# giuliop/AlgoPlonk

Hardware: AMD Instinct MI355X
Metric: proofs/sec (higher is better)
Workload: dtype u32x8 (Montgomery Fr/Fp)

## Files before the change

algoplonk_amd/_lib.py:

```python
from __future__ import annotations

import ctypes as C
import os

_HERE = os.path.dirname(os.path.abspath(__file__))
LIB_PATH = os.environ.get("APK_LIB") or os.path.join(_HERE, "libapk.so")

APK_BN254 = 0
APK_BLS12_381 = 1
APK_OK = 0
APK_ERR_ARG, APK_ERR_HIP, APK_ERR_STATE, APK_ERR_WITNESS, APK_ERR_VERIFY = 1, 2, 3, 4, 5
ABI_VERSION = 5
G1_MAX = 96
G2_MAX = 192
MAX_COMMITMENTS = 2
NB_BLINDING = 9

SYMBOLS = [
    "apk_last_error", "apk_abi_version", "apk_device_count", "apk_g1_bytes", "apk_fp_bytes",
    "apk_ctx_create", "apk_ctx_destroy", "apk_msm_ctx_create", "apk_ctx_get_vk", "apk_msm_g1", "apk_msm_g1_device", "apk_msm_g1_batch_device", "apk_ctx_set_commit_hook", "apk_device_copy", "apk_ntt",
    "apk_prove", "apk_prove_device", "apk_verify", "apk_verify_ex", "apk_g2_decompress", "apk_g2_mul_generator", "apk_g1_mul_batch", "apk_g1_decompress", "apk_g1_to_lagrange", "apk_marshal_proof", "apk_marshal_public_inputs",
    "apk_fe_from_be", "apk_fe_to_be", "apk_hash_fr", "apk_host_fe_op", "apk_host_g1_op", "apk_g1_sum",
    "apk_device_fe_op", "apk_device_g1_op", "apk_host_feu_op", "apk_device_feu_op", "apk_feu_shape", "apk_device_poly_op",
    "apk_device_alloc", "apk_device_free", "apk_device_upload", "apk_device_download",
    "apk_host_alloc", "apk_host_free", "apk_host_register", "apk_host_unregister",
    "apk_stats_enable", "apk_stats_read", "apk_paths_read",
    "apk_ctx_set_wire_hook", "apk_coset_ntt_device",
    "apk_comm_create", "apk_comm_destroy", "apk_comm_rank", "apk_comm_world", "apk_comm_barrier", "apk_comm_max_f64", "apk_comm_bind",
    "apk_comm_transport", "apk_msm_g1_sharded", "apk_comm_split_begin", "apk_comm_split_end", "apk_comm_serve", "apk_comm_set_compute",
    "apk_comm_commit", "apk_comm_wires", "apk_comm_rccl_ranks", "apk_comm_rccl_selftest",
    "apk_comm_commit_local", "apk_comm_spmd_begin", "apk_comm_spmd_end", "apk_comm_allgather_device", "apk_comm_subcoset_active",
    "apk_ctx_set_subcoset", "apk_comm_transport_reason", "apk_comm_link_probe", "apk_comm_phase_ms", "apk_ctx_msm_window",
    "apk_verify_batch", "apk_g1_lincomb_segments", "apk_device_sched_read", "apk_runtime_read",
    "apk_kzg_open", "apk_kzg_open_device", "apk_kzg_batch_open", "apk_kzg_batch_open_device", "apk_kzg_verify", "apk_kzg_batch_verify",
    "apk_kzg_fold_challenge", "apk_kzg_shape",
    "apk_kzg_open_lagrange", "apk_kzg_open_lagrange_device", "apk_kzg_batch_open_lagrange", "apk_kzg_batch_open_lagrange_device",
    "apk_kzg_lagrange_shape",
    "apk_kzg_open_multi", "apk_kzg_open_multi_device", "apk_kzg_batch_verify_multi", "apk_kzg_multi_weights",
    "apk_kzg_open_multi_lagrange", "apk_kzg_open_multi_lagrange_device",
    "apk_kzg_all_prepare", "apk_kzg_open_all", "apk_kzg_open_all_device",
    "apk_kzg_cosets_prepare", "apk_kzg_open_cosets", "apk_kzg_open_cosets_device", "apk_kzg_verify_coset",
    "apk_kzg_batch_verify_cosets", "apk_kzg_cosets_weights", "apk_kzg_cosets_fold", "apk_kzg_cosets_phase_ms",
    "apk_proof_blob_len", "apk_unmarshal_proof", "apk_unmarshal_public_inputs", "apk_verify_blob", "apk_verify_batch_keys", "apk_verify_blobs",
]


class ApkError(RuntimeError):
    def __init__(self, code: int, msg: str):
        super().__init__("libapk error %d: %s" % (code, msg))
        self.code = code


class CircuitDesc(C.Structure):
    _fields_ = [
        ("curve", C.c_int), ("device", C.c_int), ("n", C.c_uint64), ("nb_public", C.c_uint32),
        ("nb_commitments", C.c_uint32), ("srs_g1", C.c_void_p), ("srs_g1_lagrange", C.c_void_p),
        ("ql", C.c_void_p), ("qr", C.c_void_p), ("qm", C.c_void_p), ("qo", C.c_void_p), ("qk", C.c_void_p),
        ("perm", C.c_void_p), ("qcp", C.c_void_p * MAX_COMMITMENTS),
        ("commitment_constraint_index", C.c_uint32 * MAX_COMMITMENTS), ("msm_window", C.c_int), ("slots", C.c_int),
# ... 45 lines not shown
    ]


class VerifyKeysTrace(C.Structure):
    _fields_ = [
        ("d", C.c_uint8 * 32), ("rho", (C.c_uint8 * 32) * 4), ("lin_commitment", (C.c_uint8 * G1_MAX) * 4),
        ("a", C.c_uint8 * G1_MAX), ("b", C.c_uint8 * G1_MAX), ("groups", C.c_uint32), ("folds", C.c_uint32),
    ]


class KzgVk(C.Structure):
    _fields_ = [("curve", C.c_int), ("g1", C.c_uint8 * G1_MAX), ("g2", (C.c_uint8 * G2_MAX) * 2)]


class Stats(C.Structure):
    _fields_ = [
        ("msm_accumulate_ms", C.c_double), ("msm_accumulate_launches", C.c_uint64), ("msm_pairs", C.c_uint64),
        ("msm_total_ms", C.c_double), ("msm_batches", C.c_uint64), ("ntt_ms", C.c_double), ("ntt_elements", C.c_uint64),
        ("prove_ms", C.c_double), ("proofs", C.c_uint64), ("round_ms", C.c_double * 4), ("host_lincomb_ms", C.c_double),
        ("msm_sort_ms", C.c_double), ("msm_tail_ms", C.c_double),
    ]


class PathCounts(C.Structure):
    _names = ["proofs", "msm_batches", "msm_sort_two_level", "msm_sort_two_level_by_load", "msm_sort_fused", "msm_lean_tail",
              "msm_rowcol_serial", "msm_combine_quad", "msm_small_units", "msm_one_launch", "msm_lagrange_wires", "ntt_sequences",
              "ntt_radix4", "ntt_radix4_by_load", "tail_fill_proofs", "host_lincomb_pooled", "msm_units_by_load", "host_inputs",
              "gang_proofs", "gang_msm_launches", "gang_ntt_launches", "gang_kernel_launches", "forms_by_device_load"]
    _later = ["msm_inplace"]
    _fields_ = [(n, C.c_uint64) for n in _names + _later]

    def as_dict(self) -> dict:
        return {n: int(getattr(self, n)) for n in self._names + self._later}


class DeviceSched(C.Structure):
    _names = ["contexts", "max_streams", "streams_in_use", "streams_peak", "proofs_in_flight", "proofs_peak", "waiting", "device_wide"]
    _fields_ = [(n, C.c_uint32) for n in _names]

    def as_dict(self) -> dict:
        return {n: int(getattr(self, n)) for n in self._names}


HWQ_UNSET, HWQ_UNREADABLE = -1, -2


class Runtime(C.Structure):
    _names = ["hw_queues_found", "hw_queues_left", "hw_queues_need", "hw_queues_written", "hw_queues_now", "first_hip_call",
              "hw_queues_at_first_hip", "reserved"]
    _fields_ = [(n, C.c_int32) for n in _names]

    def as_dict(self) -> dict:
        return {n: int(getattr(self, n)) for n in self._names if n != "reserved"}


POLY_VECS, POLY_FRS, POLY_INTS, POLY_OUTS = 32, 24, 8, 6
(POLY_GRAND_PRODUCT, POLY_SCAN, POLY_QUOTIENT, POLY_MERGE, POLY_EVAL, POLY_LINCOMB, POLY_DERIVE_POWERS, POLY_KZG_QUOTIENT, POLY_BLIND,
 POLY_BLIND3, POLY_TAIL, POLY_KZG_QUOTIENT2) = range(12)


class PolyArgs(C.Structure):
    _fields_ = [("vec", C.c_void_p * POLY_VECS), ("len", C.c_uint64 * POLY_VECS), ("fr", (C.c_uint8 * 32) * POLY_FRS),
                ("iv", C.c_int64 * POLY_INTS), ("out", C.c_void_p * POLY_OUTS), ("out_len", C.c_uint64 * POLY_OUTS)]


COMMIT_HOOK = C.CFUNCTYPE(C.c_int, C.c_void_p, C.c_int, C.c_uint32, C.POINTER(C.c_void_p), C.POINTER(C.c_uint32), C.c_void_p)
# ... 52 lines not shown
                                         C.POINTER(vp), C.POINTER(sz), C.c_uint32, C.POINTER(i32), C.POINTER(VerifyKeysTrace)]
    lib.apk_g1_lincomb_segments.argtypes = [i32, i32, vp, vp, C.POINTER(u64), C.c_uint32, vp]
    lib.apk_g2_decompress.argtypes = [i32, vp, vp]
    lib.apk_g2_mul_generator.argtypes = [i32, vp, vp]
    lib.apk_g1_mul_batch.argtypes = [i32, i32, vp, vp, u64, vp]
    lib.apk_g1_decompress.argtypes = [i32, i32, vp, u64, vp]
    lib.apk_g1_to_lagrange.argtypes = [i32, i32, vp, u64, vp]
    lib.apk_marshal_proof.argtypes = [C.POINTER(Proof), vp, sz, C.POINTER(sz)]
    lib.apk_marshal_public_inputs.argtypes = [i32, vp, C.c_uint32, vp, sz]
    lib.apk_fe_from_be.argtypes = [i32, i32, vp, vp]
    lib.apk_fe_to_be.argtypes = [i32, i32, vp, vp]
    lib.apk_hash_fr.argtypes = [i32, vp, vp]
    lib.apk_host_fe_op.argtypes = [i32, i32, i32, vp, vp, vp]
    lib.apk_host_g1_op.argtypes = [i32, i32, vp, vp, vp]
    lib.apk_device_fe_op.argtypes = [i32, i32, i32, i32, u64, vp, vp, vp]
    lib.apk_device_g1_op.argtypes = [i32, i32, i32, u64, vp, vp, vp]
    lib.apk_host_feu_op.argtypes = [i32, i32, i32, u64, vp, vp]
    lib.apk_device_feu_op.argtypes = [i32, i32, i32, i32, u64, vp, vp]
    lib.apk_feu_shape.argtypes = [i32, i32, C.POINTER(i32), C.POINTER(i32), C.POINTER(C.c_uint32)]
    if hasattr(lib, "apk_device_poly_op"):
        lib.apk_device_poly_op.argtypes = [i32, i32, i32, C.POINTER(PolyArgs)]
    lib.apk_g1_sum.argtypes = [i32, vp, u64, vp]
    lib.apk_device_alloc.argtypes = [vp, sz, C.POINTER(vp)]
    lib.apk_device_free.argtypes = [vp, vp]
    lib.apk_device_upload.argtypes = [vp, vp, vp, sz]
    lib.apk_device_download.argtypes = [vp, vp, vp, sz]
    lib.apk_host_alloc.argtypes = [i32, sz, C.POINTER(vp)]
    lib.apk_host_free.argtypes = [vp]
    lib.apk_host_register.argtypes = [vp, sz]
    lib.apk_host_unregister.argtypes = [vp]
    lib.apk_stats_enable.argtypes = [vp, i32]
    lib.apk_stats_read.argtypes = [vp, C.POINTER(Stats), i32]
    lib.apk_paths_read.argtypes = [vp, C.POINTER(PathCounts), i32]
    if hasattr(lib, "apk_device_sched_read"):
        lib.apk_device_sched_read.argtypes = [i32, C.POINTER(DeviceSched), i32]
    if hasattr(lib, "apk_runtime_read"):
        lib.apk_runtime_read.argtypes = [C.POINTER(Runtime)]
    lib.apk_ctx_msm_window.argtypes = [vp]
    lib.apk_ctx_set_wire_hook.argtypes = [vp, WIRE_HOOK, vp]
    lib.apk_coset_ntt_device.argtypes = [vp, vp, u64, vp]
    lib.apk_comm_create.argtypes = [i32, i32, C.c_char_p, i32, C.POINTER(vp)]
    lib.apk_comm_destroy.argtypes = [vp]; lib.apk_comm_destroy.restype = None
    lib.apk_comm_rank.argtypes = [vp]
    lib.apk_comm_world.argtypes = [vp]
    lib.apk_comm_barrier.argtypes = [vp]
    lib.apk_comm_max_f64.argtypes = [vp, C.POINTER(C.c_double)]
    lib.apk_comm_bind.argtypes = [vp, vp]
    lib.apk_comm_transport.argtypes = [vp]; lib.apk_comm_transport.restype = C.c_char_p
    lib.apk_comm_rccl_ranks.argtypes = [vp]
    lib.apk_comm_transport_reason.argtypes = [vp]; lib.apk_comm_transport_reason.restype = C.c_char_p
    lib.apk_comm_link_probe.argtypes = [vp, sz, sz, C.POINTER(C.c_double), C.POINTER(C.c_double)]
    lib.apk_comm_phase_ms.argtypes = [vp, C.POINTER(C.c_double), i32]
    lib.apk_comm_rccl_selftest.argtypes = [i32, C.POINTER(i32)]
    lib.apk_msm_g1_sharded.argtypes = [vp, vp, u64, vp]
    lib.apk_comm_split_begin.argtypes = [vp]
    lib.apk_comm_split_end.argtypes = [vp]
    lib.apk_comm_serve.argtypes = [vp, C.POINTER(u64)]
    lib.apk_comm_set_compute.argtypes = [vp, C.POINTER(Compute)]
    lib.apk_comm_commit.argtypes = [vp, i32, C.c_uint32, vp, vp, vp]
    lib.apk_comm_wires.argtypes = [vp, C.c_uint32, vp, vp, vp]
    lib.apk_comm_commit_local.argtypes = [vp, i32, C.c_uint32, vp, vp, vp]
    lib.apk_comm_spmd_begin.argtypes = [vp]
    lib.apk_comm_spmd_end.argtypes = [vp]
    lib.apk_comm_allgather_device.argtypes = [vp, vp, C.c_size_t]
    lib.apk_comm_subcoset_active.argtypes = [vp]
    lib.apk_ctx_set_subcoset.argtypes = [vp, i32, i32, vp, vp]
# ... 69 lines not shown
```

algoplonk_amd/csrc/apk_api.cpp:

```cpp
#include <stdarg.h>
#include <stdio.h>
#include <stdlib.h>
#include <string.h>
#include <atomic>
#include <mutex>
#include <string>
#include <type_traits>

#include <hip/hip_runtime_api.h>

#include "backend.h"
#include "device_sched.h"
#include "ec.h"
#include "kernels_kzg.h"
#include "kernels_kzg_lagrange.h"
#include "plonk_protocol.h"
#include "poly_run.h"
#include "proof_codec.h"
#include "runtime_env.h"
#include "selftest_ops.h"

namespace apk {

static thread_local std::string g_err;
// ... 492 lines not shown
    if (e != hipSuccess) { (void)hipGetLastError(); set_error("hipHostRegister(%zu): %s", bytes, hipGetErrorString(e)); return APK_ERR_HIP; }
    return APK_OK;
}
int apk_host_unregister(void* p) {
    if (!p) return APK_OK;
    hipError_t e = hipHostUnregister(p);
    if (e != hipSuccess) { (void)hipGetLastError(); set_error("hipHostUnregister: %s", hipGetErrorString(e)); return APK_ERR_HIP; }
    return APK_OK;
}

int apk_device_alloc(apk_ctx* ctx, size_t bytes, void** p) { NEED_CTX(); return ctx->be->dev_alloc(bytes, p); }
int apk_device_free(apk_ctx* ctx, void* p) { NEED_CTX(); return ctx->be->dev_free(p); }
int apk_device_upload(apk_ctx* ctx, void* d, const void* s, size_t b) { NEED_CTX(); return ctx->be->dev_upload(d, s, b); }
int apk_device_download(apk_ctx* ctx, void* d, const void* s, size_t b) { NEED_CTX(); return ctx->be->dev_download(d, s, b); }
int apk_stats_enable(apk_ctx* ctx, int en) { NEED_CTX(); return ctx->be->stats_enable(en); }
int apk_stats_read(apk_ctx* ctx, apk_stats* out, int reset) { NEED_CTX(); if (!out) { set_error("null out"); return APK_ERR_ARG; } return ctx->be->stats_read(out, reset); }
int apk_ctx_msm_window(apk_ctx* ctx) { if (!ctx || !ctx->be) return 0; return ctx->be->msm_window(); }
int apk_device_sched_read(int device, apk_device_sched* out, int reset) {
    if (!out) { set_error("null out"); return APK_ERR_ARG; }
    if (device < 0 || device >= 4096) { set_error("device %d out of range", device); return APK_ERR_ARG; }
    memset(out, 0, sizeof *out);
    out->max_streams = (uint32_t)sched_max_streams();
    out->device_wide = sched_device_wide() ? 1u : 0u;
    DeviceSched* sc = device_sched_for(device);
    if (!sc) return APK_OK;
    const DeviceSched::Counts c = sc->read(reset != 0);
    out->contexts = c.contexts; out->max_streams = c.max_streams;
    out->streams_in_use = c.streams_in_use; out->streams_peak = c.streams_peak;
    out->proofs_in_flight = c.proofs_in_flight; out->proofs_peak = c.proofs_peak;
    out->waiting = c.waiting;
    return APK_OK;
}
int apk_paths_read(apk_ctx* ctx, apk_path_counts* out, int reset) { NEED_CTX(); if (!out) { set_error("null out"); return APK_ERR_ARG; } return ctx->be->paths_read(out, reset); }
int apk_runtime_read(apk_runtime* out) {
    if (!out) { set_error("null out"); return APK_ERR_ARG; }
    memset(out, 0, sizeof *out);
    out->hw_queues_found = g_runtime.found; out->hw_queues_left = g_runtime.left;
    out->hw_queues_need = g_runtime.need; out->hw_queues_written = g_runtime.written;
    out->hw_queues_now = hwq_parse(getenv("GPU_MAX_HW_QUEUES"));
    out->first_hip_call = g_runtime.first_hip.load();
    out->hw_queues_at_first_hip = g_runtime.at_first_hip.load();
    return APK_OK;
}

int apk_g1_mul_batch(int curve, int device, const void* base, const void* scalars, uint64_t count, void* out) {
    if (!base || !scalars || !out) { set_error("null argument"); return APK_ERR_ARG; }
    if (count == 0) return APK_OK;
    if (count >= (1ull << 31)) { set_error("count too large"); return APK_ERR_ARG; }
    runtime_checkpoint();
    if (curve == APK_BN254) return g1_mul_batch_bn254(device, base, scalars, count, out);
    if (curve == APK_BLS12_381) return g1_mul_batch_bls12381(device, base, scalars, count, out);
    set_error("unsupported curve: %d", curve);
    return APK_ERR_ARG;
}

int apk_g1_decompress(int curve, int device, const uint8_t* compressed, uint64_t count, void* out) {
    if (!compressed || !out) { set_error("null argument"); return APK_ERR_ARG; }
    if (count == 0) return APK_OK;
    if (count >= (1ull << 31)) { set_error("count too large"); return APK_ERR_ARG; }
    runtime_checkpoint();
    if (curve == APK_BN254) return g1_decompress_bn254(device, compressed, count, out);
    if (curve == APK_BLS12_381) return g1_decompress_bls12381(device, compressed, count, out);
    set_error("unsupported curve: %d", curve);
    return APK_ERR_ARG;
}

// ... 124 lines not shown
```

algoplonk_amd/csrc/backend.h:

```cpp
#pragma once
#include <stdint.h>
#include <stddef.h>
#include <stdarg.h>
#include <stdio.h>
#include "../../include/apk.h"

namespace apk {

void set_error(const char* fmt, ...);

int env_int(const char* name, int dflt, int lo, int hi);

bool ctx_alive(const void* ctx);

class DeviceSched;
DeviceSched* device_sched_for(int device);
int device_stream_pool(int device, void** streams, int cap, int* count);

struct Backend {
    virtual ~Backend() {}
    virtual int init(const apk_circuit_desc* d) = 0;
    virtual int init_msm_only(int device, const void* bases, uint64_t count, int msm_window) = 0;
    virtual int get_vk(apk_vk* out) = 0;
    virtual int msm(int basis, const void* scalars, uint64_t len, bool on_device, void* out) = 0;
    virtual int msm_batch(int basis, uint32_t count, const void* const* d_scalars, const uint64_t* offsets, const uint64_t* lens, void* out) = 0;
    virtual int kzg_open(const void* poly, uint64_t len, bool on_device, const void* point, void* out_h, void* out_value) = 0;
    virtual int kzg_batch_open(uint32_t count, const void* const* polys, const uint64_t* lens, bool on_device, const void* digests,
                               const void* point, const uint8_t* extra, size_t extra_len, void* out_h, void* out_values, void* out_gamma) = 0;
    virtual int kzg_open_multi(uint32_t count, const void* const* polys, const uint64_t* lens, bool on_device, const void* points,
                               void* out_h, void* out_values) = 0;
    virtual int kzg_open_lagrange(const void* evals, uint64_t len, bool on_device, const void* point, void* out_h, void* out_value) = 0;
    virtual int kzg_batch_open_lagrange(uint32_t count, const void* const* evals, bool on_device, const void* digests, const void* point,
                                        const uint8_t* extra, size_t extra_len, void* out_h, void* out_values, void* out_gamma) = 0;
    virtual int kzg_open_multi_lagrange(uint32_t count, const void* const* evals, bool on_device, const void* points, void* out_h,
                                        void* out_values) = 0;
    virtual int kzg_all_prepare(const void* srs_g1, uint64_t count) = 0;
    virtual int kzg_open_all(const void* poly, uint64_t len, bool on_device, void* out_h, void* out_values) = 0;
    virtual int kzg_cosets_prepare(const void* srs_g1, uint64_t count, uint32_t coset_size) = 0;
    virtual int kzg_open_cosets(const void* poly, uint64_t len, bool on_device, void* out_h, void* out_values) = 0;
    virtual int set_commit_hook(apk_commit_hook fn, void* user) = 0;
    virtual int dev_copy(void* d, const void* s, size_t bytes) = 0;
    virtual int set_wire_hook(apk_wire_hook fn, void* user) = 0;
    virtual int set_subcoset(int k, int G, apk_gather_hook fn, void* user) = 0;
    virtual int device_ordinal() = 0;
    virtual int msm_window() = 0;
    virtual uint64_t domain_size() = 0;
    virtual int coset_ntt_dev(const void* d_in, uint64_t len, void* d_out) = 0;
    virtual int ntt(int which, int inverse, int coset, void* data) = 0;
    virtual int prove(const void* L, const void* R, const void* O, bool on_device, const void* pub, const void* blinding,
                      const void* const* pi2, apk_proof* out) = 0;
    virtual int dev_alloc(size_t bytes, void** p) = 0;
    virtual int dev_free(void* p) = 0;
    virtual int dev_upload(void* d, const void* s, size_t bytes) = 0;
    virtual int dev_download(void* d, const void* s, size_t bytes) = 0;
    virtual int stats_enable(int enable) = 0;
    virtual int stats_read(apk_stats* out, int reset) = 0;
    virtual int paths_read(apk_path_counts* out, int reset) = 0;
};

int g1_mul_batch_bn254(int device, const void* base, const void* scalars, uint64_t count, void* out);
int g1_mul_batch_bls12381(int device, const void* base, const void* scalars, uint64_t count, void* out);
int g1_decompress_bn254(int device, const uint8_t* in, uint64_t count, void* out);
int g1_decompress_bls12381(int device, const uint8_t* in, uint64_t count, void* out);
int g1_to_lagrange_bn254(int device, const void* points, uint64_t n, void* out);
int g1_to_lagrange_bls12381(int device, const void* points, uint64_t n, void* out);
int fe_op_device_bn254(int device, int field, int op, uint64_t count, const void* a, const void* b, void* out);
int fe_op_device_bls12381(int device, int field, int op, uint64_t count, const void* a, const void* b, void* out);
int feu_op_device_bn254(int device, int field, int op, uint64_t count, const void* in, void* out);
int feu_op_device_bls12381(int device, int field, int op, uint64_t count, const void* in, void* out);
int g1_op_device_bn254(int device, int op, uint64_t count, const void* p, const void* q, void* out);
int g1_op_device_bls12381(int device, int op, uint64_t count, const void* p, const void* q, void* out);
int poly_op_device_bn254(int device, int op, const apk_poly_args* args);
int poly_op_device_bls12381(int device, int op, const apk_poly_args* args);
int g1_lincomb_segments_bn254(int device, const void* points, const void* scalars, const uint64_t* seg, uint32_t nb_segments, void* out);
int g1_lincomb_segments_bls12381(int device, const void* points, const void* scalars, const uint64_t* seg, uint32_t nb_segments, void* out);
int g1_check_points_bn254(int device, const void* points, uint64_t count, uint8_t* flags);
int g1_check_points_bls12381(int device, const void* points, uint64_t count, uint8_t* flags);
int kzg_cosets_fold_bn254(int device, int log_l, uint32_t count, const void* values, const void* scale, const void* step, const void* tw, void* out);
int kzg_cosets_fold_bls12381(int device, int log_l, uint32_t count, const void* values, const void* scale, const void* step, const void* tw, void* out);
Backend* make_backend_bn254();
Backend* make_backend_bls12381();

int host_fe_from_be(int curve, int field, const uint8_t* be, void* out);
int host_fe_to_be(int curve, int field, const void* in, uint8_t* be);

}
```

algoplonk_amd/csrc/backend_impl.h:

```cpp
#pragma once
#include <hip/hip_runtime.h>
#include <algorithm>
#include <atomic>
#include <chrono>
#include <condition_variable>
#include <memory>
#include <new>
#include <mutex>
#include <string.h>
#include <time.h>
#include <vector>

#include "backend.h"
#include "dev_buf.h"
#include "slot_pinned.h"
#include "msm_run.h"
#include "kzg_run.h"
#include "kzg_all_run.h"
#include "kzg_cosets_run.h"
#include "ntt_run.h"
#include "kernels_poly.h"
#include "poly_run.h"
#include "gang_run.h"
#include "setup_run.h"
// ... 3 lines not shown
#include "plonk_protocol.h"

namespace apk {

template <class FRP, class FPP, int CURVE_ID>
class CurveBackend : public Backend {
  public:
    using Fr = Fe<FRP>;
    using Fp = Fe<FPP>;
    using Aff = Affine<FPP>;
    using Pt = XYZZ<FPP>;
    using PtU = XYZZ<FPP, FeU<FPP>>;
    using Proto = PlonkProtocol<FRP, FPP>;

    static Fr fr_u64(uint64_t v) {
        Fr a = Fr::zero();
        a.l[0] = (uint32_t)v;
        a.l[1] = (uint32_t)(v >> 32);
        return Fr::to_mont(a);
    }

    static_assert(PIN_AFF + MSM_MAX_BATCH * sizeof(Aff) <= PIN_XYZZ, "a proof's batch of affine commitments fits its region");
    static_assert(PIN_XYZZ + MSM_ARGS_MAX * sizeof(Pt) <= PIN_FR, "the XYZZ sums of a launch sequence fit their region");
    static_assert(PIN_FR + (EVAL_MAX > KZG_MAX_POLYS ? EVAL_MAX : KZG_MAX_POLYS) * sizeof(Fr) <= PIN_TAIL, "evaluations and an opening's values fit the scalar region");

    struct ProverKnobs {
        int lc_threads = env_int("APK_HOST_LINCOMB_THREADS", FPP::N <= 8 ? 1 : 3, 1, 8);
        bool host_glv = env_int("APK_HOST_GLV", 1, 0, 1) != 0;
        bool host_fixed = env_int("APK_HOST_FIXED", 1, 0, 1) != 0;
        int powers_derive = env_int("APK_POWERS_DERIVE", 1, 0, 1);
        int open_pair = env_int("APK_OPEN_PAIR", 1, 0, 1);
        int lin_early_h = env_int("APK_LIN_EARLY_H", 1, 0, 1);
        int tail_fill = env_int("APK_TAIL_FILL", 1, 0, 2);
    };
    static const ProverKnobs& prover_knobs() { static const ProverKnobs k{}; return k; }

    struct GraphKey {
        const void* table; MsmBatchArgs a;
        bool operator==(const GraphKey& o) const { return table == o.table && memcmp(&a, &o.a, sizeof a) == 0; }
    };
    struct Slot {
        hipStream_t stream = nullptr;
        hipStream_t own_stream = nullptr;
        Slot* lead = nullptr;
        int gang_idx = 0;
        bool in_gang = false;
        uint32_t res_off = 0;
        uint32_t res_write_off = 0;
        Gang gang;
        GangRecorder cmds;
        hipEvent_t ev0 = nullptr, ev1 = nullptr, ev2 = nullptr, ev3 = nullptr;
        size_t index = 0;
        DevBuf wl, wr, wo;
        DevBuf cl, cr, co, cz;
        DevBuf qk_lag, qk_can;
        DevBuf ratio, zlag, scan_tot;
        DevBuf el, er, eo, ez, eqk;
        DevBuf quot, hcan;
        DevBuf pw_z, pw_zi, pw_zw, pw_zwi;
        DevBuf tmp2, folded, tmp, q1, q2;
        DevBuf eval_partial, eval_result;
        DevBuf pi2_can[APK_MAX_COMMITMENTS], epi2[APK_MAX_COMMITMENTS];
        DevBuf scratch_in;
        KzgScratch<FRP> kzg;
        KzgAllScratch<FRP, FPP> kzg_all;
        KzgCosetsScratch<FRP, FPP> kzg_cosets;
        DevBuf ntt_wide;
        MsmWorkspace<FPP> msm;
        void* h_pinned = nullptr;
        uint32_t pending_pts = 0;
        uint8_t* d_pinned = nullptr;
        std::vector<std::pair<GraphKey, hipGraphExec_t>> graphs;
        bool hook_pending = false;
        int hook_basis = 0;
        MsmBatchArgs hook_args{};
        DevBuf sc_gather;
        DevBuf tail_flag;
        uint32_t epoch = 0;
        hipStream_t side = nullptr;
        hipEvent_t ev_acc = nullptr, ev_side = nullptr;
        hipEvent_t ev_sync = nullptr;
        int mark_acc = 0; bool side_pending = false;
    };

    int curve_ = CURVE_ID;
    int device_ = 0;
    uint32_t n_ = 0, log_n_ = 0, n4_ = 0;
    uint32_t nb_public_ = 0, nb_commit_ = 0;
    uint32_t cci_[APK_MAX_COMMITMENTS] = {0, 0};
    MsmCtxPlan msm_ctx_{};
    bool msm_only_ = false;
    std::unique_ptr<HostPool> lc_pool_;
    bool many_slots_ = false;
    int gang_cap_ = 1;
    uint32_t ws_batch_ = MSM_MAX_BATCH;
    Gang::Launcher gang_launcher_;
    uint32_t msm_bases_ = 0;
    Fr omega_, omega_inv_, omega4_, omega4_inv_, shift_, shift_inv_, n_inv_, n4_inv_;
    Fr zh_inv_[4];
    DevBuf tw_n_, twu_n_, twi_n_, tw_4n_, twi_4n_, coset_pre_, coset_post_inv_, scales_;
    DevBuf twu_n_x_, twi_n_x_, tw_4n_x_, twi_4n_x_;
    bool ntt_twu_ = false;
    DevBuf x4_, l0_4_;
    DevBuf s_lag_[3], ql_c_, qr_c_, qm_c_, qo_c_, qk_c_, s_c_[3], qcp_c_[APK_MAX_COMMITMENTS];
    DevBuf qk_lag_trace_;
    bool qk_direct_ = false;
    DevBuf eqk_trace_, inj_tab_[QK_INJECT_MAX];
    std::vector<uint32_t> inj_row_;
    std::vector<Fr> inj_trace_val_;
    DevBuf eql_, eqr_, eqm_, eqo_, es_[3], eqcp_[APK_MAX_COMMITMENTS];
    MsmTables tab_can_, tab_lag_;
    int wires_lag_mode_ = -1;
    DevBuf srs_keep_;
    Aff lag_dk_[3];
// ... 8 lines not shown
    KzgAllTables<FRP, FPP> all_tab_;
    std::mutex all_mu_;
    std::atomic<bool> all_ready_{false};
    bool tw_ready_ = false;
    KzgCosetsTables cos_tab_;
    std::atomic<uint32_t> cos_l_{0};
    std::vector<Slot*> slots_;
    std::vector<hipStream_t> stream_pool_;
    bool owns_streams_ = false;
    SlotGate gate_;
    struct InputSet {
        DevBuf w[3], pi2[APK_MAX_COMMITMENTS];
        hipStream_t copy = nullptr;
        hipEvent_t ready = nullptr;
        size_t index = 0;
    };
    std::vector<InputSet*> in_sets_;
    SlotGate in_gate_;
    hipStream_t copy_stream_ = nullptr;
    std::mutex mu_;
    apk_commit_hook hook_ = nullptr;
    void* hook_user_ = nullptr;
    apk_wire_hook wire_hook_ = nullptr;
    void* wire_hook_user_ = nullptr;
    struct SubCoset {
        int k = 0, G = 1, glog = 0;
        apk_gather_hook hook = nullptr;
        void* user = nullptr;
        DevBuf pre[2], post;
        Fr rho_inv[8];
        bool on() const { return G > 1 && hook; }
    } sc_;
    enum PathIdx { P_PROOFS, P_MSM_BATCHES, P_SORT2, P_SORT2_LOAD, P_SORT_FUSED, P_LEAN_TAIL, P_ROWCOL_SERIAL, P_COMBINE_QUAD, P_SMALL_UNITS,
                   P_ONE_LAUNCH, P_LAGRANGE_WIRES, P_NTT_SEQ, P_NTT_R4, P_NTT_R4_LOAD, P_TAIL_FILL, P_LINCOMB_POOL, P_UNIT_LOADED, P_HOST_INPUTS, P_GANG_PROOFS, P_GANG_MSM, P_GANG_NTT, P_GANG_KERNELS, P_DEVICE_LOAD, P_MSM_INPLACE, P_COUNT };
    std::atomic<uint64_t> paths_[P_COUNT] = {};
    void path(PathIdx i) { paths_[i].fetch_add(1, std::memory_order_relaxed); }
    bool device_load_over(int thr, bool* foreign = nullptr) {
        int own = 0;
        const int dev = gate_.load(&own);
        if (foreign) *foreign = dev > thr && own <= thr;
        return dev > thr;
    }
    int paths_read(apk_path_counts* out, int reset) override {
        static_assert(sizeof(apk_path_counts) >= P_COUNT * sizeof(uint64_t), "apk_path_counts holds every counter");
        memset(out, 0, sizeof *out);
        uint64_t* o = reinterpret_cast<uint64_t*>(out);
        for (int i = 0; i < P_COUNT; i++) o[i] = reset ? paths_[i].exchange(0, std::memory_order_relaxed) : paths_[i].load(std::memory_order_relaxed);
        return APK_OK;
    }
    bool stats_on_ = false;
    uint32_t simds_ = 1024;
    std::mutex stats_mu_;
    apk_stats stats_{};

    ~CurveBackend() override {
        (void)hipSetDevice(device_);
        gate_.detach();
        for (hipStream_t st : stream_pool_) if (st) (void)hipStreamSynchronize(st);
        if (copy_stream_) (void)hipStreamSynchronize(copy_stream_);
        for (InputSet* is : in_sets_) {
            if (is->ready) (void)hipEventDestroy(is->ready);
            delete is;
        }
        if (copy_stream_) (void)hipStreamDestroy(copy_stream_);
        for (Slot* s : slots_) {
            for (auto& e : s->graphs) (void)hipGraphExecDestroy(e.second);
            if (s->ev0) (void)hipEventDestroy(s->ev0);
            if (s->ev1) (void)hipEventDestroy(s->ev1);
            if (s->ev2) (void)hipEventDestroy(s->ev2);
            if (s->ev3) (void)hipEventDestroy(s->ev3);
            if (s->h_pinned) (void)hipHostFree(s->h_pinned);
            if (s->side) { (void)hipStreamSynchronize(s->side); (void)hipStreamDestroy(s->side); }
            if (s->ev_acc) (void)hipEventDestroy(s->ev_acc);
            if (s->ev_side) (void)hipEventDestroy(s->ev_side);
            if (s->ev_sync) (void)hipEventDestroy(s->ev_sync);
            delete s;
        }
        if (owns_streams_) for (hipStream_t st : stream_pool_) if (st) (void)hipStreamDestroy(st);
    }

    int run_ntt_batch(hipStream_t st, int which, bool inverse, int count, const Fr* const* ins, Fr* const* outs, const uint32_t* in_lens,
                      uint32_t out_len, const Fr* pre, const Fr* post, const Fr* scale, int sub_log = 0, bool semi = false) {
        Slot* m = gang_member();
        if (m && m->in_gang && st == m->stream && count <= NTT_MAX_BATCH) {
            NttReq<Fr> nr{};
            nr.which = which; nr.inverse = inverse; nr.count = count;
            for (int i = 0; i < count; i++) { nr.ins[i] = ins[i]; nr.outs[i] = outs[i]; nr.in_lens[i] = in_lens[i]; }
            nr.out_len = out_len; nr.pre = pre; nr.post = post; nr.scale = scale; nr.sub_log = sub_log; nr.semi = semi;
            GangReq r;
            r.kind = GANG_KIND_NTT; r.args = &nr; r.member = m;
            const int rc = m->lead->gang.meet(m->gang_idx, r, gang_launcher_);
            if (rc != APK_OK) set_error("%s", r.err.c_str());
            return rc;
        }
        return run_ntt_batch_now(st, which, inverse, count, ins, outs, in_lens, out_len, pre, post, scale, sub_log, semi);
    }
    const Fr* ntt_table(int which, bool inverse) const {
        if (ntt_twu_) return which ? (inverse ? ptr<Fr>(twi_4n_x_) : ptr<Fr>(tw_4n_x_)) : (inverse ? ptr<Fr>(twi_n_x_) : ptr<Fr>(twu_n_x_));
        return which ? (inverse ? ptr<Fr>(twi_4n_) : ptr<Fr>(tw_4n_)) : (inverse ? ptr<Fr>(twi_n_) : ptr<Fr>(twu_n_));
    }
    int run_ntt_batch_now(hipStream_t st, int which, bool inverse, int count, const Fr* const* ins, Fr* const* outs, const uint32_t* in_lens,
                          uint32_t out_len, const Fr* pre, const Fr* post, const Fr* scale, int sub_log = 0, bool semi = false) {
        const int log_n = (which ? (int)log_n_ + 2 : (int)log_n_) - sub_log;
        Slot* owner = nullptr;
        for (Slot* s : slots_) if (s->own_stream == st || (s->side && s->side == st)) owner = s;
        bool busy_now = false, busy_foreign = false;
        if (slots_.size() > 2 && ntt_plan_reads_load(log_n)) busy_now = device_load_over(1, &busy_foreign);
        const NttPlanIn in{log_n, count, out_len, sub_log, semi, (uint32_t)sizeof(FeU<FRP>), owner != nullptr, busy_now, busy_foreign};
        const NttPlan plan = ntt_plan(ntt_knobs(), in);
        if (plan.rc != APK_OK) { set_error("%s", plan.message); return plan.rc; }
        NttBatch nb{};
        for (int i = 0; i < count; i++) { nb.in[i] = ins[i]; nb.out[i] = outs[i]; nb.in_len[i] = in_lens[i]; }
        if (plan.needs_wide) for (int i = 0; i < count; i++) nb.wide[i] = ptr<FeU<FRP>>(owner->ntt_wide) + ((size_t)i << log_n);
        static constexpr PathIdx PATH_OF_BIT[] = {P_NTT_SEQ, P_NTT_R4, P_NTT_R4_LOAD, P_DEVICE_LOAD};
        for (uint32_t i = 0; i < sizeof PATH_OF_BIT / sizeof PATH_OF_BIT[0]; i++) if (plan.paths >> i & 1u) path(PATH_OF_BIT[i]);
        Slot* timed = stats_on_ ? owner : nullptr;
        if (timed) HIPCHK(hipEventRecord(timed->ev2, st));
        CHK(ntt_launch<FRP>(st, plan, nb, count, ntt_table(which, inverse), ntt_twu_, pre, post, scale));
        if (timed) {
            HIPCHK(hipEventRecord(timed->ev3, st));
            HIPCHK(hipEventSynchronize(timed->ev3));
            float ms = 0;
            HIPCHK(hipEventElapsedTime(&ms, timed->ev2, timed->ev3));
            std::lock_guard<std::mutex> g(stats_mu_);
            stats_.ntt_ms += ms;
            stats_.ntt_elements += ((uint64_t)1 << log_n) * count;
        }
        return APK_OK;
    }
    int run_ntt(hipStream_t st, int which, bool inverse, const Fr* in, Fr* out, uint32_t in_len, uint32_t out_len,
                const Fr* pre, const Fr* post, const Fr* scale, int sub_log = 0, bool semi = false) {
        return run_ntt_batch(st, which, inverse, 1, &in, &out, &in_len, out_len, pre, post, scale, sub_log, semi);
    }
    int coset_eval(hipStream_t st, int count, const Fr* const* ins, const uint32_t* lens, Fr* const* outs, int cls = 0) {
        if (!sc_.on()) return run_ntt_batch(st, 1, false, count, ins, outs, lens, n4_, ptr<Fr>(coset_pre_), nullptr, nullptr, 0, true);
        return run_ntt_batch(st, 1, false, count, ins, outs, lens, n4_ >> sc_.glog, ptr<Fr>(sc_.pre[cls]), nullptr, nullptr, sc_.glog);
    }
    int inv_ntt_n(hipStream_t st, const Fr* in, Fr* out) { return run_ntt(st, 0, true, in, out, n_, n_, nullptr, nullptr, ptr<Fr>(scales_)); }
    int coset_ntt_4n(hipStream_t st, const Fr* in, uint32_t len, Fr* out, bool semi = false) {
        return run_ntt(st, 1, false, in, out, len, n4_, ptr<Fr>(coset_pre_), nullptr, nullptr, 0, semi);
    }

    int build_lagrange_table(hipStream_t st, const Aff* d_srs, const void* h_lagrange) {
        DevBuf lag;
        CHK(lag.alloc((size_t)(n_ + 3) * sizeof(Aff)));
        if (h_lagrange) HIPCHK(hipMemcpyAsync(lag.p, h_lagrange, (size_t)n_ * sizeof(Aff), hipMemcpyHostToDevice, st));
        else CHK((g1_to_lagrange_dev<FRP, FPP>(d_srs, n_, ptr<Aff>(lag), st)));
        HIPCHK(hipMemcpyAsync(ptr<Aff>(lag) + n_, lag_dk_, sizeof lag_dk_, hipMemcpyHostToDevice, st));
        CHK((build_tables<FRP, FPP>(st, msm_ctx_, ptr<Aff>(lag), n_ + 3, tab_lag_, true)));
        HIPCHK(hipStreamSynchronize(st));
        lag_ready_.store(true, std::memory_order_release);
        return APK_OK;
    }
    bool lagrange_ready() const { return lag_ready_.load(std::memory_order_acquire); }
    bool lagrange_possible() const { return lagrange_ready() || (srs_keep_.p && !lag_failed_.load(std::memory_order_relaxed)); }
    bool ensure_lagrange_table(hipStream_t st) {
        if (lagrange_ready()) return true;
        std::lock_guard<std::mutex> lk(lag_mu_);
        if (lagrange_ready()) return true;
        if (!srs_keep_.p || lag_failed_.load(std::memory_order_relaxed)) return false;
        const int rc = build_lagrange_table(st, ptr<Aff>(srs_keep_), nullptr);
        if (rc != APK_OK) {
            (void)hipGetLastError();
            tab_lag_.table.release();
            tab_lag_.built = false;
// ... 24 lines not shown
        HIPCHK(hipStreamBeginCapture(s.stream, hipStreamCaptureModeThreadLocal));
        const int rc = run_msm_body(s, T, a);
        const hipError_t e = hipStreamEndCapture(s.stream, &g);
        if (rc != APK_OK) { if (g) (void)hipGraphDestroy(g); return rc; }
        HIPCHK(e);
        hipGraphExec_t exec = nullptr;
        HIPCHK(hipGraphInstantiate(&exec, g, nullptr, nullptr, 0));
        (void)hipGraphDestroy(g);
        constexpr size_t GRAPH_CACHE = 8;
        if (s.graphs.size() >= GRAPH_CACHE) {
            HIPCHK(hipStreamSynchronize(s.stream));
            (void)hipGraphExecDestroy(s.graphs.back().second);
            s.graphs.pop_back();
        }
        s.graphs.insert(s.graphs.begin(), std::make_pair(key, exec));
        HIPCHK(hipGraphLaunch(exec, s.stream));
        s.pending_pts = a.batch;
        return APK_OK;
    }

    int run_msm_body(Slot& s, const MsmTables& T, const MsmBatchArgs& a) {
        hipStream_t st = s.stream;
        MsmBatchIn in{};
        in.batch = a.batch; in.len = a.len; in.offset = a.offset;
        in.n_bases = T.n_bases; in.ctx_bases = msm_bases_;
        in.simds = simds_; in.slots = (uint32_t)slots_.size();
        if (slots_.size() > 2) in.others_busy = device_load_over(1, &in.others_foreign);
        in.scan_runs = APK_PHASE(32);
        in.ws_batch = ws_batch_;
        in.lt_max = MsmQuad<FPP>::LT;
        in.counts_words = s.msm.counts.bytes / 4; in.sort_tmp_bytes = s.msm.sort_tmp.bytes;
        in.has_sort_tmp = s.msm.sort_tmp.p != nullptr; in.has_ptot2 = s.msm.ptot2.p != nullptr;
        const MsmBatchPlan p = msm_plan_batch(msm_ctx_, msm_knobs(), in);
        static constexpr PathIdx PATH_OF_BIT[] = {P_UNIT_LOADED, P_SMALL_UNITS, P_SORT2, P_SORT2_LOAD, P_SORT_FUSED, P_LEAN_TAIL, P_COMBINE_QUAD, P_ROWCOL_SERIAL, P_DEVICE_LOAD, P_MSM_INPLACE};
        for (uint32_t i = 0; i < sizeof PATH_OF_BIT / sizeof PATH_OF_BIT[0]; i++) if (p.paths >> i & 1u) path(PATH_OF_BIT[i]);
        if (p.rc == APK_ERR_ARG) { set_error("%s", p.message); return p.rc; }
        if (p.rc == APK_OK) {
            path(P_MSM_BATCHES);
            if (s.res_write_off + a.batch > (uint32_t)MSM_ARGS_MAX) { set_error("msm: result area overflow"); return APK_ERR_STATE; }
        }
        Pt* const res_out = s.d_pinned ? pin_dev<Pt>(s.d_pinned, PIN_XYZZ) + s.res_write_off : ptr<Pt>(s.msm.result_xyzz);
        MsmEvents ev;
        if (stats_on_) { ev.before = s.ev0; ev.scanned = s.ev2; ev.accumulated = s.ev3; ev.reduced = s.ev1; }
        ev.acc = s.ev_acc; ev.mark_acc = s.mark_acc;
        CHK((msm_launch_batch<FRP, FPP>(st, msm_ctx_, s.msm, ptr<Aff>(T.table), T.n_bases, a, p, res_out, ev)));
        if (!s.d_pinned) HIPCHK(hipMemcpyAsync(pin_host<Pt>(s.h_pinned, PIN_XYZZ) + s.res_write_off, s.msm.result_xyzz.p, a.batch * sizeof(Pt), hipMemcpyDeviceToHost, st));
        s.pending_pts = a.batch;
        if (stats_on_) {
            HIPCHK(hipEventSynchronize(s.ev1));
            float tot = 0, acc = 0, srt = 0, tail = 0;
            HIPCHK(hipEventElapsedTime(&tot, s.ev0, s.ev1));
            HIPCHK(hipEventElapsedTime(&acc, s.ev2, s.ev3));
            HIPCHK(hipEventElapsedTime(&srt, s.ev0, s.ev2));
            HIPCHK(hipEventElapsedTime(&tail, s.ev3, s.ev1));
            std::lock_guard<std::mutex> g(stats_mu_);
            stats_.msm_sort_ms += srt;
            stats_.msm_tail_ms += tail;
            stats_.msm_total_ms += tot;
            stats_.msm_batches += 1;
            stats_.msm_accumulate_ms += acc;
            stats_.msm_accumulate_launches += 1;
            for (uint32_t b = 0; b < a.batch; b++) stats_.msm_pairs += a.len[b];
        }
        return APK_OK;
    }

    static Slot*& hook_slot() { static thread_local Slot* p = nullptr; return p; }

    int commit(Slot& s, const MsmTables& T, int basis, const MsmBatchArgs& a) {
        if (!hook_ && s.in_gang) {
            MsmReq mr{&T, a};
            GangReq r;
            r.kind = GANG_KIND_MSM; r.args = &mr; r.member = &s;
            const int rc = s.lead->gang.meet(s.gang_idx, r, gang_launcher_);
            if (rc != APK_OK) set_error("%s", r.err.c_str());
            return rc;
        }
        if (!hook_) return run_msm(s, T, a);
        for (uint32_t b = 0; b < a.batch; b++)
            if (a.len[b] > T.n_bases || a.offset[b] > T.n_bases - a.len[b]) { set_error("msm: %u scalars exceed the %u bases", a.len[b], T.n_bases); return APK_ERR_ARG; }
        s.hook_pending = true; s.hook_basis = basis; s.hook_args = a;
        s.hook_args.plain = T.plain ? 1u : 0u;
        return APK_OK;
    }

    int tail_fill(Slot& s) {
        const int on = prover_knobs().tail_fill;
        const int graphs = msm_knobs().graph;
        if (!on || graphs || hook_ || wire_hook_ || stats_on_ || !qk_direct_ || sc_.on()) return 0;
        if (gate_.load() != 1) return 0;
        if (!s.side) {
            int least = 0, greatest = 0;
            (void)hipDeviceGetStreamPriorityRange(&least, &greatest);
            if (hipStreamCreateWithPriority(&s.side, hipStreamNonBlocking, least) != hipSuccess) { s.side = nullptr; return 0; }
            if (hipEventCreateWithFlags(&s.ev_acc, hipEventDisableTiming) != hipSuccess ||
                hipEventCreateWithFlags(&s.ev_side, hipEventDisableTiming) != hipSuccess) return 0;
        }
        return s.ev_acc && s.ev_side ? on : 0;
    }
    int side_begin(Slot& s) { HIPCHK(hipStreamWaitEvent(s.side, s.ev_acc, 0)); return APK_OK; }
    int side_end(Slot& s) { HIPCHK(hipEventRecord(s.ev_side, s.side)); s.side_pending = true; return APK_OK; }

    int wait_stream(Slot& s) {
        static const int mode = env_int("APK_SYNC_BLOCKING", -1, -1, 2);
        static const int poll_us = env_int("APK_SYNC_POLL_US", 50, 1, 10000);
        const bool loaded = slots_.size() > 2 && device_load_over(2);
        if (s.ev_sync && (mode == 2 || (mode < 0 && loaded))) {
            HIPCHK(hipEventRecord(s.ev_sync, s.stream));
            for (;;) {
                const hipError_t e = hipEventQuery(s.ev_sync);
                if (e == hipSuccess) return APK_OK;
                if (e != hipErrorNotReady) { (void)hipGetLastError(); set_error("hipEventQuery: %s", hipGetErrorString(e)); return APK_ERR_HIP; }
                struct timespec ts = {0, (long)poll_us * 1000L};
                nanosleep(&ts, nullptr);
            }
        }
        if (mode == 1 && s.ev_sync) {
            HIPCHK(hipEventRecord(s.ev_sync, s.stream));
            HIPCHK(hipEventSynchronize(s.ev_sync));
            return APK_OK;
        }
        HIPCHK(hipStreamSynchronize(s.stream));
        return APK_OK;
    }

    int sync_results(Slot& s) {
        if (s.in_gang) {
            GangReq r;
            r.kind = GANG_KIND_FLUSH; r.member = &s;
            const int rc = s.lead->gang.meet(s.gang_idx, r, gang_launcher_);
            if (rc != APK_OK) { set_error("%s", r.err.c_str()); return rc; }
        }
        CHK(wait_stream(s));
        if (s.side_pending) { s.side_pending = false; HIPCHK(hipStreamWaitEvent(s.stream, s.ev_side, 0)); }
        if (s.hook_pending) {
            s.hook_pending = false;
            const MsmBatchArgs& a = s.hook_args;
            uint8_t pts[MSM_MAX_BATCH * sizeof(Aff)];
            hook_slot() = &s;
            const int rc = hook_(hook_user_, s.hook_basis, a.batch, a.scalars, a.len, pts);
            hook_slot() = nullptr;
            if (rc != APK_OK) { set_error("commit hook failed with %d", rc); return rc == APK_ERR_ARG ? APK_ERR_ARG : APK_ERR_STATE; }
            memcpy(pin_host<Aff>(s.h_pinned, PIN_AFF), pts, a.batch * sizeof(Aff));
            s.pending_pts = 0;
            return APK_OK;
        }
        const Slot& from = s.lead ? *s.lead : s;
        const Pt* g = pin_host<Pt>(from.h_pinned, PIN_XYZZ) + s.res_off;
        static_assert(MSM_MAX_BATCH <= HOST_AFFINE_BATCH, "a proof's batch of sums is one batch conversion");
        host_xyzz_batch_to_affine<FPP>(g, s.pending_pts, pin_host<Aff>(s.h_pinned, PIN_AFF));
        s.pending_pts = 0;
        return APK_OK;
    }

    int alloc_slot(Slot& s) {
        s.lead = &s;
        HIPCHK(hipEventCreate(&s.ev0));
        HIPCHK(hipEventCreate(&s.ev1));
        HIPCHK(hipEventCreate(&s.ev2));
        HIPCHK(hipEventCreate(&s.ev3));
        if (hipEventCreateWithFlags(&s.ev_sync, hipEventBlockingSync | hipEventDisableTiming) != hipSuccess) { (void)hipGetLastError(); s.ev_sync = nullptr; }
        HIPCHK(hipHostMalloc(&s.h_pinned, PIN_BYTES, hipHostMallocDefault));
        memset(s.h_pinned, 0, PIN_BYTES);
        static const int zero_copy = env_int("APK_ZERO_COPY", 1, 0, 1);
        if (zero_copy) {
            void* dp = nullptr;
            if (hipHostGetDevicePointer(&dp, s.h_pinned, 0) == hipSuccess) s.d_pinned = static_cast<uint8_t*>(dp);
            else (void)hipGetLastError();
        }
        const size_t fn = (size_t)n_ * sizeof(Fr), fn3 = (size_t)(n_ + 4) * sizeof(Fr), f4 = (size_t)n4_ * sizeof(Fr);
        if (msm_only_) {
            CHK(s.scratch_in.alloc((size_t)msm_bases_ * sizeof(Fr)));
            return s.msm.alloc(msm_ctx_, msm_knobs(), msm_bases_, 1, many_slots_);
        }
        CHK(s.wl.alloc(fn3)); CHK(s.wr.alloc(fn3)); CHK(s.wo.alloc(fn3));
        CHK(s.cl.alloc(fn3)); CHK(s.cr.alloc(fn3)); CHK(s.co.alloc(fn3)); CHK(s.cz.alloc(fn3));
        for (DevBuf* b : {&s.cl, &s.cr, &s.co, &s.cz}) HIPCHK(hipMemset(b->p, 0, fn3));
        CHK(s.qk_lag.alloc(fn)); CHK(s.qk_can.alloc(fn));
        CHK(s.ratio.alloc(fn)); CHK(s.zlag.alloc(fn));
        CHK(s.scan_tot.alloc((size_t)(2 * (cdiv(n_ + 4, SCAN_BLOCK) + 1) + 2) * sizeof(Fr)));
        CHK(s.el.alloc(f4)); CHK(s.er.alloc(f4)); CHK(s.eo.alloc(f4)); CHK(s.ez.alloc(f4)); CHK(s.eqk.alloc(f4));
        CHK(s.quot.alloc(f4)); CHK(s.hcan.alloc(f4));
        CHK(s.pw_z.alloc(fn3)); CHK(s.pw_zi.alloc(fn3)); CHK(s.pw_zw.alloc(fn3)); CHK(s.pw_zwi.alloc(fn3));
        CHK(s.tmp2.alloc(fn3)); CHK(s.folded.alloc(fn3)); CHK(s.tmp.alloc(fn3)); CHK(s.q1.alloc(fn3)); CHK(s.q2.alloc(fn3));
        CHK(s.eval_partial.alloc((size_t)EVAL_MAX * cdiv(n_ + 4, EVAL_BLOCK) * sizeof(Fr)));
        CHK(s.eval_result.alloc(EVAL_MAX * sizeof(Fr)));
        for (uint32_t k = 0; k < nb_commit_; k++) { CHK(s.pi2_can[k].alloc(fn)); CHK(s.epi2[k].alloc(f4)); }
        CHK(s.scratch_in.alloc(f4));
        CHK(s.tail_flag.alloc(16));
        HIPCHK(hipMemset(s.tail_flag.p, 0, 16));
        CHK(s.ntt_wide.alloc((size_t)NTT_MAX_BATCH * gang_cap_ * n4_ * sizeof(FeU<FRP>)));
        return s.msm.alloc(msm_ctx_, msm_knobs(), msm_bases_, ws_batch_, many_slots_);
    }

// ... 113 lines not shown
            pr[i] = reqs[i]->kind == GANG_KIND_MSM ? msm_of(reqs[i]).plan_req() : reqs[i]->kind == GANG_KIND_NTT ? ntt_of(reqs[i]).plan_req() : GangPlanReq{GANG_KIND_FLUSH, 0, nullptr, GangNttShape{}};
            recs[i] = &member_of(reqs[i]).cmds;
        }
        const GangPlan plan = gang_plan_meeting(pr, count, ws_batch_, (uint32_t)(NTT_MAX_BATCH * gang_cap_));
        int merged = 0;
        const int frc = gang_flush(recs, count, member_of(reqs[0]).stream, &merged);
        for (int i = 0; i < merged; i++) path(P_GANG_KERNELS);
        if (frc != APK_OK) {
            for (int i = 0; i < count; i++) { reqs[i]->rc = frc; reqs[i]->err = apk_last_error(); }
            return;
        }
        for (int i = 0; i < count; i++) if (reqs[i]->kind == GANG_KIND_FLUSH) reqs[i]->rc = APK_OK;
        for (int gi = 0; gi < plan.groups; gi++) {
            const GangGroup& g = plan.group[gi];
            Slot& lead = *member_of(reqs[g.req[0]]).lead;
            int rc;
            if (g.kind == GANG_KIND_MSM) {
                MsmBatchArgs c{};
                c.batch = g.total;
                for (int k = 0; k < g.n; k++) {
                    const MsmBatchArgs& a = msm_of(reqs[g.req[k]]).a;
                    for (uint32_t b = 0; b < a.batch; b++) { c.scalars[g.first[k] + b] = a.scalars[b]; c.len[g.first[k] + b] = a.len[b]; c.offset[g.first[k] + b] = a.offset[b]; }
                    member_of(reqs[g.req[k]]).res_off = g.res_off(k);
                }
                const uint32_t lead_pending = lead.pending_pts;
                lead.res_write_off = g.res_base;
                rc = run_msm(lead, *msm_of(reqs[g.req[0]]).T, c);
                lead.res_write_off = 0;
                lead.pending_pts = lead_pending;
                if (g.n > 1) path(P_GANG_MSM);
                for (int k = 0; k < g.n; k++) member_of(reqs[g.req[k]]).pending_pts = rc == APK_OK ? msm_of(reqs[g.req[k]]).a.batch : 0;
            } else {
                const Fr* ins[NTT_ARGS_MAX]; Fr* outs[NTT_ARGS_MAX]; uint32_t lens[NTT_ARGS_MAX];
                for (int k = 0; k < g.n; k++) {
                    const NttReq<Fr>& m = ntt_of(reqs[g.req[k]]);
                    for (int t = 0; t < m.count; t++) { ins[g.first[k] + t] = m.ins[t]; outs[g.first[k] + t] = m.outs[t]; lens[g.first[k] + t] = m.in_lens[t]; }
                }
                const NttReq<Fr>& f = ntt_of(reqs[g.req[0]]);
                rc = run_ntt_batch_now(lead.own_stream, f.which, f.inverse, (int)g.total, ins, outs, lens, f.out_len, f.pre, f.post, f.scale, f.sub_log, f.semi);
                if (g.n > 1) path(P_GANG_NTT);
            }
            for (int k = 0; k < g.n; k++) { reqs[g.req[k]]->rc = rc; if (rc != APK_OK) reqs[g.req[k]]->err = apk_last_error(); }
        }
    }

    Slot* acquire() {
        const SlotGate::Ticket t = gate_.acquire();
        Slot* s = slots_[t.slot];
        s->own_stream = s->stream = stream_pool_[(size_t)t.stream];
        return s;
    }
    void drain(Slot* s) {
        if (s->stream) (void)hipStreamSynchronize(s->stream);
        if (s->side_pending && s->side) { (void)hipStreamSynchronize(s->side); s->side_pending = false; }
        (void)hipGetLastError();
    }
    void release(Slot* s, bool ok) {
        if (!ok) drain(s);
        if (s->side_pending) { s->side_pending = false; if (s->own_stream) (void)hipStreamWaitEvent(s->own_stream, s->ev_side, 0); }
        s->own_stream = s->stream = nullptr;
        gate_.release(s->index);
    }
    struct SlotGuard {
        CurveBackend* b; Slot* s; bool ok = false;
        SlotGuard(CurveBackend* b_) : b(b_), s(b_->acquire()) {}
        ~SlotGuard() { b->release(s, ok); }
    };
    struct MaybeGuard {
        CurveBackend* b; Slot* s; bool owned; bool ok = false;
        static Slot* own(CurveBackend* b) { return std::count(b->slots_.begin(), b->slots_.end(), hook_slot()) ? hook_slot() : nullptr; }
        MaybeGuard(CurveBackend* b_) : b(b_), s(own(b_)), owned(s == nullptr) { if (owned) s = b->acquire(); }
        ~MaybeGuard() { if (owned) b->release(s, ok); }
// ... 992 lines not shown
        CHK(sync_results(s));
        run.bsb[k] = hp[0];
        run.cval[k] = Proto::hash_fr(run.bsb[k]);
        store_pt(run.out->bsb22[k], run.bsb[k]);
    }
    Fr* canon[3] = {ptr<Fr>(s.cl), ptr<Fr>(s.cr), ptr<Fr>(s.co)};
    const Fr* wires[3] = {run.dL, run.dR, run.dO};
    CHK(wire_route(run));
    const bool use_lag = run.use_lag;
    Fr* lagv[3] = {ptr<Fr>(s.wl), ptr<Fr>(s.wr), ptr<Fr>(s.wo)};
    if (use_lag)
        for (int j = 0; j < 3; j++) HIPCHK(hipMemcpyAsync(lagv[j], wires[j], fn, hipMemcpyDeviceToDevice, st));
    {
        const uint32_t lens[3] = {n, n, n};
        CHK(run_ntt_batch(st, 0, true, 3, wires, canon, lens, n, nullptr, nullptr, ptr<Fr>(scales_)));
    }
    {
        Blind3<FRP> b3{};
        for (int j = 0; j < 3; j++) {
            b3.p[j] = canon[j]; b3.b[j].v[0] = run.bl[2 * j]; b3.b[j].v[1] = run.bl[2 * j + 1];
            b3.lag[j] = use_lag ? lagv[j] : nullptr;
        }
        CHK((klaunch<Blind3K<FRP>, 256>(st, 3, 64, 0, b3, n, 2)));
    }
    const int fill = run.fill = tail_fill(s);
    if (fill) path(P_TAIL_FILL);
    {
        MsmBatchArgs a{};
        a.batch = 3;
        for (int j = 0; j < 3; j++) { a.scalars[j] = use_lag ? lagv[j] : canon[j]; a.len[j] = n + 2; a.offset[j] = 0; }
        a.plain = use_lag ? 1u : 0u;
        if (use_lag) path(P_LAGRANGE_WIRES);
        s.mark_acc = fill;
        const int rc = use_lag ? commit(s, tab_lag_, 1, a) : commit(s, tab_can_, 0, a);
        s.mark_acc = 0;
        CHK(rc);
    }
    if (!qk_direct_) {
        HIPCHK(hipMemcpyAsync(s.qk_lag.p, qk_lag_trace_.p, fn, hipMemcpyDeviceToDevice, st));
        if (nb_public_) HIPCHK(hipMemcpyAsync(s.qk_lag.p, run.pubv, (size_t)nb_public_ * sizeof(Fr), hipMemcpyHostToDevice, st));
        for (uint32_t k = 0; k < nb_commit_; k++)
            HIPCHK(hipMemcpyAsync(ptr<Fr>(s.qk_lag) + nb_public_ + cci_[k], &run.cval[k], sizeof(Fr), hipMemcpyHostToDevice, st));
        CHK(inv_ntt_n(st, ptr<Fr>(s.qk_lag), ptr<Fr>(s.qk_can)));
        CHK(coset_ntt_4n(st, ptr<Fr>(s.qk_can), n, ptr<Fr>(s.eqk)));
    }
    {
        Fr* ev[3] = {ptr<Fr>(s.el), ptr<Fr>(s.er), ptr<Fr>(s.eo)};
        const uint32_t lens[3] = {n + 2, n + 2, n + 2};
        if (wire_hook_ && !sc_.on()) {
            HIPCHK(hipStreamSynchronize(st));
            const void* cin[3] = {canon[0], canon[1], canon[2]};
            void* eout[3] = {ev[0], ev[1], ev[2]};
            hook_slot() = &s;
            const int rc = wire_hook_(wire_hook_user_, 3, cin, lens, eout);
            hook_slot() = nullptr;
            if (rc != APK_OK) { set_error("wire hook failed with %d", rc); return rc == APK_ERR_ARG ? APK_ERR_ARG : APK_ERR_STATE; }
        } else if (fill) {
            CHK(side_begin(s));
            CHK(run_ntt_batch(s.side, 1, false, 3, canon, ev, lens, n4_, ptr<Fr>(coset_pre_), nullptr, nullptr, 0, true));
            CHK(side_end(s));
        } else {
            CHK(coset_eval(st, 3, canon, lens, ev));
        }
    }
    CHK(sync_results(s));
    if (run.measuring) wire_route_finish(run);
    for (int j = 0; j < 3; j++) { run.lro[j] = hp[j]; store_pt(run.out->lro[j], run.lro[j]); }
    return APK_OK;
}

template <class FRP, class FPP, int CURVE_ID>
int CurveBackend<FRP, FPP, CURVE_ID>::round2_grand_product(ProofRun& run) {
    Slot& s = run.s;
    hipStream_t st = run.st;
    const uint32_t n = n_;
    const int fill = run.fill;
    {
        Fr* hfr = pin_host<Fr>(s.h_pinned, PIN_FR);
        const GpScan<FRP> g = poly_gp_scan<FRP>(ptr<Fr>(s.ratio), ptr<Fr>(s.tmp), ptr<Fr>(s.scan_tot), n);
        CHK(poly_gp_terms<FRP>(kl(), st, run.dL, run.dR, run.dO, (const Fr*)ptr<Fr>(s_lag_[0]), (const Fr*)ptr<Fr>(s_lag_[1]), (const Fr*)ptr<Fr>(s_lag_[2]),
                               (const Fr*)ptr<Fr>(tw_n_), n, run.beta * fr_u64(32), run.gamma, run.beta_u * fr_u64(32), run.beta_u2 * fr_u64(32), g));
        Fr* const tot_pin = pin_dev<Fr>(s.d_pinned, PIN_FR);
        Fr* const tot_out = tot_pin ? tot_pin : poly_gp_total_slot<FRP>(g, n);
        CHK(poly_gp_scans<FRP>(kl(), st, g, n, tot_out));
        if (!tot_pin) HIPCHK(hipMemcpyAsync(hfr, tot_out, sizeof(Fr), hipMemcpyDeviceToHost, st));
        CHK(sync_results(s));
        CHK(poly_gp_finish<FRP>(kl(), st, g, n, hfr[0], ptr<Fr>(s.zlag)));
    }
    CHK(inv_ntt_n(st, ptr<Fr>(s.zlag), ptr<Fr>(s.cz)));
    {
        Fr4<FRP> b{};
        b.v[0] = run.bl[6]; b.v[1] = run.bl[7]; b.v[2] = run.bl[8];
        CHK((klaunch<BlindK<FRP>, 256>(st, 1, 64, 0, ptr<Fr>(s.cz), n, b, 3)));
        MsmBatchArgs a{};
        a.batch = 1; a.scalars[0] = s.cz.p; a.len[0] = n + 3; a.offset[0] = 0;
        s.mark_acc = fill;
        const int rc = commit(s, tab_can_, 0, a);
        s.mark_acc = 0;
        CHK(rc);
    }
    if (fill) {
        CHK(side_begin(s));
        CHK(coset_ntt_4n(s.side, ptr<Fr>(s.cz), n + 3, ptr<Fr>(s.ez), true));
        CHK(side_end(s));
    } else {
        const Fr* cin = ptr<Fr>(s.cz); Fr* eout = ptr<Fr>(s.ez);
        const uint32_t zl = n + 3;
        CHK(coset_eval(st, 1, &cin, &zl, &eout));
        if (sc_.on() && sc_.glog == 3) {
            Fr* e2 = ptr<Fr>(s.eqk);
            CHK(coset_eval(st, 1, &cin, &zl, &e2, 1));
        }
    }
    CHK(sync_results(s));
    run.zcom = pin_host<Aff>(s.h_pinned, PIN_AFF)[0];
    store_pt(run.out->z, run.zcom);
    return APK_OK;
}

template <class FRP, class FPP, int CURVE_ID>
QuotientArgs<FRP> CurveBackend<FRP, FPP, CURVE_ID>::quotient_args(const ProofRun& run) {
    Slot& s = run.s;
    QuotientArgs<FRP> q{};
    q.l = ptr<Fr>(s.el); q.r = ptr<Fr>(s.er); q.o = ptr<Fr>(s.eo); q.z = ptr<Fr>(s.ez); q.qk = ptr<Fr>(s.eqk);
    if (qk_direct_) {
        q.qk = ptr<Fr>(eqk_trace_);
        q.nb_inject = (int)inj_row_.size();
        for (size_t j = 0; j < inj_row_.size(); j++) {
            const Fr written = j < nb_public_ ? run.pubv[j] : run.cval[j - nb_public_];
            q.inj_delta[j] = written - inj_trace_val_[j];
            q.inj_tab[j] = inj_row_[j] == 0 ? ptr<Fr>(l0_4_) : ptr<Fr>(inj_tab_[j]);
        }
    }
    q.ql = ptr<Fr>(eql_); q.qr = ptr<Fr>(eqr_); q.qm = ptr<Fr>(eqm_); q.qo = ptr<Fr>(eqo_);
    q.s1 = ptr<Fr>(es_[0]); q.s2 = ptr<Fr>(es_[1]); q.s3 = ptr<Fr>(es_[2]);
    q.x = ptr<Fr>(x4_); q.l0 = ptr<Fr>(l0_4_);
    q.nb_commit = (int)nb_commit_;
    for (uint32_t k = 0; k < nb_commit_; k++) { q.qcp[k] = ptr<Fr>(eqcp_[k]); q.pi2[k] = ptr<Fr>(s.epi2[k]); }
    const Fr c5 = fr_u64(1u << 5), c10 = fr_u64(1u << 10), c20 = fr_u64(1u << 20);
    q.alpha = run.alpha * c20; q.beta = run.beta * c5; q.gamma = run.gamma; q.beta_u = run.beta_u * c5; q.beta_u2 = run.beta_u2 * c5;
    q.alpha2 = run.alpha * run.alpha * c10;
    for (int k = 0; k < 4; k++) q.zh_inv[k] = zh_inv_[k] * c5;
    for (int j = 0; j < q.nb_inject; j++) q.inj_delta[j] = q.inj_delta[j] * c5;
    q.n4 = n4_;
    return q;
}

template <class FRP, class FPP, int CURVE_ID>
int CurveBackend<FRP, FPP, CURVE_ID>::round3_quotient(ProofRun& run) {
    Slot& s = run.s;
    hipStream_t st = run.st;
    const uint32_t n = n_;
    {
        QuotientArgs<FRP> q = quotient_args(run);
        if (!sc_.on()) {
            CHK((klaunch<QuotientK<FRP>, POLY_THREADS>(st, cdiv(n4_, POLY_THREADS), POLY_THREADS, 0, q, ptr<Fr>(s.quot))));
            CHK(run_ntt(st, 1, true, ptr<Fr>(s.quot), ptr<Fr>(s.hcan), n4_, n4_, nullptr, ptr<Fr>(coset_post_inv_), nullptr));
        } else {
            const uint32_t m = n4_ >> sc_.glog;
            q.n4 = m; q.sub_k = (uint32_t)sc_.k; q.sub_glog = (uint32_t)sc_.glog; q.zs = ptr<Fr>(s.eqk);
            quotient_kernel<FRP><<<cdiv(m, POLY_THREADS), POLY_THREADS, 0, st>>>(q, ptr<Fr>(s.quot)); KCHK();
            Fr* mine = ptr<Fr>(s.sc_gather) + (size_t)sc_.k * m;
            CHK(run_ntt(st, 1, true, ptr<Fr>(s.quot), mine, m, m, nullptr, ptr<Fr>(sc_.post), nullptr, sc_.glog));
            HIPCHK(hipStreamSynchronize(st));
            hook_slot() = &s;
            const int grc = sc_.hook(sc_.user, s.sc_gather.p, (size_t)m * sizeof(Fr));
            hook_slot() = nullptr;
            if (grc != APK_OK) { set_error("sub-coset gather hook failed with %d", grc); return grc == APK_ERR_ARG ? APK_ERR_ARG : APK_ERR_STATE; }
            SubMergeArgs<FRP> ma{};
            for (int e = 0; e < 8; e++) ma.rho_inv[e] = sc_.rho_inv[e];
            ma.m = m; ma.glog = (uint32_t)sc_.glog;
            subcoset_merge_kernel<FRP><<<cdiv(m, POLY_THREADS), POLY_THREADS, 0, st>>>(ma, ptr<Fr>(s.sc_gather), ptr<Fr>(coset_post_inv_), ptr<Fr>(s.hcan)); KCHK();
        }
        MsmBatchArgs a{};
        a.batch = 3;
        for (int j = 0; j < 3; j++) { a.scalars[j] = ptr<Fr>(s.hcan) + (size_t)j * (n + 2); a.len[j] = n + 2; a.offset[j] = 0; }
        CHK(commit(s, tab_can_, 0, a));
        s.epoch++;
        const uint32_t tail4 = (n4_ - 3 * (n + 2)) * (uint32_t)(sizeof(Fr) / 16);
        uint32_t* const flag_pin = pin_dev<uint32_t>(s.d_pinned, PIN_TAIL);
        CHK(poly_tail_nonzero(kl(), st, reinterpret_cast<const uint4*>(ptr<Fr>(s.hcan) + 3 * (size_t)(n + 2)), tail4, s.epoch,
                              flag_pin ? flag_pin : ptr<uint32_t>(s.tail_flag)));
        if (!flag_pin) HIPCHK(hipMemcpyAsync(pin_host<uint32_t>(s.h_pinned, PIN_TAIL), s.tail_flag.p, 4, hipMemcpyDeviceToHost, st));
    }
    CHK(sync_results(s));
    if (*pin_host<const volatile uint32_t>(s.h_pinned, PIN_TAIL) == s.epoch) {
        set_error("quotient is not a polynomial: the witness does not satisfy the circuit");
        return APK_ERR_WITNESS;
    }
    const Aff* hp = pin_host<Aff>(s.h_pinned, PIN_AFF);
    for (int j = 0; j < 3; j++) { run.hcom[j] = hp[j]; store_pt(run.out->h[j], run.hcom[j]); }
    return APK_OK;
}

template <class FRP, class FPP, int CURVE_ID>
int CurveBackend<FRP, FPP, CURVE_ID>::zeta_powers(ProofRun& run) {
    Slot& s = run.s;
    hipStream_t st = run.st;
    const uint32_t n = n_;
    const Fr& zeta = run.zeta;
    const Fr zw = zeta * omega_;
    const bool z0 = zeta.is_zero();
    const Fr zeta_inv = Fr::inv(zeta), zw_inv = zeta_inv * omega_inv_;
    Fr* outs[4] = {ptr<Fr>(s.pw_z), ptr<Fr>(s.pw_zw), ptr<Fr>(s.pw_zi), ptr<Fr>(s.pw_zwi)};
    const Fr ws[4] = {zeta, zw, zeta_inv, zw_inv};
    if (z0 || !prover_knobs().powers_derive) return powers_batch(st, z0 ? 2 : 4, outs, ws, n + 3);
    Fr* two[2] = {outs[0], outs[2]};
    const Fr w2[2] = {zeta, zeta_inv};
    CHK(powers_batch(st, 2, two, w2, n + 3));
    DerivePowers<FRP> dp{};
    dp.in[0] = outs[0]; dp.out[0] = outs[1]; dp.inverse[0] = 0;
    dp.in[1] = outs[2]; dp.out[1] = outs[3]; dp.inverse[1] = 1;
    return klaunch<DerivePowersK<FRP>, POLY_THREADS>(st, dim3(cdiv(n + 3, POLY_THREADS), 2), POLY_THREADS, 0, dp, (const Fr*)ptr<Fr>(twu_n_), n, n + 3);
}

// ... 129 lines not shown
```

algoplonk_amd/csrc/gang_run.h:

```cpp
#pragma once
#include <hip/hip_runtime.h>
#include <new>
#include <vector>

#include "dev_buf.h"
#include "gang_kernel.h"
#include "gang_plan.h"
#include "msm_run.h"
#include "ntt_plan.h"

namespace apk {

constexpr size_t CMD_BLOB = 1024;
struct Cmd {
    dim3 grid, block;
    uint32_t lds = 0;
    int (*multi)(hipStream_t, const Cmd* const*, int) = nullptr;
    alignas(16) unsigned char blob[CMD_BLOB];
    GangSig sig() const { return GangSig{true, reinterpret_cast<uintptr_t>(multi), grid.x, grid.y, block.x, lds}; }
};

template <class K, int BOUNDS, class... P>
int launch_multi(hipStream_t st, const Cmd* const* cmds, int count) {
    static_assert(sizeof(Pack<P...>) <= CMD_BLOB, "kernel arguments exceed a recorded launch's blob");
    static_assert(sizeof(GangPack<P...>) <= 4096, "a gang's arguments exceed the kernel argument segment");
    GangPack<P...> g{};
    for (int i = 0; i < count; i++) g.m[i] = *reinterpret_cast<const Pack<P...>*>(cmds[i]->blob);
    dim3 grid = cmds[0]->grid;
    grid.z = (uint32_t)count;
    polyG_kernel<K, BOUNDS, P...><<<grid, cmds[0]->block, cmds[0]->lds, st>>>(g);
    KCHK();
    return APK_OK;
}

class GangRecorder {
  public:
    template <class K, int BOUNDS, class... P>
    void record(dim3 grid, dim3 block, size_t lds, P... p) {
        cmds_.emplace_back();
        Cmd& c = cmds_.back();
        c.grid = grid; c.block = block; c.lds = (uint32_t)lds;
        c.multi = &launch_multi<K, BOUNDS, P...>;
// ... 6 lines not shown
  private:
    std::vector<Cmd> cmds_;
};

inline int gang_flush(GangRecorder* const* recs, int count, hipStream_t st, int* merged) {
    size_t longest = 0;
    for (int m = 0; m < count; m++) if (recs[m]->size() > longest) longest = recs[m]->size();
    int rc = APK_OK;
    for (size_t i = 0; i < longest && rc == APK_OK; i++) {
        GangSig sigs[GANG_MAX];
        for (int m = 0; m < count; m++) sigs[m] = i < recs[m]->size() ? (*recs[m])[i].sig() : GangSig{};
        const GangFlushStep s = gang_plan_flush_step(sigs, count);
        for (int g = 0; g < s.groups && rc == APK_OK; g++) {
            const Cmd* grp[GANG_MAX];
            for (int k = 0; k < s.n[g]; k++) grp[k] = &(*recs[s.member[g][k]])[i];
            rc = grp[0]->multi(st, grp, s.n[g]);
            if (s.n[g] > 1) ++*merged;
        }
    }
    for (int m = 0; m < count; m++) recs[m]->clear();
    return rc;
}

struct MsmReq {
    const MsmTables* T;
    MsmBatchArgs a;
    GangPlanReq plan_req() const { return GangPlanReq{GANG_KIND_MSM, a.batch, T, GangNttShape{}}; }
};
template <class Fr>
struct NttReq {
    int which; bool inverse; int count;
    const Fr* ins[NTT_MAX_BATCH]; Fr* outs[NTT_MAX_BATCH]; uint32_t in_lens[NTT_MAX_BATCH];
    uint32_t out_len; const Fr *pre, *post, *scale; int sub_log; bool semi;
    GangPlanReq plan_req() const { return GangPlanReq{GANG_KIND_NTT, (uint32_t)count, nullptr, GangNttShape{which, inverse, out_len, pre, post, scale, sub_log, semi}}; }
};

}
```

algoplonk_amd/csrc/kernels_msm.h:

```cpp
#pragma once
#include "ec.h"
#include "msm_plan.h"

namespace apk {

constexpr uint32_t MSM_HEAVY_UNITS = 512;
__device__ __forceinline__ uint32_t msm_heavy_threshold(int lanes_log, uint32_t per_lane) {
    const uint32_t t = (4u * per_lane) << lanes_log;
    return t < 32u ? 32u : (t > MSM_HEAVY_UNITS ? MSM_HEAVY_UNITS : t);
}

struct MsmBatchArgs {
    const void* scalars[MSM_ARGS_MAX];
    uint32_t len[MSM_ARGS_MAX];
    uint32_t offset[MSM_ARGS_MAX];
    uint32_t batch;
    uint32_t plain;
};


constexpr int MSM_DIGITS_THREADS = 1024;
template <class FR, bool SCATTER, bool PLAIN = false>
__global__ void __launch_bounds__(MSM_DIGITS_THREADS) msm_digits_kernel(MsmBatchArgs a, MsmWindows win, uint32_t nb, uint32_t n_max, uint32_t G,
                                                         uint32_t* __restrict__ counts,
// ... 652 lines not shown


struct MsmScanTotalsLds {
    uint32_t s_bintot[MSM_BINS];
    uint16_t s_bins[MSM_SCAN_MAX_BLOCKS * MSM_BINS];
};
__device__ __forceinline__ void msm_scan_totals_body(uint32_t* __restrict__ block_tot, uint32_t* __restrict__ block_bins, uint32_t nblocks, uint32_t total,
                                                     uint32_t* __restrict__ offsets, uint32_t* __restrict__ unit_off, uint32_t* __restrict__ full_off,
                                                     uint32_t* s_cnt, uint32_t* s_unit, uint32_t* s_full, MsmScanTotalsLds& L) {
    const uint32_t t = threadIdx.x;
    const uint32_t h = t < nblocks ? block_tot[t] : 0u, hu = t < nblocks ? block_tot[nblocks + t] : 0u,
                   hf = t < nblocks ? block_tot[2 * nblocks + t] : 0u;
    s_cnt[t] = h; s_unit[t] = hu; s_full[t] = hf;
    for (uint32_t i = t; i < nblocks * MSM_BINS; i += MSM_SCAN_BLOCK) L.s_bins[i] = (uint16_t)block_bins[i];
    __syncthreads();
    if (t < MSM_BINS) {
        uint32_t run = 0;
        for (uint32_t blk = 0; blk < nblocks; blk++) run += L.s_bins[blk * MSM_BINS + t];
        L.s_bintot[t] = run;
    }
    __syncthreads();
    for (uint32_t d = 1; d < MSM_SCAN_BLOCK; d <<= 1) {
        uint32_t vc = 0, vu = 0, vf = 0;
        if (t >= d) { vc = s_cnt[t - d]; vu = s_unit[t - d]; vf = s_full[t - d]; }
        __syncthreads();
        s_cnt[t] += vc; s_unit[t] += vu; s_full[t] += vf;
        __syncthreads();
    }
    if (t < nblocks) { block_tot[t] = s_cnt[t] - h; block_tot[nblocks + t] = s_unit[t] - hu; block_tot[2 * nblocks + t] = s_full[t] - hf; }
    if (t == MSM_SCAN_BLOCK - 1) {
        offsets[total] = s_cnt[t]; unit_off[total] = s_unit[t]; full_off[total] = s_full[t];
        const uint32_t nonempty = total - L.s_bintot[MSM_UNIT_MAX];
        block_bins[nblocks * MSM_BINS] = nonempty ? s_unit[t] / nonempty : 0u;
    }
    if (t < MSM_BINS) {
        uint32_t run = 0;
        const uint32_t top = t < (uint32_t)MSM_UNIT_MAX ? MSM_UNIT_MAX : MSM_BINS;
        for (uint32_t r = top - 1; r > t; r--) run += L.s_bintot[r];
        for (uint32_t blk = 0; blk < nblocks; blk++) {
            const uint32_t v = L.s_bins[blk * MSM_BINS + t];
            block_bins[blk * MSM_BINS + t] = run;
            run += v;
        }
    }
}
template <int FUSED, int ITEMS = 1>
__global__ void __launch_bounds__(MSM_SCAN_BLOCK) msm_scan_local_kernel(const uint32_t* __restrict__ hist, uint32_t total, uint32_t unit,
                                                                         uint32_t* __restrict__ offsets, uint32_t* __restrict__ unit_off,
                                                                         uint32_t* __restrict__ full_off, uint32_t* __restrict__ rem_rank,
                                                                         uint32_t* __restrict__ merge_rank,
                                                                         uint32_t* __restrict__ block_tot ,
                                                                         uint32_t* __restrict__ block_bins , uint32_t nblocks,
                                                                         uint32_t* __restrict__ done) {
    constexpr uint32_t items = ITEMS;
    wave_priority<APK_PRIO_SORT>();
    __shared__ uint32_t s_cnt[MSM_SCAN_BLOCK];
    __shared__ uint32_t s_unit[MSM_SCAN_BLOCK];
    __shared__ uint32_t s_full[MSM_SCAN_BLOCK];
    __shared__ uint32_t s_bins[MSM_BINS];
    const uint32_t t = threadIdx.x, i0 = (blockIdx.x * MSM_SCAN_BLOCK + t) * items;
    if (t < MSM_BINS) s_bins[t] = 0;
    __syncthreads();
    uint32_t hv[ITEMS], sh = 0, su = 0, sf = 0;
#pragma unroll
    for (int it = 0; it < ITEMS; it++) {
        const uint32_t i = i0 + (uint32_t)it;
// ... 215 lines not shown
        }
    }
    if (slot < total_buckets && lane == 0 && !settled && unit_off[k + 1] - unit_off[k] <= heavy) bucket_sum[k] = acc;
}

template <class FP>
__device__ __forceinline__ void msm_combine_heavy_body(const XYZZ<FP, FeU<FP>>* __restrict__ partial, const uint32_t* __restrict__ unit_off,
                                                       uint32_t total_buckets, XYZZ<FP, FeU<FP>>* __restrict__ bucket_sum, uint32_t blk, uint32_t nblk,
                                                       uint32_t heavy) {
    using PT = XYZZ<FP, FeU<FP>>;
    __shared__ PT sm[256];
    const uint32_t t = threadIdx.x;
    const uint32_t per = (total_buckets + nblk - 1) / nblk;
    const uint32_t k0 = blk * per, k1 = min(k0 + per, total_buckets);
    bool any = false;
    for (uint32_t k = k0 + t; k < k1; k += 256) any |= unit_off[k + 1] - unit_off[k] > heavy;
    if (!__syncthreads_or(any)) return;
    for (uint32_t k = k0; k < k1; k++) {
        const uint32_t beg = unit_off[k], end = unit_off[k + 1];
        if (end - beg <= heavy) continue;
        PT acc = PT::inf();
        for (uint32_t u = beg + t; u < end; u += 256) acc.add_lazy(partial[u]);
        sm[t] = acc;
        __syncthreads();
        for (uint32_t d = 128; d >= 1; d >>= 1) {
            if (t < d) { PT o = sm[t + d]; acc.add_lazy(o); sm[t] = acc; }
            __syncthreads();
        }
        if (t == 0) bucket_sum[k] = acc;
        __syncthreads();
    }
}


template <class FP>
__global__ void __launch_bounds__(256) msm_rowcol_kernel(const XYZZ<FP, FeU<FP>>* __restrict__ bucket_sum, uint32_t nb, uint32_t rows,
                                                         uint32_t cols, XYZZ<FP, FeU<FP>>* __restrict__ rc) {
    wave_priority<APK_PRIO_TAIL>();
    using PT = XYZZ<FP, FeU<FP>>;
    __shared__ PT sm[256];
    const uint32_t m = blockIdx.y, x = blockIdx.x, t = threadIdx.x;
    const PT* src = bucket_sum + (size_t)m * nb;
    PT acc = PT::inf();
    if (x < rows) {
        for (uint32_t lo = t; lo < cols; lo += 256) acc.add_lazy(src[x * cols + lo]);
    } else {
        const uint32_t col = x - rows;
        for (uint32_t hi = t; hi < rows; hi += 256) acc.add_lazy(src[hi * cols + col]);
    }
    sm[t] = acc;
    __syncthreads();
    for (uint32_t d = 128; d >= 1; d >>= 1) {
        if (t < d) { PT o = sm[t + d]; acc.add_lazy(o); sm[t] = acc; }
        __syncthreads();
    }
    if (t == 0) rc[(size_t)m * (rows + cols) + x] = acc;
}

template <class FP>
__global__ void __launch_bounds__(256) msm_bitsum_kernel(const XYZZ<FP, FeU<FP>>* __restrict__ rc, uint32_t rows, uint32_t cols,
                                                         XYZZ<FP, FeU<FP>>* __restrict__ bit_partial) {
    wave_priority<APK_PRIO_TAIL>();
    using PT = XYZZ<FP, FeU<FP>>;
    __shared__ PT sm[256];
    const uint32_t bit = blockIdx.x, which = blockIdx.y, m = blockIdx.z, t = threadIdx.x;
    const PT* src = rc + (size_t)m * (rows + cols) + (which ? rows : 0);
// ... 347 lines not shown
```

algoplonk_amd/csrc/kernels_ntt.h:

```cpp
#pragma once
#include "ff.h"
#include "ffu.h"
#include "ntt_plan.h"

namespace apk {

__device__ __forceinline__ uint32_t bitrev32(uint32_t x, int bits) { return __brev(x) >> (32 - bits); }

struct NttBatch {
    const void* in[NTT_ARGS_MAX];
    void* out[NTT_ARGS_MAX];
    uint32_t in_len[NTT_ARGS_MAX];
    void* wide[NTT_ARGS_MAX];
};

template <class FR, bool TWU = false>
__global__ void __launch_bounds__(NTT_THREADS) ntt_pass_kernel(NttBatch nb, const Fe<FR>* __restrict__ tw,
                                                               const Fe<FR>* __restrict__ pre,
                                                               const Fe<FR>* __restrict__ post,
                                                               const Fe<FR>* __restrict__ scale,
                                                               NttPassArgs a) {
    wave_priority<APK_PRIO_FR>();
    using Fr = Fe<FR>;
    using Fu = FeU<FR>;
    static_assert(Fu::HEADROOM >= 64, "values reach (4 + 2 log2 N) p < 64 p over the stages of a transform (N <= 2^29)");
    extern __shared__ __attribute__((aligned(16))) unsigned char smem_raw[];
    Fu* sm = reinterpret_cast<Fu*>(smem_raw);
    const Fu* __restrict__ twu = reinterpret_cast<const Fu*>(tw);
    auto twiddle = [&](uint32_t idx) -> Fu {
        if constexpr (TWU) return twu[idx];
        else { Fr w = tw[idx]; return Fu::unpack(w.l); }
    };
    Fr* __restrict__ out = reinterpret_cast<Fr*>(nb.out[blockIdx.y]);
    const Fr* __restrict__ in = reinterpret_cast<const Fr*>(nb.in[blockIdx.y]);
    Fu* __restrict__ wide = reinterpret_cast<Fu*>(nb.wide[blockIdx.y]);
    const uint32_t in_len = nb.in_len[blockIdx.y];
    const int s = a.t1 - a.t0;
    const int tile_log = a.tile_log;
    const int clog = tile_log - s;
    const uint32_t C = 1u << clog;
    const uint32_t tile_elems = 1u << tile_log;
    const uint32_t g0 = blockIdx.x << clog;
    const uint32_t lomask = (1u << a.t0) - 1u;

    const uint32_t NT = blockDim.x;
    for (uint32_t e = threadIdx.x; e < tile_elems; e += NT) {
        uint32_t c = e & (C - 1), mid = e >> clog;
        uint32_t g = g0 + c;
        uint32_t idx = ((g >> a.t0) << a.t1) | (mid << a.t0) | (g & lomask);
        Fu v;
        if (a.first) {
            uint32_t src = bitrev32(idx, a.log_n);
            if (src < in_len) {
                Fr raw = in[src];
// ... 53 lines not shown
            if (t != 0) {
                y2 = Fu::mul_nr(twiddle(k2 << a.tw_shift), y2);
                sm[e00] = Fu::add_n(y0, y2);
                sm[e10] = Fu::template sub_k<2>(y0, y2);
            } else {
                sm[e00] = Fu::add_n(y0, y2);
                sm[e10] = Fu::template sub_k<4>(y0, y2);
            }
            sm[e01] = Fu::add_n(y1, y3);
            sm[e11] = Fu::template sub_n<2>(y1, y3);
        }
        __syncthreads();
    }
    const uint32_t nbf = tile_elems >> 1;
    for (; q < s; q++) {
        const int t = a.t0 + q;
        for (uint32_t bf = threadIdx.x; bf < nbf; bf += NT) {
            uint32_t c = bf & (C - 1), pr = bf >> clog;
            uint32_t low = pr & ((1u << q) - 1u);
            uint32_t mid0 = ((pr >> q) << (q + 1)) | low;
            uint32_t mid1 = mid0 | (1u << q);
            uint32_t g = g0 + c;
            uint32_t imod = (low << a.t0) | (g & lomask);
            uint32_t tidx = (imod << (a.log_n - 1 - t)) << a.tw_shift;
            uint32_t e0 = (mid0 << clog) | c, e1 = (mid1 << clog) | c;
            Fu u = sm[e0];
            Fu v = sm[e1];
            if (t != 0 && !(padded && v.is_zero())) v = Fu::mul_nr(twiddle(tidx), v);
            sm[e0] = Fu::add_n(u, v);
            sm[e1] = Fu::template sub_k<2>(u, v);
        }
        __syncthreads();
    }
    for (uint32_t e = threadIdx.x; e < tile_elems; e += NT) {
        uint32_t c = e & (C - 1), mid = e >> clog;
        uint32_t g = g0 + c;
        uint32_t idx = ((g >> a.t0) << a.t1) | (mid << a.t0) | (g & lomask);
        Fu v = sm[e];
        if (!a.last) { wide[idx] = v; continue; }
        if (idx >= a.out_len) continue;
        if (post) { Fr pw = post[idx]; v = Fu::mul_nr(Fu::unpack(pw.l), v); }
        if (scale) { Fr sc = scale[0]; v = Fu::mul_nr(Fu::unpack(sc.l), v); }
        if (!(post || scale)) v = Fu::template reduce_2p<32>(v);
        if (post || scale || !a.semi) v = Fu::template canon<1>(v);
        Fr o;
        v.pack(o.l);
        out[idx] = o;
    }
}

template <class FR>
__global__ void __launch_bounds__(256) unpack_table_kernel(const Fe<FR>* __restrict__ in, FeU<FR>* __restrict__ out, uint32_t count) {
    const uint32_t i = blockIdx.x * blockDim.x + threadIdx.x;
    if (i >= count) return;
    Fe<FR> v = in[i];
    out[i] = FeU<FR>::unpack(v.l);
}

constexpr int POWERS_MAX_BATCH = 4;
template <class FR>
struct PowersBatch {
    Fe<FR>* out[POWERS_MAX_BATCH];
    Fe<FR> w[POWERS_MAX_BATCH];
    Fe<FR> scale[POWERS_MAX_BATCH];
};
template <class FR>
struct PowersK {
    static __device__ __forceinline__ void run(PowersBatch<FR> pb, uint32_t count) {
        using Fr = Fe<FR>;
        using U = FeU<FR>;
        constexpr uint32_t PER = 8;
        Fr* __restrict__ out = pb.out[blockIdx.y];
        uint32_t t = blockIdx.x * blockDim.x + threadIdx.x;
        uint32_t start = t * PER;
        if (start >= count) return;
        const U wu = U::from_fe(pb.w[blockIdx.y]);
        U r = U::one();
        bool started = false;
        for (int b = 31; b >= 0; b--) {
            if (started) r = U::sqr(r);
            if ((start >> b) & 1u) { r = started ? U::mul(r, wu) : wu; started = true; }
// ... 16 lines not shown
```

algoplonk_amd/csrc/msm_plan.h:

```cpp
#pragma once
#include <stdint.h>
#include <stdio.h>
#include "../../include/apk.h"

namespace apk {

static inline uint32_t cdiv(uint64_t a, uint64_t b) { return (uint32_t)((a + b - 1) / b); }

constexpr int MSM_MAX_BATCH = 4;
constexpr int MSM_ARGS_MAX = 16;
constexpr int MSM_UNIT = 16;
constexpr int MSM_UNIT_MIN = 16, MSM_UNIT_MAX = 64;
constexpr int MSM_UNIT_SMALL = 4;
constexpr uint64_t MSM_SMALL_ENTRIES = 1ull << 20;
constexpr int MSM_COMBINE_LANES = 16;
#ifndef APK_MSM_PACKED_NB
#define APK_MSM_PACKED_NB 65536
#endif
constexpr uint32_t MSM_PACKED_NB = APK_MSM_PACKED_NB;
constexpr uint32_t MSM_G_MAX = 256;
constexpr uint32_t MSM_PART_MAX = 8192;
constexpr uint32_t MSM_PART_GMAX = 16384;
constexpr uint32_t MSM_LDS_WORDS = 40960;
constexpr uint32_t MSM_PART_TILE = 36864;
// ... 17 lines not shown
    uint16_t off[MSM_MAX_WINDOWS + 1];
    uint8_t width[MSM_MAX_WINDOWS];
};
struct MsmPartCfg {
    uint32_t idx_bits, pb_log;
    uint32_t P;
    uint32_t run_lanes;
};

struct MsmKnobs {
    int window = 0;
    uint32_t part_target = MSM_PART_TILE - 2048;
    int part_pblog = 0;
    int graph = 0;
    uint32_t unit = 0;
    uint32_t unit_loaded = 48;
    uint32_t unit_loaded_bases = 65536;
    uint32_t unit_small = MSM_UNIT_SMALL;
    uint32_t small_waves = 2;
    uint32_t slice = 2048;
    int digits_threads = 1024;
    int lean_tail = -1;
    int sort2 = -1;
    int part_small_scan = 1;
    int sort_fused = 1;
    int scan_fused = 0;
    int combine_dyn = 1;
    int sorted_merge = 1;
    int combine_quad = -1;
    int quad_tail = -1;
    int rowcol_serial = -1;
    int rowcol_lanes = 16;
    int inplace = -1;
};

struct MsmCtxPlan {
    int rc = APK_OK;
    char message[224] = {0};
    int c = 0, W = 0;
    uint32_t NB = 0;
    MsmWindows win{};
    MsmPartCfg part{};
};

inline size_t msm_digits_lds_bytes(uint32_t NB) { return NB >= MSM_PACKED_NB ? (size_t)NB * 2 : (size_t)NB * 4; }
inline bool msm_one_level_ok(uint32_t NB) { return NB <= 65536u; }
inline uint32_t msm_ctx_stage_max(const MsmCtxPlan& x) { return msm_part_stage_max(x.part.P ? x.part.P : 4u); }

inline MsmCtxPlan msm_plan_window(int bits, uint32_t bases, int c, const MsmKnobs& k) {
    MsmCtxPlan x;
    x.c = c;
    x.rc = APK_ERR_ARG;
    if (c < 7 || c > 20) { snprintf(x.message, sizeof x.message, "msm_window %d out of [7,20]", c); return x; }
    if (c == 17 && (uint64_t)bases > (uint64_t)MSM_G_MAX * 3072u) { snprintf(x.message, sizeof x.message, "msm_window 17 supports at most %u bases", MSM_G_MAX * 3072u); return x; }
    x.W = (bits + 1 + c - 1) / c;
    x.NB = 1u << (c - 1);
    {
        const int base = (bits + 1) / x.W, extra = (bits + 1) % x.W;
        x.win.W = x.W;
        int o = 0;
        for (int j = 0; j < x.W; j++) {
            x.win.off[j] = (uint16_t)o;
            x.win.width[j] = (uint8_t)(base + (j < extra ? 1 : 0));
            o += x.win.width[j];
        }
        x.win.off[x.W] = (uint16_t)o;
    }
// ... 60 lines not shown
    uint32_t items = 1;
    while (items < (uint32_t)MSM_SCAN_ITEMS_MAX && (uint64_t)MSM_SCAN_BLOCK * MSM_SCAN_MAX_BLOCKS * items < total_buckets) items <<= 1;
    return items;
}

struct MsmWorkspacePlan {
    uint64_t counts;
    uint64_t sort_tmp;
    uint64_t partial;
    uint64_t scan_blk;
};
inline MsmWorkspacePlan msm_plan_workspace(const MsmCtxPlan& x, const MsmKnobs& k, uint32_t bases, uint32_t batch, bool many_slots) {
    MsmWorkspacePlan w{};
    const uint64_t entries = (uint64_t)batch * bases * x.W;
    const uint32_t tb = batch * x.NB;
    const uint64_t g2max = (uint64_t)cdiv(bases, msm_slice_two_level(x, k)) + 1u;
    const uint64_t g2 = g2max > MSM_PART_GMAX ? MSM_PART_GMAX : g2max;
    const uint64_t two_level = (uint64_t)batch * g2 * ((uint64_t)x.part.P + 1) * 2 + (uint64_t)batch * x.part.P * (2 + MSM_PART_CHUNKS);
    const uint64_t one_level = msm_one_level_ok(x.NB) ? (uint64_t)tb * MSM_G_MAX : 0;
    w.counts = one_level > two_level ? one_level : two_level;
    if (msm_sort2_wanted(x, k, bases, many_slots) && (x.part.P >= 4 || !msm_one_level_ok(x.NB)))
        w.sort_tmp = entries + (uint64_t)batch * MSM_PART_GMAX * (uint64_t)x.W + 4096u;
    const uint64_t big = msm_max_units(entries, MSM_UNIT_MIN, tb);
    const uint64_t small = msm_max_units(entries < 4 * MSM_SMALL_ENTRIES ? entries : 4 * MSM_SMALL_ENTRIES, MSM_UNIT_SMALL, tb);
    w.partial = big > small ? big : small;
    w.scan_blk = (uint64_t)(3 + MSM_BINS) * (cdiv(tb, MSM_SCAN_BLOCK) + 1);
    return w;
}

enum MsmSortForm { MSM_SORT_ONE_LEVEL, MSM_SORT_FOUR_LAUNCH, MSM_SORT_FUSED };
enum MsmPathBit : uint32_t {
    MSM_PATH_UNIT_LOADED = 1u << 0, MSM_PATH_SMALL_UNITS = 1u << 1, MSM_PATH_SORT2 = 1u << 2, MSM_PATH_SORT2_LOAD = 1u << 3, MSM_PATH_SORT_FUSED = 1u << 4,
    MSM_PATH_LEAN_TAIL = 1u << 5, MSM_PATH_COMBINE_QUAD = 1u << 6, MSM_PATH_ROWCOL_SERIAL = 1u << 7, MSM_PATH_DEVICE_LOAD = 1u << 8,
    MSM_PATH_INPLACE = 1u << 9
};
struct MsmBatchIn {
    uint32_t batch;
    const uint32_t* len;
    const uint32_t* offset;
    uint32_t n_bases;
    uint32_t ctx_bases;
    uint32_t simds, slots;
    bool others_busy, others_foreign;
    bool scan_runs;
    uint32_t ws_batch;
    uint32_t lt_max;
    uint64_t counts_words, sort_tmp_bytes;
    bool has_sort_tmp, has_ptot2;
};
struct MsmBatchPlan {
    int rc = APK_OK;
    char message[160] = {0};
    uint32_t paths = 0;
    uint32_t maxlen = 0, total_buckets = 0;
    uint64_t entries = 0;
    uint32_t unit = 0, max_units = 0;
    uint32_t G = 0;
    MsmSortForm sort = MSM_SORT_ONE_LEVEL;
    bool small_scan = false;
    uint32_t stage_cap = 0, tile_cap = 0, run_lanes = 0;
    uint32_t scan_items = 1, scan_nblk = 0;
    bool lean = false;
    uint32_t per_lane = 5;
    int lanes_log = 0;
    bool dyn_lanes = false, cquad = false;
    bool inplace = false;
    int quad = 0;
    bool serial = false;
    int rowcol_lanes = 16;
    uint32_t rows = 0, cols = 0, cols_log = 0, nbits = 0, lt = 0;
};

inline MsmBatchPlan msm_plan_batch(const MsmCtxPlan& x, const MsmKnobs& k, const MsmBatchIn& in) {
    MsmBatchPlan p;
    if (in.batch == 0 || in.batch > in.ws_batch || in.batch > (uint32_t)MSM_ARGS_MAX) {
        p.rc = APK_ERR_ARG;
        snprintf(p.message, sizeof p.message, "msm: a batch of %u exceeds the workspace's %u", in.batch, in.ws_batch);
        return p;
    }
    for (uint32_t b = 0; b < in.batch; b++) {
        if (in.len[b] > in.n_bases || in.offset[b] > in.n_bases - in.len[b]) {
            p.rc = APK_ERR_ARG;
            snprintf(p.message, sizeof p.message, "msm: %u scalars exceed the %u bases", in.len[b], in.n_bases);
            return p;
        }
        if (in.len[b] > p.maxlen) p.maxlen = in.len[b];
        p.entries += (uint64_t)in.len[b] * x.W;
    }
    const uint64_t entries = p.entries;
    const uint32_t maxlen = p.maxlen, total_buckets = p.total_buckets = in.batch * x.NB;
    uint32_t unit = k.unit;
    if (!unit) {
        const uint64_t lanes_wanted = (uint64_t)in.simds * 64 * 8;
        const uint64_t by_size = entries / lanes_wanted;
        if (by_size >= 24) {
            unit = by_size > (uint64_t)MSM_UNIT_MAX ? (uint32_t)MSM_UNIT_MAX : (uint32_t)by_size;
        } else {
            uint64_t best = ~0ull;
            for (uint32_t u = MSM_UNIT; u <= MSM_UNIT + 2; u++) {
// ... 35 lines not shown
        return p;
    }
    if (sort2) { p.paths |= MSM_PATH_SORT2; if (k.sort2 < 0 && in.n_bases < 65536u) p.paths |= MSM_PATH_SORT2_LOAD; }
    if (p.lean) p.paths |= MSM_PATH_LEAN_TAIL;
    if (sort2) {
        const uint32_t per_slice = cdiv(maxlen, p.G);
        p.stage_cap = per_slice * (uint32_t)x.W;
        if (p.stage_cap > stage_max) p.stage_cap = stage_max;
        p.tile_cap = (uint32_t)(entries / ((uint64_t)in.batch * P)) + (uint32_t)(entries / ((uint64_t)in.batch * P)) / 7u + 256u;
        if (p.tile_cap > MSM_PART_TILE) p.tile_cap = MSM_PART_TILE;
        const bool fused = k.sort_fused && !k.graph  && p.stage_cap / P >= 64u &&
                           (uint64_t)per_slice * x.W <= stage_max && in.has_ptot2 && (uint64_t)in.ws_batch * P <= (uint64_t)MSM_MAX_BATCH * MSM_PART_MAX &&
                           (uint64_t)in.batch * p.G * (P + 1) <= in.counts_words &&
                           (uint64_t)in.batch * p.G * p.stage_cap * 4 <= in.sort_tmp_bytes;
        p.sort = fused ? MSM_SORT_FUSED : MSM_SORT_FOUR_LAUNCH;
        if (fused) p.paths |= MSM_PATH_SORT_FUSED;
        const uint32_t mean_run = p.stage_cap / P + 1;
        p.run_lanes = 8;
        while (p.run_lanes < 64 && p.run_lanes < mean_run) p.run_lanes <<= 1;
    }
    p.scan_items = msm_scan_items(total_buckets);
    p.scan_nblk = cdiv(total_buckets, (uint64_t)MSM_SCAN_BLOCK * p.scan_items);
    p.per_lane = p.lean && total_buckets >= 32768u ? 32u : 5u;
    {
        const uint64_t upb = (entries / unit) / total_buckets + 1;
        while ((1u << p.lanes_log) < MSM_COMBINE_LANES && (upb >> p.lanes_log) > p.per_lane) p.lanes_log++;
    }
    p.dyn_lanes = k.combine_dyn && !p.lean && in.scan_runs;
    if (p.dyn_lanes) { p.lanes_log += 2; if ((1u << p.lanes_log) > MSM_COMBINE_LANES) p.lanes_log = 4; }
    p.cquad = k.combine_quad >= 0 ? k.combine_quad != 0 : (!p.lean && !k.graph && x.NB <= 4096u);
    if (p.cquad) p.paths |= MSM_PATH_COMBINE_QUAD;
    p.inplace = in.scan_runs && (k.inplace >= 0 ? k.inplace != 0 : (p.lanes_log == 0 && !p.cquad));
    if (p.inplace) p.paths |= MSM_PATH_INPLACE;
    const int m_bits = x.c - 1;
    p.cols_log = (uint32_t)(m_bits - m_bits / 2);
    p.rows = 1u << (m_bits / 2); p.cols = 1u << p.cols_log;
    p.nbits = p.cols_log + 1;
    p.quad = k.quad_tail >= 0 ? k.quad_tail : (in.slots <= 2 ? 7 : 14);
    p.lt = (p.rows > p.cols ? p.rows : p.cols) > in.lt_max ? in.lt_max : (p.rows > p.cols ? p.rows : p.cols);
    if (k.quad_tail < 0 && !k.graph && p.rows % 4 == 0 && p.cols % 4 == 0) p.serial = k.rowcol_serial >= 0 ? k.rowcol_serial != 0 : p.lean;
    if (p.serial) p.paths |= MSM_PATH_ROWCOL_SERIAL;
    p.rowcol_lanes = k.rowcol_lanes == 8 && p.rows % 8 == 0 && p.cols % 8 == 0 ? 8 : 16;
    return p;
}

}
```

algoplonk_amd/csrc/msm_run.h:

```cpp
#pragma once
#include <hip/hip_runtime.h>

#include "backend.h"
#include "dev_buf.h"
#include "kernels_msm.h"
#include "msm_plan.h"

namespace apk {

inline MsmKnobs msm_knobs_from_env() {
    MsmKnobs k;
    k.window = env_int("APK_MSM_WINDOW", 0, 0, 20);
    k.part_target = (uint32_t)env_int("APK_MSM_PART_TARGET", MSM_PART_TILE - 2048, 1024, MSM_PART_TILE - 2048);
    k.part_pblog = env_int("APK_MSM_PART_PBLOG", 0, 0, 8);
    k.graph = env_int("APK_MSM_GRAPH", 0, 0, 1);
    k.unit = (uint32_t)env_int("APK_MSM_UNIT", 0, 0, MSM_UNIT_MAX);
    k.unit_loaded = (uint32_t)env_int("APK_MSM_UNIT_LOADED", 48, 0, MSM_UNIT_MAX);
    k.unit_loaded_bases = (uint32_t)env_int("APK_MSM_UNIT_LOADED_BASES", 65536, 0, 1 << 30);
    k.unit_small = (uint32_t)env_int("APK_MSM_UNIT_SMALL", MSM_UNIT_SMALL, MSM_UNIT_SMALL, MSM_UNIT_MIN);
    k.small_waves = (uint32_t)env_int("APK_MSM_SMALL_WAVES", 2, 1, 4);
    k.slice = (uint32_t)env_int("APK_MSM_SLICE", 2048, 64, 1 << 20);
    k.digits_threads = env_int("APK_MSM_DIGITS_THREADS", MSM_DIGITS_THREADS, 64, MSM_DIGITS_THREADS) & ~63;
    k.lean_tail = env_int("APK_MSM_LEAN_TAIL", -1, -1, 1);
    k.sort2 = env_int("APK_MSM_SORT2", -1, -1, 1);
    k.part_small_scan = env_int("APK_MSM_PART_SMALL_SCAN", 1, 0, 1);
    k.sort_fused = env_int("APK_MSM_SORT_FUSED", 1, 0, 1);
    k.scan_fused = env_int("APK_MSM_SCAN_FUSED", 0, 0, 1);
    k.combine_dyn = env_int("APK_MSM_COMBINE_DYN", 1, 0, 1);
    k.sorted_merge = env_int("APK_MSM_SORTED_MERGE", 1, 0, 1);
    k.combine_quad = env_int("APK_MSM_COMBINE_QUAD", -1, -1, 1);
    k.quad_tail = env_int("APK_MSM_QUAD_TAIL", -1, -1, 15);
    k.rowcol_serial = env_int("APK_MSM_ROWCOL_SERIAL", -1, -1, 1);
    k.rowcol_lanes = env_int("APK_MSM_ROWCOL_LANES", 16, 8, 16);
    k.inplace = env_int("APK_MSM_INPLACE", -1, -1, 1);
    return k;
}
inline const MsmKnobs& msm_knobs() { static const MsmKnobs k = msm_knobs_from_env(); return k; }

struct MsmTables {
    DevBuf table;
    uint32_t n_bases = 0;
    bool built = false;
    bool plain = false;
};

template <class FRP, class FPP>
int build_tables(hipStream_t st, const MsmCtxPlan& x, const Affine<FPP>* d_bases, uint32_t count, MsmTables& T, bool plain = false) {
    using Fr = Fe<FRP>;
    using Aff = Affine<FPP>;
    CHK(T.table.alloc((size_t)count * x.W * sizeof(Aff)));
    T.n_bases = count;
    T.plain = plain;
    MsmPreScale pre{};
#ifndef APK_MSM_NO_RINV
    if (!plain) {
        Fr one_int{};
        one_int.l[0] = 1u;
        const Fr rinv = Fr::from_mont(one_int);
        static_assert(Fr::N <= 16, "MsmPreScale holds 16 words");
        for (int i = 0; i < Fr::N; i++) pre.l[i] = rinv.l[i];
        pre.nwords = Fr::N;
    }
#endif
    msm_table_kernel<FPP><<<cdiv(count, 256), 256, 0, st>>>(d_bases, count, x.win, pre, ptr<Aff>(T.table));
    KCHK();
    T.built = true;
    return APK_OK;
// ... 35 lines not shown
        const uint32_t tb = batch * x.NB;
        const MsmWorkspacePlan w = msm_plan_workspace(x, k, bases, batch, many_slots);
        CHK(hist.alloc((size_t)(tb + 1) * 4)); CHK(offsets.alloc((size_t)(tb + 1) * 4));
        CHK(unit_off.alloc((size_t)(tb + 1) * 4));
        CHK(scan_blk.alloc((size_t)w.scan_blk * 4));
        CHK(merge_rank.alloc((size_t)(tb + 1) * 4)); CHK(merge_list.alloc((size_t)(tb + 1) * 4));
        CHK(full_off.alloc((size_t)(tb + 1) * 4)); CHK(rem_rank.alloc((size_t)(tb + 1) * 4)); CHK(rem_list.alloc((size_t)(tb + 1) * 4));
        CHK(counts.alloc((size_t)w.counts * 4));
        CHK(sorted.alloc(entries * 4));
        if (w.sort_tmp) {
            CHK(sort_tmp.alloc(w.sort_tmp * 4));
            CHK(ptot2.alloc((size_t)2 * MSM_MAX_BATCH * MSM_PART_MAX * 4));
            HIPCHK(hipMemset(ptot2.p, 0, (size_t)2 * MSM_MAX_BATCH * MSM_PART_MAX * 4));
        }
        CHK(partial.alloc(w.partial * sizeof(PtU)));
        CHK(bucket_sum.alloc((size_t)tb * sizeof(PtU)));
        {
            const int m_bits = x.c - 1;
            const uint32_t rows = 1u << (m_bits / 2), cols = 1u << (m_bits - m_bits / 2);
            CHK(rowcol.alloc((size_t)batch * (rows + cols) * sizeof(PtU)));
        }
        CHK(bit_partial.alloc((size_t)batch * 2 * 32 * sizeof(PtU)));
        CHK(result_xyzz.alloc(MSM_ARGS_MAX * sizeof(Pt)));
        CHK(done_count.alloc((MSM_ARGS_MAX + 1) * sizeof(uint32_t)));
        HIPCHK(hipMemset(done_count.p, 0, (MSM_ARGS_MAX + 1) * sizeof(uint32_t)));
        return APK_OK;
    }
};

struct MsmEvents {
    hipEvent_t before = nullptr, scanned = nullptr, accumulated = nullptr, reduced = nullptr;
    hipEvent_t acc = nullptr;
    int mark_acc = 0;
};

#ifdef APK_DEBUG_KNOCKOUT
#define APK_PHASE(bit) ((env_int("APK_DEBUG_SKIP", 0, 0, 127) & (bit)) == 0)
#else
#define APK_PHASE(bit) true
#endif

template <class FRP, class FPP>
int msm_launch_sort(hipStream_t st, const MsmCtxPlan& x, MsmWorkspace<FPP>& ws, uint32_t n_bases, const MsmBatchArgs& a, const MsmBatchPlan& p) {
    const int dth = msm_knobs().digits_threads;
    const dim3 gd(p.G, a.batch);
    if (p.sort == MSM_SORT_ONE_LEVEL) {
        if (!APK_PHASE(1)) return APK_OK;
        const size_t lds = msm_digits_lds_bytes(x.NB);
        if (a.plain) msm_digits_kernel<FRP, false, true><<<gd, dth, lds, st>>>(a, x.win, x.NB, n_bases, p.G, ptr<uint32_t>(ws.counts), nullptr, nullptr);
        else msm_digits_kernel<FRP, false, false><<<gd, dth, lds, st>>>(a, x.win, x.NB, n_bases, p.G, ptr<uint32_t>(ws.counts), nullptr, nullptr);
        KCHK();
        msm_colscan_kernel<0><<<cdiv(p.total_buckets, 256), 256, 0, st>>>(ptr<uint32_t>(ws.counts), x.NB, p.G, p.total_buckets, ptr<uint32_t>(ws.hist));
        KCHK();
        return APK_OK;
    }
    if (!APK_PHASE(1)) return APK_OK;
    const MsmPartCfg& pc = x.part;
    const uint32_t P = pc.P, G = p.G, stage_cap = p.stage_cap, tile_cap = p.tile_cap;
    uint32_t* pcounts = ptr<uint32_t>(ws.counts);
    uint32_t* runstart = pcounts + (size_t)a.batch * G * P;
    uint32_t* ptot = runstart + (size_t)a.batch * G * P;
    uint32_t* csum = ptot + (size_t)a.batch * P;
    const size_t cursors_lds = (size_t)(2 * P + 1) * 4;
    if (p.sort == MSM_SORT_FUSED) {
        uint32_t* pt_cur = ptr<uint32_t>(ws.ptot2) + (size_t)(ws.ptot_parity & 1u) * MSM_MAX_BATCH * MSM_PART_MAX;
        uint32_t* pt_next = ptr<uint32_t>(ws.ptot2) + (size_t)((ws.ptot_parity & 1u) ^ 1u) * MSM_MAX_BATCH * MSM_PART_MAX;
// ... 58 lines not shown
        msm_scan_apply_kernel<PtU><<<cdiv(total_buckets, MSM_SCAN_BLOCK), MSM_SCAN_BLOCK, 0, st>>>(blk_tot, blk_bins, ptr<uint32_t>(ws.hist), ptr<uint32_t>(ws.rem_rank),
                                                                  ptr<uint32_t>(ws.merge_rank), nblk,
                                                                  total_buckets, unit, ptr<uint32_t>(ws.offsets), ptr<uint32_t>(ws.unit_off),
                                                                  ptr<uint32_t>(ws.full_off), ptr<uint32_t>(ws.rem_list), ptr<uint32_t>(ws.merge_list), items,
                                                                  p.inplace ? ptr<PtU>(ws.bucket_sum) : nullptr);
        KCHK();
    }
    if (p.sort == MSM_SORT_ONE_LEVEL && APK_PHASE(64)) {
        const dim3 gd(p.G, a.batch);
        const int dth = msm_knobs().digits_threads;
        const size_t lds = msm_digits_lds_bytes(x.NB);
        if (a.plain) msm_digits_kernel<FRP, true, true><<<gd, dth, lds, st>>>(a, x.win, x.NB, n_bases, p.G, ptr<uint32_t>(ws.counts), ptr<uint32_t>(ws.offsets), ptr<uint32_t>(ws.sorted));
        else msm_digits_kernel<FRP, true, false><<<gd, dth, lds, st>>>(a, x.win, x.NB, n_bases, p.G, ptr<uint32_t>(ws.counts), ptr<uint32_t>(ws.offsets), ptr<uint32_t>(ws.sorted));
        KCHK();
    }
    return APK_OK;
}

template <class FPP>
int msm_launch_accumulate(hipStream_t st, MsmWorkspace<FPP>& ws, const Affine<FPP>* table, const MsmBatchPlan& p, const MsmEvents& ev) {
    using PtU = typename MsmWorkspace<FPP>::PtU;
    const uint32_t total_buckets = p.total_buckets;
    if (APK_PHASE(2))
    msm_accumulate_kernel<FPP><<<cdiv(p.max_units, MsmAcc<FPP>::THREADS), MsmAcc<FPP>::THREADS, 0, st>>>(table, ptr<uint32_t>(ws.sorted), ptr<uint32_t>(ws.offsets),
                                                                    ptr<uint32_t>(ws.unit_off), ptr<uint32_t>(ws.full_off), ptr<uint32_t>(ws.rem_list),
                                                                    total_buckets, p.max_units, p.unit, ptr<PtU>(ws.partial),
                                                                    p.inplace ? ptr<PtU>(ws.bucket_sum) : nullptr);
    KCHK();
    if (ev.accumulated) HIPCHK(hipEventRecord(ev.accumulated, st));
    if (ev.mark_acc == 1 && ev.acc) HIPCHK(hipEventRecord(ev.acc, st));
    if (!APK_PHASE(4)) return APK_OK;
    const uint32_t* avg_partials = p.dyn_lanes ? ptr<uint32_t>(ws.scan_blk) + (size_t)(3 + MSM_BINS) * p.scan_nblk : nullptr;
    const uint32_t* merge_list = msm_knobs().sorted_merge ? ptr<uint32_t>(ws.merge_list) : nullptr;
    if (p.cquad) {
        const uint32_t qblocks = cdiv(((uint64_t)total_buckets << p.lanes_log) * 4, 256);
        msm_combine_quad_kernel<FPP><<<qblocks + MSM_HEAVY_BLOCKS, 256, 0, st>>>(
            ptr<PtU>(ws.partial), ptr<uint32_t>(ws.unit_off), merge_list, total_buckets, p.lanes_log,
            qblocks, ptr<PtU>(ws.bucket_sum), avg_partials, p.per_lane, p.inplace ? 1u : 0u);
    } else {
        const uint32_t normal_blocks = cdiv((uint64_t)total_buckets << p.lanes_log, 256);
        msm_combine_kernel<FPP><<<normal_blocks + MSM_HEAVY_BLOCKS, 256, 0, st>>>(
            ptr<PtU>(ws.partial), ptr<uint32_t>(ws.unit_off), merge_list, total_buckets, p.lanes_log,
            normal_blocks, ptr<PtU>(ws.bucket_sum), avg_partials, p.per_lane, p.inplace ? 1u : 0u);
    }
    KCHK();
    return APK_OK;
}

template <class FPP>
int msm_launch_reduce(hipStream_t st, const MsmCtxPlan& x, MsmWorkspace<FPP>& ws, const MsmBatchArgs& a, const MsmBatchPlan& p, XYZZ<FPP>* res_out) {
    using PtU = typename MsmWorkspace<FPP>::PtU;
    const uint32_t rows = p.rows, cols = p.cols, lt = p.lt, nbits = p.nbits;
    const int quad = p.quad, cols_log = (int)p.cols_log;
    if (!APK_PHASE(8)) {
    } else if (p.serial) {
        if (p.rowcol_lanes == 8)
            msm_rowcol_serial_kernel<FPP, 8><<<dim3((rows + cols + 31) / 32, a.batch), 256, 0, st>>>(ptr<PtU>(ws.bucket_sum), x.NB, rows, cols, ptr<PtU>(ws.rowcol));
        else
            msm_rowcol_serial_kernel<FPP, 16><<<dim3((rows + cols + 15) / 16, a.batch), 256, 0, st>>>(ptr<PtU>(ws.bucket_sum), x.NB, rows, cols, ptr<PtU>(ws.rowcol));
    }
    else if (quad & 1)
        msm_rowcol_quad_kernel<FPP><<<dim3(rows + cols, a.batch), 4 * lt, lt * sizeof(PtU), st>>>(ptr<PtU>(ws.bucket_sum), x.NB, rows, cols, ptr<PtU>(ws.rowcol));
    else if (quad & 8)
        msm_rowcol_hybrid_kernel<FPP><<<dim3(rows + cols, a.batch), 256, 0, st>>>(ptr<PtU>(ws.bucket_sum), x.NB, rows, cols, ptr<PtU>(ws.rowcol));
    else
        msm_rowcol_kernel<FPP><<<dim3(rows + cols, a.batch), 256, 0, st>>>(ptr<PtU>(ws.bucket_sum), x.NB, rows, cols, ptr<PtU>(ws.rowcol));
    KCHK();
// ... 1 lines not shown
    } else if ((quad & 6) == 6) {
        const uint32_t threads = 4 * lt > 256 ? 4 * lt : 256;
        const size_t lds = (size_t)(lt > 64 ? lt : 64) * sizeof(PtU);
        msm_bitsum_final_quad_kernel<FPP><<<dim3(nbits, 2, a.batch), threads, lds, st>>>(
            ptr<PtU>(ws.rowcol), rows, cols, lt, ptr<PtU>(ws.bit_partial), ptr<uint32_t>(ws.done_count), cols_log, res_out);
        KCHK();
    } else {
        if (quad & 2)
            msm_bitsum_quad_kernel<FPP><<<dim3(nbits, 2, a.batch), 4 * lt, lt * sizeof(PtU), st>>>(ptr<PtU>(ws.rowcol), rows, cols, ptr<PtU>(ws.bit_partial));
        else
            msm_bitsum_kernel<FPP><<<dim3(nbits, 2, a.batch), 256, 0, st>>>(ptr<PtU>(ws.rowcol), rows, cols, ptr<PtU>(ws.bit_partial));
        KCHK();
        if (quad & 4)
            msm_final_quad_kernel<FPP><<<a.batch, 256, 0, st>>>(ptr<PtU>(ws.bit_partial), nbits, cols_log, nullptr, res_out);
        else
            msm_final_kernel<FPP><<<a.batch, 64, 0, st>>>(ptr<PtU>(ws.bit_partial), nbits, cols_log, nullptr, res_out);
        KCHK();
    }
    return APK_OK;
}

template <class FRP, class FPP>
int msm_launch_batch(hipStream_t st, const MsmCtxPlan& x, MsmWorkspace<FPP>& ws, const Affine<FPP>* table, uint32_t n_bases, const MsmBatchArgs& a,
                     const MsmBatchPlan& p, XYZZ<FPP>* res_out, const MsmEvents& ev) {
    if (ev.before) HIPCHK(hipEventRecord(ev.before, st));
    if (ev.mark_acc == 2 && ev.acc) HIPCHK(hipEventRecord(ev.acc, st));
    if (p.rc != APK_OK) { set_error("%s", p.message); return p.rc; }
    CHK((msm_launch_sort<FRP>(st, x, ws, n_bases, a, p)));
    CHK((msm_launch_scan<FRP>(st, x, ws, n_bases, a, p)));
    if (ev.scanned) HIPCHK(hipEventRecord(ev.scanned, st));
    CHK(msm_launch_accumulate(st, ws, table, p, ev));
    CHK(msm_launch_reduce(st, x, ws, a, p, res_out));
    if (ev.reduced) HIPCHK(hipEventRecord(ev.reduced, st));
    return APK_OK;
}

}
```

algoplonk_amd/csrc/ntt_run.h:

```cpp
#pragma once
#include <hip/hip_runtime.h>

#include "backend.h"
#include "dev_buf.h"
#include "kernels_ntt.h"
#include "ntt_plan.h"

namespace apk {

inline const NttKnobs& ntt_knobs() {
    static const NttKnobs k = [] {
        NttKnobs e;
        e.tile_log = env_int("APK_NTT_TILE_LOG", 0, 0, NTT_TILE_LOG);
        e.stages = env_int("APK_NTT_STAGES", 0, 0, NTT_TILE_LOG);
        e.radix4 = env_int("APK_NTT_RADIX4", -1, -1, 1);
        e.threads = env_int("APK_NTT_THREADS", 0, 0, NTT_THREADS) & ~63;
        return e;
    }();
    return k;
}

template <class FRP>
int ntt_allow_tile_lds() {
    const int lds = (int)(((size_t)1 << NTT_TILE_LOG) * sizeof(FeU<FRP>));
    HIPCHK(hipFuncSetAttribute(reinterpret_cast<const void*>(&ntt_pass_kernel<FRP, false>), hipFuncAttributeMaxDynamicSharedMemorySize, lds));
    HIPCHK(hipFuncSetAttribute(reinterpret_cast<const void*>(&ntt_pass_kernel<FRP, true>), hipFuncAttributeMaxDynamicSharedMemorySize, lds));
    return APK_OK;
}

template <class FRP>
int ntt_launch(hipStream_t st, const NttPlan& plan, const NttBatch& nb, int count, const Fe<FRP>* tw, bool twu, const Fe<FRP>* pre,
               const Fe<FRP>* post, const Fe<FRP>* scale) {
    const dim3 grid(plan.grid_x, count);
    for (int p = 0; p < plan.passes; p++) {
        if (twu) ntt_pass_kernel<FRP, true><<<grid, plan.threads, plan.lds_bytes, st>>>(nb, tw, pre, post, scale, plan.pass[p]);
        else ntt_pass_kernel<FRP, false><<<grid, plan.threads, plan.lds_bytes, st>>>(nb, tw, pre, post, scale, plan.pass[p]);
        KCHK();
    }
    return APK_OK;
}

}
```

algoplonk_amd/csrc/poly_run.h:

```cpp
#pragma once
#include <hip/hip_runtime.h>
#include <string.h>

#include "dev_buf.h"
#include "gang_kernel.h"
#include "kernels_poly.h"
#include "msm_plan.h"

namespace apk {

struct PlainLaunch {
    template <class K, int BOUNDS, class... P>
    int go(hipStream_t st, dim3 grid, dim3 block, size_t lds, P... p) const {
        poly1_kernel<K, BOUNDS, P...><<<grid, block, lds, st>>>(p...);
        KCHK();
        return APK_OK;
    }
};

static inline uint32_t poly_scan_blocks(uint32_t count) { return cdiv(count, SCAN_BLOCK); }
template <class FRP, class KL>
int poly_scan(const KL& kl, hipStream_t st, Fe<FRP>* data, uint32_t count, bool rev, bool mul_op, Fe<FRP>* tot, Fe<FRP>* out, int shift) {
    using Fr = Fe<FRP>;
    const uint32_t nb = poly_scan_blocks(count);
// ... 64 lines not shown
int poly_gp_terms(const KL& kl, hipStream_t st, const Fe<FRP>* L, const Fe<FRP>* R, const Fe<FRP>* O, const Fe<FRP>* S1, const Fe<FRP>* S2,
                  const Fe<FRP>* S3, const Fe<FRP>* tw, uint32_t n, Fe<FRP> beta32, Fe<FRP> gamma, Fe<FRP> beta_u32, Fe<FRP> beta_u2_32,
                  const GpScan<FRP>& g) {
    return kl.template go<GpTermsK<FRP>, POLY_THREADS>(st, cdiv(n, POLY_THREADS), POLY_THREADS, 0, L, R, O, S1, S2, S3, tw, n, beta32, gamma,
                                                       beta_u32, beta_u2_32, g.data[0], g.data[1]);
}
template <class FRP, class KL>
int poly_gp_scans(const KL& kl, hipStream_t st, const GpScan<FRP>& g, uint32_t n, Fe<FRP>* total_out) {
    const uint32_t nb = poly_scan_blocks(n);
    CHK((kl.template go<GpScanBlockK<FRP>, POLY_THREADS>(st, dim3(nb, 2), POLY_THREADS, 0, g, n)));
    CHK((kl.template go<GpScanTotalsK<FRP>, POLY_THREADS>(st, 2, POLY_THREADS, 0, g, nb, total_out)));
    return APK_OK;
}
template <class FRP, class KL>
int poly_gp_finish(const KL& kl, hipStream_t st, const GpScan<FRP>& g, uint32_t n, const Fe<FRP>& den_total, Fe<FRP>* z) {
    const Fe<FRP> den_total_inv = Fe<FRP>::inv(den_total);
    return kl.template go<GpFinishK<FRP>, POLY_THREADS>(st, cdiv(n, POLY_THREADS), POLY_THREADS, 0, g, n, den_total_inv, z);
}

static inline uint32_t poly_tail_grid(uint32_t count4) { return cdiv(count4, 256 * 8) < 512 ? cdiv(count4, 256 * 8) : 512; }
template <class KL>
int poly_tail_nonzero(const KL& kl, hipStream_t st, const uint4* words, uint32_t count4, uint32_t epoch, uint32_t* flag) {
    return kl.template go<TailNonzeroK<0>, 256>(st, poly_tail_grid(count4), 256, 0, words, count4, epoch, flag);
}

static inline const char* poly_op_check(int op, const apk_poly_args* a) {
    if (!a) return "null argument block";
    constexpr uint64_t CAP = 1ull << 26;
    auto in = [&](int i, uint64_t len) { return a->vec[i] && a->len[i] == len; };
    auto out = [&](int i, uint64_t len) { return a->out[i] && a->out_len[i] == len; };
    auto pow2 = [](int64_t v) { return v >= 2 && v <= (int64_t)CAP && (v & (v - 1)) == 0; };
    auto flag = [&](int i) { return a->iv[i] == 0 || a->iv[i] == 1; };
    const int64_t* iv = a->iv;
    static constexpr int places[] = {7, 1, 25, 2, 2 * EVAL_MAX + 1, LC_MAX, 3, 3, 1, 6, 1, 6};
    if (op < 0 || op >= (int)(sizeof places / sizeof places[0])) return "unknown polynomial-stage op";
    for (int i = places[op]; i < APK_POLY_VECS; i++) if (a->vec[i]) return "a vector outside the op's layout must be null";
    switch (op) {
        case APK_POLY_GRAND_PRODUCT: {
            if (!pow2(iv[0])) return "grand product: n must be a power of two, 2 .. 2^26";
            const uint64_t n = (uint64_t)iv[0];
            for (int i = 0; i < 6; i++) if (!in(i, n)) return "grand product: L, R, O, S1, S2, S3 take n elements each";
            if (!in(6, n / 2)) return "grand product: the twiddle table takes n / 2 elements";
            if (!out(0, n) || !out(1, n) || !out(2, n)) return "grand product: num, den and Z take n elements each";
            return nullptr;
        }
        case APK_POLY_SCAN: {
            if (a->len[0] == 0 || a->len[0] > CAP) return "scan: 1 .. 2^26 elements";
            if (!in(0, a->len[0]) || !out(0, a->len[0])) return "scan: data and out take the same number of elements";
            if (!flag(0) || !flag(1) || !flag(2)) return "scan: op, rev and shift are 0 or 1";
            if (iv[1] && iv[2]) return "scan: shift is for forward scans only";
            return nullptr;
        }
        case APK_POLY_QUOTIENT: {
            if (iv[4] < 0 || iv[4] > 3) return "quotient: sub_glog > 3";
            if (iv[0] < 4 || (uint64_t)iv[0] > CAP >> iv[4]) return "quotient: 4 .. 2^26 points";
            if (iv[1] < 0 || iv[1] > 2) return "quotient: nb_commit > 2";
            if (iv[2] < 0 || iv[2] > QK_INJECT_MAX) return "quotient: nb_inject > QK_INJECT_MAX";
            if (iv[3] < 0 || iv[3] >= (1 << iv[4])) return "quotient: sub_k outside the 2^sub_glog classes";
            const uint64_t m = (uint64_t)iv[0], full = m << iv[4];
            for (int i = 0; i < 4; i++) if (!in(i, m)) return "quotient: l, r, o, z take n4 elements each";
            if (iv[4] == 3 ? !in(4, m) : a->vec[4] != nullptr) return "quotient: zs takes n4 elements with eight classes and is null otherwise";
            for (int k = 0; k < 2; k++)
                if (k < iv[1] ? !in(5 + k, m) || !in(17 + k, full) : (a->vec[5 + k] || a->vec[17 + k])) return "quotient: pi2 (n4) and qcp (the whole coset) per commitment, null beyond";
            for (int i = 7; i <= 16; i++) if (!in(i, full)) return "quotient: the per-circuit tables take the whole coset (n4 << sub_glog)";
            for (int j = 0; j < QK_INJECT_MAX; j++)
                if (j < iv[2] ? !in(19 + j, full) : a->vec[19 + j] != nullptr) return "quotient: one whole-coset table per injection, null beyond";
            if (!out(0, m)) return "quotient: out takes n4 elements";
// ... 39 lines not shown
            if (!flag(1)) return "kzg quotient: z_is_zero is 0 or 1";
            if (!in(0, len) || (iv[1] ? (a->vec[1] || a->vec[2]) : (!in(1, len) || !in(2, len))) || !out(0, len - 1))
                return "kzg quotient: f takes len elements, q len - 1, pw and pwi len each or null for z = 0";
            return nullptr;
        }
        case APK_POLY_KZG_QUOTIENT2: {
            for (int p = 0; p < 2; p++) {
                if (iv[p] < 2 || (uint64_t)iv[p] > CAP) return "kzg quotient pair: 2 .. 2^26 coefficients each";
                const uint64_t len = (uint64_t)iv[p];
                if (!in(3 * p, len) || !in(3 * p + 1, len) || !in(3 * p + 2, len) || !out(p, len - 1))
                    return "kzg quotient pair: f, pw and pwi take len elements each, q len - 1, per polynomial";
            }
            return nullptr;
        }
        case APK_POLY_BLIND: {
            if (iv[0] < 3 || (uint64_t)iv[0] > CAP || iv[1] < 1 || iv[1] > 3) return "blind: n 3 .. 2^26, d 1 .. 3";
            const uint64_t cap = (uint64_t)(iv[0] + iv[1]);
            if (!in(0, cap) || !out(0, cap)) return "blind: p and out take n + d elements";
            return nullptr;
        }
        case APK_POLY_BLIND3: {
            if (iv[0] < 3 || (uint64_t)iv[0] > CAP || iv[1] < 1 || iv[1] > 3) return "blind3: n 3 .. 2^26, d 1 .. 3";
            const uint64_t cap = (uint64_t)(iv[0] + iv[1]);
            for (int i = 0; i < 6; i++)
                if (a->vec[i] ? (!in(i, cap) || !out(i, cap)) : a->out[i] != nullptr) return "blind3: p and lag take n + d elements each, with an out each, or are null";
            return nullptr;
        }
        case APK_POLY_TAIL: {
            if (a->len[0] == 0 || a->len[0] > CAP) return "tail: 1 .. 2^26 records of 16 bytes";
            if (!in(0, a->len[0]) || !out(0, 1)) return "tail: the records and one flag word";
            if (iv[0] < 0 || iv[0] > 0xffffffffll || iv[1] < 0 || iv[1] > 0xffffffffll) return "tail: epoch and flag are 32-bit words";
            return nullptr;
        }
        default: return "unknown polynomial-stage op";
    }
}

}
```

algoplonk_amd/csrc/seam_run.h:

```cpp
#pragma once
#include <hip/hip_runtime.h>
#include <string.h>

#include "backend.h"
#include "dev_buf.h"
#include "kernels_poly.h"
#include "poly_run.h"
#include "selftest_ops.h"
#include "setup_run.h"

namespace apk {

template <class P>
__global__ void __launch_bounds__(256) fe_op_kernel(int op, uint32_t count, const Fe<P>* __restrict__ a, const Fe<P>* __restrict__ b,
                                                    Fe<P>* __restrict__ out) {
    const uint32_t i = blockIdx.x * blockDim.x + threadIdx.x;
    if (i < count) (void)fe_op_t<P>(op, a + i, b + i, out + i);
}
template <class P>
__global__ void __launch_bounds__(256) feu_op_kernel(int op, uint32_t count, const uint32_t* __restrict__ in, uint32_t* __restrict__ out) {
    constexpr int L = FeU<P>::L;
    const uint32_t i = blockIdx.x * blockDim.x + threadIdx.x;
    if (i < count) (void)feu_op_t<P>(op, in + (size_t)i * 4 * L, out + (size_t)i * L);
}
template <class FRP, class FPP>
__global__ void __launch_bounds__(256) g1_op_kernel(int op, uint32_t count, const Affine<FPP>* __restrict__ p, const uint8_t* __restrict__ q,
                                                    uint32_t q_bytes, Affine<FPP>* __restrict__ out) {
    const uint32_t t = blockIdx.x * blockDim.x + threadIdx.x;
    if (op >= 20) {
        const uint32_t i = t >> 2;
        if (i < count) (void)g1_quad_op_t<FRP, FPP>(op, (int)(t & 3u), p + i, q ? q + (size_t)i * q_bytes : nullptr, out + t);
    } else if (t < count) {
        (void)g1_op_t<FRP, FPP>(op, p + t, q ? q + (size_t)t * q_bytes : nullptr, out + t);
    }
}

template <class P>
int fe_op_device_t(int op, uint64_t count, const void* a, const void* b, void* out) {
    using F = Fe<P>;
// ... 156 lines not shown
                const uint32_t l0 = u(0), l1 = u(1);
                CHK(mk(res[0], l0)); CHK(mk(res[1], l1)); CHK(mk(scratch[0], (size_t)l0 + l1)); CHK(mk(scratch[1], poly_scan_blocks(l0) + poly_scan_blocks(l1)));
                for (int p = 0; p < 2; p++) {
                    b.f[p] = v(3 * p); b.pw[p] = v(3 * p + 1); b.pwi[p] = v(3 * p + 2); b.len[p] = u(p); b.q[p] = ptr<Fr>(res[p]);
                    b.tmp[p] = ptr<Fr>(scratch[0]) + (p ? l0 : 0); b.tot[p] = ptr<Fr>(scratch[1]) + (p ? poly_scan_blocks(l0) : 0);
                }
                CHK(poly_kzg_quotient_batch<FRP>(kl, st, b, 2));
                CHK(down(0, res[0].p));
                return down(1, res[1].p);
            }
            case APK_POLY_BLIND: {
                Fr4<FRP> b{};
                for (int i = 0; i < 3; i++) b.v[i] = c(i);
                CHK((kl.template go<BlindK<FRP>, 256>(st, 1, 64, 0, v(0), u(0), b, (int)u(1))));
                return down(0, v(0));
            }
            case APK_POLY_BLIND3: {
                Blind3<FRP> b3{};
                for (int j = 0; j < 3; j++) {
                    b3.p[j] = v(j); b3.lag[j] = v(3 + j);
                    for (int i = 0; i < 4; i++) b3.b[j].v[i] = c(4 * j + i);
                }
                CHK((kl.template go<Blind3K<FRP>, 256>(st, 3, 64, 0, b3, u(0), (int)u(1))));
                for (int i = 0; i < 6; i++) if (a.out[i]) CHK(down(i, v(i)));
                return APK_OK;
            }
            case APK_POLY_TAIL: {
                const uint32_t flag0 = u(1);
                CHK(scratch[0].alloc(16));
                HIPCHK(hipMemcpy(scratch[0].p, &flag0, 4, hipMemcpyHostToDevice));
                CHK(poly_tail_nonzero(kl, st, reinterpret_cast<const uint4*>(in[0].p), (uint32_t)a.len[0], u(0), ptr<uint32_t>(scratch[0])));
                return down(0, scratch[0].p, 4);
            }
        }
        set_error("unknown polynomial-stage op %d", op);
        return APK_ERR_ARG;
    }
};
template <class FRP, class FPP>
int poly_op_device_impl(int device, int op, const apk_poly_args* args) {
    CHK(pick_device(device));
    PolySeam<FRP> seam(*args);
    return seam.run(op);
}

}
```

algoplonk_amd/plonk.py:

```python
from __future__ import annotations

import ctypes as C
import os
from dataclasses import dataclass, field
from typing import List, Optional, Sequence

from . import ecc, frontend
from . import _lib
from ._lib import lib, check
from .setup import SRS


@dataclass
class VerifyingKey:
    curve: ecc.ID
    Size: int
    SizeInv: int
    Generator: int
    CosetShift: int
    NbPublicVariables: int
    Ql: ecc.Point
    Qr: ecc.Point
    Qm: ecc.Point
    Qo: ecc.Point
# ... 52 lines not shown
        try:
            self.close()
        except Exception:
            pass

    def msm(self, scalars: Sequence[int], basis: int = 0) -> ecc.Point:
        cv = self.curve
        buf = cv.fr_vector(scalars)
        out = C.create_string_buffer(2 * cv.fp_bytes)
        check(lib.apk_msm_g1(self.ctx, basis, buf, len(scalars), out))
        return cv.g1_from_bytes(out.raw)

    def ntt(self, values: Sequence[int], which: int = 0, inverse: bool = False, coset: bool = False) -> List[int]:
        cv = self.curve
        buf = C.create_string_buffer(cv.fr_vector(values), len(values) * 32)
        check(lib.apk_ntt(self.ctx, which, int(inverse), int(coset), buf))
        return cv.fr_vector_decode(buf.raw)

    def stats(self, reset: bool = False) -> "_lib.Stats":
        st = _lib.Stats()
        check(lib.apk_stats_read(self.ctx, C.byref(st), int(reset)))
        return st

    def enable_stats(self, on: bool = True) -> None:
        check(lib.apk_stats_enable(self.ctx, int(on)))

    @property
    def msm_window(self) -> int:
        return lib.apk_ctx_msm_window(self.ctx)

    def paths(self, reset: bool = False) -> dict:
        pc = _lib.PathCounts()
        check(lib.apk_paths_read(self.ctx, C.byref(pc), int(reset)))
        return pc.as_dict()


@dataclass
class Proof:
    curve: ecc.ID
    raw: "_lib.Proof"

    def _pt(self, slot) -> ecc.Point:
        return self.curve.g1_from_bytes(bytes(slot))

    def _fr(self, slot) -> int:
        return self.curve.fr_from_mont_bytes(bytes(slot))

    @property
    def LRO(self): return [self._pt(self.raw.lro[i]) for i in range(3)]
    @property
    def Z(self): return self._pt(self.raw.z)
    @property
    def H(self): return [self._pt(self.raw.h[i]) for i in range(3)]
    @property
    def Bsb22Commitments(self): return [self._pt(self.raw.bsb22[i]) for i in range(self.raw.nb_commitments)]
    @property
    def BatchedProofH(self): return self._pt(self.raw.batched_h)
    @property
    def ClaimedValues(self): return [self._fr(self.raw.claimed_values[i]) for i in range(6 + self.raw.nb_commitments)]
    @property
    def ZShiftedOpeningH(self): return self._pt(self.raw.zshift_h)
    @property
    def ZShiftedOpeningClaimedValue(self): return self._fr(self.raw.zshift_value)
    @property
    def challenges(self): return {k: self._fr(getattr(self.raw, k)) for k in ("gamma", "beta", "alpha", "zeta", "gamma_kzg")}


# ... 233 lines not shown
```

include/apk.h:

```cpp
#ifndef APK_H
#define APK_H

#include <stddef.h>
#include <stdint.h>

#ifdef __cplusplus
extern "C" {
#endif

#define APK_ABI_VERSION 5

#define APK_BN254 0
#define APK_BLS12_381 1

#define APK_OK 0
#define APK_ERR_ARG 1
#define APK_ERR_HIP 2
#define APK_ERR_STATE 3
#define APK_ERR_WITNESS 4
#define APK_ERR_VERIFY 5

#define APK_FR_BYTES 32
#define APK_G1_MAX_BYTES 96
#define APK_G2_MAX_BYTES 192
// ... 229 lines not shown
int apk_g2_decompress(int curve, const uint8_t* compressed, void* out);
int apk_g2_mul_generator(int curve, const void* scalar_fr, void* out);

int apk_g1_mul_batch(int curve, int device, const void* base, const void* scalars, uint64_t count, void* out);

int apk_g1_decompress(int curve, int device, const uint8_t* compressed, uint64_t count, void* out);
int apk_g1_to_lagrange(int curve, int device, const void* points, uint64_t n, void* out);

int apk_marshal_proof(const apk_proof* proof, uint8_t* out, size_t cap, size_t* len);
int apk_marshal_public_inputs(int curve, const void* public_inputs, uint32_t nb_public, uint8_t* out, size_t cap);
int apk_fe_from_be(int curve, int field, const uint8_t* be, void* out);
int apk_fe_to_be(int curve, int field, const void* in, uint8_t* be);
int apk_hash_fr(int curve, const void* g1_affine, void* out_fr);

int apk_host_fe_op(int curve, int field, int op, const void* a, const void* b, void* out);
int apk_host_g1_op(int curve, int op, const void* p, const void* q, void* out);
int apk_device_fe_op(int curve, int field, int op, int device, uint64_t count, const void* a, const void* b, void* out);
int apk_device_g1_op(int curve, int op, int device, uint64_t count, const void* p, const void* q, void* out);
int apk_host_feu_op(int curve, int field, int op, uint64_t count, const void* in, void* out);
int apk_device_feu_op(int curve, int field, int op, int device, uint64_t count, const void* in, void* out);
int apk_feu_shape(int curve, int field, int* ul, int* ub, uint32_t* headroom);
#define APK_POLY_GRAND_PRODUCT 0
#define APK_POLY_SCAN 1
#define APK_POLY_QUOTIENT 2
#define APK_POLY_MERGE 3
#define APK_POLY_EVAL 4
#define APK_POLY_LINCOMB 5
#define APK_POLY_DERIVE_POWERS 6
#define APK_POLY_KZG_QUOTIENT 7
#define APK_POLY_BLIND 8
#define APK_POLY_BLIND3 9
#define APK_POLY_TAIL 10
#define APK_POLY_KZG_QUOTIENT2 11
#define APK_POLY_VECS 32
#define APK_POLY_FRS 24
#define APK_POLY_INTS 8
#define APK_POLY_OUTS 6
typedef struct {
    const void* vec[APK_POLY_VECS];
    uint64_t len[APK_POLY_VECS];
    uint8_t fr[APK_POLY_FRS][32];
    int64_t iv[APK_POLY_INTS];
    void* out[APK_POLY_OUTS];
    uint64_t out_len[APK_POLY_OUTS];
} apk_poly_args;
int apk_device_poly_op(int curve, int op, int device, const apk_poly_args* args);
int apk_g1_sum(int curve, const void* points, uint64_t count, void* out);

int apk_host_alloc(int device, size_t bytes, void** ptr);
int apk_host_free(void* ptr);
int apk_host_register(void* ptr, size_t bytes);
int apk_host_unregister(void* ptr);

int apk_device_alloc(apk_ctx* ctx, size_t bytes, void** d_ptr);
int apk_device_free(apk_ctx* ctx, void* d_ptr);
int apk_device_upload(apk_ctx* ctx, void* d_dst, const void* src, size_t bytes);
int apk_device_download(apk_ctx* ctx, void* dst, const void* d_src, size_t bytes);
int apk_device_copy(apk_ctx* ctx, void* d_dst, const void* d_src, size_t bytes);

typedef struct {
    double msm_accumulate_ms;
    uint64_t msm_accumulate_launches;
    uint64_t msm_pairs;
    double msm_total_ms;
    uint64_t msm_batches;
    double ntt_ms;
// ... 5 lines not shown
    double msm_sort_ms;
    double msm_tail_ms;
} apk_stats;
int apk_stats_enable(apk_ctx* ctx, int enable);
int apk_stats_read(apk_ctx* ctx, apk_stats* out, int reset);

typedef struct {
    uint64_t proofs;
    uint64_t msm_batches;
    uint64_t msm_sort_two_level;
    uint64_t msm_sort_two_level_by_load;
    uint64_t msm_sort_fused;
    uint64_t msm_lean_tail;
    uint64_t msm_rowcol_serial;
    uint64_t msm_combine_quad;
    uint64_t msm_small_units;
    uint64_t msm_one_launch;
    uint64_t msm_lagrange_wires;
    uint64_t ntt_sequences;
    uint64_t ntt_radix4;
    uint64_t ntt_radix4_by_load;
    uint64_t tail_fill_proofs;
    uint64_t host_lincomb_pooled;
    uint64_t msm_units_by_load;
    uint64_t host_inputs;
    uint64_t gang_proofs;
    uint64_t gang_msm_launches;
    uint64_t gang_ntt_launches;
    uint64_t gang_kernel_launches;
    uint64_t forms_by_device_load;
    uint64_t msm_inplace;
} apk_path_counts;
int apk_paths_read(apk_ctx* ctx, apk_path_counts* out, int reset);

typedef struct {
    uint32_t contexts;
    uint32_t max_streams;
    uint32_t streams_in_use, streams_peak;
    uint32_t proofs_in_flight, proofs_peak;
    uint32_t waiting;
    uint32_t device_wide;
} apk_device_sched;
int apk_device_sched_read(int device, apk_device_sched* out, int reset);

#define APK_HWQ_UNSET (-1)
#define APK_HWQ_UNREADABLE (-2)
typedef struct {
    int32_t hw_queues_found;
    int32_t hw_queues_left;
    int32_t hw_queues_need;
    int32_t hw_queues_written;
    int32_t hw_queues_now;
    int32_t first_hip_call;
    int32_t hw_queues_at_first_hip;
    int32_t reserved;
} apk_runtime;
int apk_runtime_read(apk_runtime* out);

#ifdef __cplusplus
}
#endif
#endif
```

Before: 556.0.

## Fuse tail check into NTT last pass, add thin MSM merge and early sums

Adds three separate mechanisms. The first folds the blinding-tail nonzero check into the last NTT pass through a new tail kernel, removing a separate pass over the data. The second adds a thin combine kernel for the MSM bucket merge. The third records an event right after the MSM batch finishes so the host can read the sums without waiting for the whole stream. It also adds path counters and a test op, and the extra conditions add complexity and a risk of ordering bugs.

New measurement: 559.9, median of 4. Within noise of the previous version (+0.7%).

```diff
diff --git a/algoplonk_amd/_lib.py b/algoplonk_amd/_lib.py
--- a/algoplonk_amd/_lib.py
+++ b/algoplonk_amd/_lib.py
@@ -24,7 +24,7 @@
     "apk_device_fe_op", "apk_device_g1_op", "apk_host_feu_op", "apk_device_feu_op", "apk_feu_shape", "apk_device_poly_op",
     "apk_device_alloc", "apk_device_free", "apk_device_upload", "apk_device_download",
     "apk_host_alloc", "apk_host_free", "apk_host_register", "apk_host_unregister",
-    "apk_stats_enable", "apk_stats_read", "apk_paths_read",
+    "apk_stats_enable", "apk_stats_read", "apk_paths_read", "apk_paths_more_read",
     "apk_ctx_set_wire_hook", "apk_coset_ntt_device",
     "apk_comm_create", "apk_comm_destroy", "apk_comm_rank", "apk_comm_world", "apk_comm_barrier", "apk_comm_max_f64", "apk_comm_bind",
     "apk_comm_transport", "apk_msm_g1_sharded", "apk_comm_split_begin", "apk_comm_split_end", "apk_comm_serve", "apk_comm_set_compute",
@@ -136,6 +136,14 @@
 
     def as_dict(self) -> dict:
         return {n: int(getattr(self, n)) for n in self._names + self._later}
+
+
+class PathCountsMore(C.Structure):
+    _names = ["msm_thin_merge", "tail_in_ntt", "early_sums"]
+    _fields_ = [(n, C.c_uint64) for n in _names] + [("reserved", C.c_uint64 * 5)]
+
+    def as_dict(self) -> dict:
+        return {n: int(getattr(self, n)) for n in self._names}
 
 
 class DeviceSched(C.Structure):
@@ -254,6 +262,8 @@
     lib.apk_stats_enable.argtypes = [vp, i32]
     lib.apk_stats_read.argtypes = [vp, C.POINTER(Stats), i32]
     lib.apk_paths_read.argtypes = [vp, C.POINTER(PathCounts), i32]
+    if hasattr(lib, "apk_paths_more_read"):
+        lib.apk_paths_more_read.argtypes = [vp, C.POINTER(PathCountsMore), i32]
     if hasattr(lib, "apk_device_sched_read"):
         lib.apk_device_sched_read.argtypes = [i32, C.POINTER(DeviceSched), i32]
     if hasattr(lib, "apk_runtime_read"):
diff --git a/algoplonk_amd/csrc/apk_api.cpp b/algoplonk_amd/csrc/apk_api.cpp
--- a/algoplonk_amd/csrc/apk_api.cpp
+++ b/algoplonk_amd/csrc/apk_api.cpp
@@ -548,6 +548,7 @@
     return APK_OK;
 }
 int apk_paths_read(apk_ctx* ctx, apk_path_counts* out, int reset) { NEED_CTX(); if (!out) { set_error("null out"); return APK_ERR_ARG; } return ctx->be->paths_read(out, reset); }
+int apk_paths_more_read(apk_ctx* ctx, apk_path_counts_more* out, int reset) { NEED_CTX(); if (!out) { set_error("null out"); return APK_ERR_ARG; } return ctx->be->paths_more_read(out, reset); }
 int apk_runtime_read(apk_runtime* out) {
     if (!out) { set_error("null out"); return APK_ERR_ARG; }
     memset(out, 0, sizeof *out);
diff --git a/algoplonk_amd/csrc/backend.h b/algoplonk_amd/csrc/backend.h
--- a/algoplonk_amd/csrc/backend.h
+++ b/algoplonk_amd/csrc/backend.h
@@ -56,6 +56,7 @@
     virtual int stats_enable(int enable) = 0;
     virtual int stats_read(apk_stats* out, int reset) = 0;
     virtual int paths_read(apk_path_counts* out, int reset) = 0;
+    virtual int paths_more_read(apk_path_counts_more* out, int reset) = 0;
 };
 
 int g1_mul_batch_bn254(int device, const void* base, const void* scalars, uint64_t count, void* out);
diff --git a/algoplonk_amd/csrc/backend_impl.h b/algoplonk_amd/csrc/backend_impl.h
--- a/algoplonk_amd/csrc/backend_impl.h
+++ b/algoplonk_amd/csrc/backend_impl.h
@@ -59,6 +59,8 @@
         int open_pair = env_int("APK_OPEN_PAIR", 1, 0, 1);
         int lin_early_h = env_int("APK_LIN_EARLY_H", 1, 0, 1);
         int tail_fill = env_int("APK_TAIL_FILL", 1, 0, 2);
+        int tail_in_ntt = env_int("APK_TAIL_IN_NTT", 1, 0, 1);
+        int early_sums = env_int("APK_EARLY_SUMS", -1, -1, 1);
     };
     static const ProverKnobs& prover_knobs() { static const ProverKnobs k{}; return k; }
 
@@ -107,6 +109,9 @@
         hipStream_t side = nullptr;
         hipEvent_t ev_acc = nullptr, ev_side = nullptr;
         hipEvent_t ev_sync = nullptr;
+        hipEvent_t ev_batch = nullptr;
+        bool early_next = false;
+        bool batch_marked = false;
         int mark_acc = 0; bool side_pending = false;
     };
 
@@ -181,8 +186,9 @@
         bool on() const { return G > 1 && hook; }
     } sc_;
     enum PathIdx { P_PROOFS, P_MSM_BATCHES, P_SORT2, P_SORT2_LOAD, P_SORT_FUSED, P_LEAN_TAIL, P_ROWCOL_SERIAL, P_COMBINE_QUAD, P_SMALL_UNITS,
-                   P_ONE_LAUNCH, P_LAGRANGE_WIRES, P_NTT_SEQ, P_NTT_R4, P_NTT_R4_LOAD, P_TAIL_FILL, P_LINCOMB_POOL, P_UNIT_LOADED, P_HOST_INPUTS, P_GANG_PROOFS, P_GANG_MSM, P_GANG_NTT, P_GANG_KERNELS, P_DEVICE_LOAD, P_MSM_INPLACE, P_COUNT };
-    std::atomic<uint64_t> paths_[P_COUNT] = {};
+                   P_ONE_LAUNCH, P_LAGRANGE_WIRES, P_NTT_SEQ, P_NTT_R4, P_NTT_R4_LOAD, P_TAIL_FILL, P_LINCOMB_POOL, P_UNIT_LOADED, P_HOST_INPUTS, P_GANG_PROOFS, P_GANG_MSM, P_GANG_NTT, P_GANG_KERNELS, P_DEVICE_LOAD, P_MSM_INPLACE, P_COUNT,
+                   P_MSM_THIN_MERGE = P_COUNT, P_TAIL_IN_NTT, P_EARLY_SUMS, P_COUNT_ALL };
+    std::atomic<uint64_t> paths_[P_COUNT_ALL] = {};
     void path(PathIdx i) { paths_[i].fetch_add(1, std::memory_order_relaxed); }
     bool device_load_over(int thr, bool* foreign = nullptr) {
         int own = 0;
@@ -195,6 +201,13 @@
         memset(out, 0, sizeof *out);
         uint64_t* o = reinterpret_cast<uint64_t*>(out);
         for (int i = 0; i < P_COUNT; i++) o[i] = reset ? paths_[i].exchange(0, std::memory_order_relaxed) : paths_[i].load(std::memory_order_relaxed);
+        return APK_OK;
+    }
+    int paths_more_read(apk_path_counts_more* out, int reset) override {
+        static_assert(sizeof(apk_path_counts_more) >= (P_COUNT_ALL - P_COUNT) * sizeof(uint64_t), "apk_path_counts_more holds every later counter");
+        memset(out, 0, sizeof *out);
+        uint64_t* o = reinterpret_cast<uint64_t*>(out);
+        for (int i = P_COUNT; i < P_COUNT_ALL; i++) o[i - P_COUNT] = reset ? paths_[i].exchange(0, std::memory_order_relaxed) : paths_[i].load(std::memory_order_relaxed);
         return APK_OK;
     }
     bool stats_on_ = false;
@@ -223,18 +236,20 @@
             if (s->ev_acc) (void)hipEventDestroy(s->ev_acc);
             if (s->ev_side) (void)hipEventDestroy(s->ev_side);
             if (s->ev_sync) (void)hipEventDestroy(s->ev_sync);
+            if (s->ev_batch) (void)hipEventDestroy(s->ev_batch);
             delete s;
         }
         if (owns_streams_) for (hipStream_t st : stream_pool_) if (st) (void)hipStreamDestroy(st);
     }
 
     int run_ntt_batch(hipStream_t st, int which, bool inverse, int count, const Fr* const* ins, Fr* const* outs, const uint32_t* in_lens,
-                      uint32_t out_len, const Fr* pre, const Fr* post, const Fr* scale, int sub_log = 0, bool semi = false) {
+                      uint32_t out_len, const Fr* pre, const Fr* post, const Fr* scale, int sub_log = 0, bool semi = false,
+                      const NttTail* tails = nullptr ) {
         Slot* m = gang_member();
         if (m && m->in_gang && st == m->stream && count <= NTT_MAX_BATCH) {
             NttReq<Fr> nr{};
             nr.which = which; nr.inverse = inverse; nr.count = count;
-            for (int i = 0; i < count; i++) { nr.ins[i] = ins[i]; nr.outs[i] = outs[i]; nr.in_lens[i] = in_lens[i]; }
+            for (int i = 0; i < count; i++) { nr.ins[i] = ins[i]; nr.outs[i] = outs[i]; nr.in_lens[i] = in_lens[i]; if (tails) nr.tails[i] = tails[i]; }
             nr.out_len = out_len; nr.pre = pre; nr.post = post; nr.scale = scale; nr.sub_log = sub_log; nr.semi = semi;
             GangReq r;
             r.kind = GANG_KIND_NTT; r.args = &nr; r.member = m;
@@ -242,14 +257,15 @@
             if (rc != APK_OK) set_error("%s", r.err.c_str());
             return rc;
         }
-        return run_ntt_batch_now(st, which, inverse, count, ins, outs, in_lens, out_len, pre, post, scale, sub_log, semi);
+        return run_ntt_batch_now(st, which, inverse, count, ins, outs, in_lens, out_len, pre, post, scale, sub_log, semi, tails);
     }
     const Fr* ntt_table(int which, bool inverse) const {
         if (ntt_twu_) return which ? (inverse ? ptr<Fr>(twi_4n_x_) : ptr<Fr>(tw_4n_x_)) : (inverse ? ptr<Fr>(twi_n_x_) : ptr<Fr>(twu_n_x_));
         return which ? (inverse ? ptr<Fr>(twi_4n_) : ptr<Fr>(tw_4n_)) : (inverse ? ptr<Fr>(twi_n_) : ptr<Fr>(twu_n_));
     }
     int run_ntt_batch_now(hipStream_t st, int which, bool inverse, int count, const Fr* const* ins, Fr* const* outs, const uint32_t* in_lens,
-                          uint32_t out_len, const Fr* pre, const Fr* post, const Fr* scale, int sub_log = 0, bool semi = false) {
+                          uint32_t out_len, const Fr* pre, const Fr* post, const Fr* scale, int sub_log = 0, bool semi = false,
+                          const NttTail* tails = nullptr) {
         const int log_n = (which ? (int)log_n_ + 2 : (int)log_n_) - sub_log;
         Slot* owner = nullptr;
         for (Slot* s : slots_) if (s->own_stream == st || (s->side && s->side == st)) owner = s;
@@ -260,12 +276,15 @@
         if (plan.rc != APK_OK) { set_error("%s", plan.message); return plan.rc; }
         NttBatch nb{};
         for (int i = 0; i < count; i++) { nb.in[i] = ins[i]; nb.out[i] = outs[i]; nb.in_len[i] = in_lens[i]; }
+        NttTails nt{};
+        bool any_tail = false;
+        if (tails) for (int i = 0; i < count; i++) { nt.t[i] = tails[i]; any_tail |= tails[i].flag != nullptr; }
         if (plan.needs_wide) for (int i = 0; i < count; i++) nb.wide[i] = ptr<FeU<FRP>>(owner->ntt_wide) + ((size_t)i << log_n);
         static constexpr PathIdx PATH_OF_BIT[] = {P_NTT_SEQ, P_NTT_R4, P_NTT_R4_LOAD, P_DEVICE_LOAD};
         for (uint32_t i = 0; i < sizeof PATH_OF_BIT / sizeof PATH_OF_BIT[0]; i++) if (plan.paths >> i & 1u) path(PATH_OF_BIT[i]);
         Slot* timed = stats_on_ ? owner : nullptr;
         if (timed) HIPCHK(hipEventRecord(timed->ev2, st));
-        CHK(ntt_launch<FRP>(st, plan, nb, count, ntt_table(which, inverse), ntt_twu_, pre, post, scale));
+        CHK(ntt_launch<FRP>(st, plan, nb, count, ntt_table(which, inverse), ntt_twu_, pre, post, scale, any_tail ? &nt : nullptr));
         if (timed) {
             HIPCHK(hipEventRecord(timed->ev3, st));
             HIPCHK(hipEventSynchronize(timed->ev3));
@@ -278,8 +297,8 @@
         return APK_OK;
     }
     int run_ntt(hipStream_t st, int which, bool inverse, const Fr* in, Fr* out, uint32_t in_len, uint32_t out_len,
-                const Fr* pre, const Fr* post, const Fr* scale, int sub_log = 0, bool semi = false) {
-        return run_ntt_batch(st, which, inverse, 1, &in, &out, &in_len, out_len, pre, post, scale, sub_log, semi);
+                const Fr* pre, const Fr* post, const Fr* scale, int sub_log = 0, bool semi = false, const NttTail* tail = nullptr) {
+        return run_ntt_batch(st, which, inverse, 1, &in, &out, &in_len, out_len, pre, post, scale, sub_log, semi, tail);
     }
     int coset_eval(hipStream_t st, int count, const Fr* const* ins, const uint32_t* lens, Fr* const* outs, int cls = 0) {
         if (!sc_.on()) return run_ntt_batch(st, 1, false, count, ins, outs, lens, n4_, ptr<Fr>(coset_pre_), nullptr, nullptr, 0, true);
@@ -370,7 +389,7 @@
         in.counts_words = s.msm.counts.bytes / 4; in.sort_tmp_bytes = s.msm.sort_tmp.bytes;
         in.has_sort_tmp = s.msm.sort_tmp.p != nullptr; in.has_ptot2 = s.msm.ptot2.p != nullptr;
         const MsmBatchPlan p = msm_plan_batch(msm_ctx_, msm_knobs(), in);
-        static constexpr PathIdx PATH_OF_BIT[] = {P_UNIT_LOADED, P_SMALL_UNITS, P_SORT2, P_SORT2_LOAD, P_SORT_FUSED, P_LEAN_TAIL, P_COMBINE_QUAD, P_ROWCOL_SERIAL, P_DEVICE_LOAD, P_MSM_INPLACE};
+        static constexpr PathIdx PATH_OF_BIT[] = {P_UNIT_LOADED, P_SMALL_UNITS, P_SORT2, P_SORT2_LOAD, P_SORT_FUSED, P_LEAN_TAIL, P_COMBINE_QUAD, P_ROWCOL_SERIAL, P_DEVICE_LOAD, P_MSM_INPLACE, P_MSM_THIN_MERGE};
         for (uint32_t i = 0; i < sizeof PATH_OF_BIT / sizeof PATH_OF_BIT[0]; i++) if (p.paths >> i & 1u) path(PATH_OF_BIT[i]);
         if (p.rc == APK_ERR_ARG) { set_error("%s", p.message); return p.rc; }
         if (p.rc == APK_OK) {
@@ -381,6 +400,7 @@
         MsmEvents ev;
         if (stats_on_) { ev.before = s.ev0; ev.scanned = s.ev2; ev.accumulated = s.ev3; ev.reduced = s.ev1; }
         ev.acc = s.ev_acc; ev.mark_acc = s.mark_acc;
+        if (s.early_next && s.ev_batch && s.d_pinned && p.rc == APK_OK) { ev.done = s.ev_batch; s.batch_marked = true; }
         CHK((msm_launch_batch<FRP, FPP>(st, msm_ctx_, s.msm, ptr<Aff>(T.table), T.n_bases, a, p, res_out, ev)));
         if (!s.d_pinned) HIPCHK(hipMemcpyAsync(pin_host<Pt>(s.h_pinned, PIN_XYZZ) + s.res_write_off, s.msm.result_xyzz.p, a.batch * sizeof(Pt), hipMemcpyDeviceToHost, st));
         s.pending_pts = a.batch;
@@ -439,14 +459,14 @@
     int side_begin(Slot& s) { HIPCHK(hipStreamWaitEvent(s.side, s.ev_acc, 0)); return APK_OK; }
     int side_end(Slot& s) { HIPCHK(hipEventRecord(s.ev_side, s.side)); s.side_pending = true; return APK_OK; }
 
-    int wait_stream(Slot& s) {
+    int wait_stream(Slot& s, hipEvent_t behind = nullptr) {
         static const int mode = env_int("APK_SYNC_BLOCKING", -1, -1, 2);
         static const int poll_us = env_int("APK_SYNC_POLL_US", 50, 1, 10000);
         const bool loaded = slots_.size() > 2 && device_load_over(2);
         if (s.ev_sync && (mode == 2 || (mode < 0 && loaded))) {
-            HIPCHK(hipEventRecord(s.ev_sync, s.stream));
+            if (!behind) HIPCHK(hipEventRecord(s.ev_sync, s.stream));
             for (;;) {
-                const hipError_t e = hipEventQuery(s.ev_sync);
+                const hipError_t e = hipEventQuery(behind ? behind : s.ev_sync);
                 if (e == hipSuccess) return APK_OK;
                 if (e != hipErrorNotReady) { (void)hipGetLastError(); set_error("hipEventQuery: %s", hipGetErrorString(e)); return APK_ERR_HIP; }
                 struct timespec ts = {0, (long)poll_us * 1000L};
@@ -454,22 +474,32 @@
             }
         }
         if (mode == 1 && s.ev_sync) {
-            HIPCHK(hipEventRecord(s.ev_sync, s.stream));
-            HIPCHK(hipEventSynchronize(s.ev_sync));
+            if (!behind) HIPCHK(hipEventRecord(s.ev_sync, s.stream));
+            HIPCHK(hipEventSynchronize(behind ? behind : s.ev_sync));
             return APK_OK;
         }
-        HIPCHK(hipStreamSynchronize(s.stream));
-        return APK_OK;
-    }
-
-    int sync_results(Slot& s) {
+        if (behind) HIPCHK(hipEventSynchronize(behind));
+        else HIPCHK(hipStreamSynchronize(s.stream));
+        return APK_OK;
+    }
+    bool early_sums_ok(const Slot& s, bool measuring, int fill) {
+        const int k = prover_knobs().early_sums;
+        if (!k || !s.ev_batch || !s.d_pinned || s.in_gang || hook_ || wire_hook_ || stats_on_ || sc_.on() || fill || measuring || msm_knobs().graph) return false;
+        return k > 0 || (slots_.size() > 2 && device_load_over(2));
+    }
+
+    int sync_results(Slot& s, bool early = false) {
         if (s.in_gang) {
             GangReq r;
             r.kind = GANG_KIND_FLUSH; r.member = &s;
             const int rc = s.lead->gang.meet(s.gang_idx, r, gang_launcher_);
             if (rc != APK_OK) { set_error("%s", r.err.c_str()); return rc; }
         }
-        CHK(wait_stream(s));
+        const bool marked = s.batch_marked;
+        s.batch_marked = false;
+        const bool behind_batch = early && marked && !s.in_gang && !s.hook_pending;
+        CHK(wait_stream(s, behind_batch ? s.ev_batch : nullptr));
+        if (behind_batch) path(P_EARLY_SUMS);
         if (s.side_pending) { s.side_pending = false; HIPCHK(hipStreamWaitEvent(s.stream, s.ev_side, 0)); }
         if (s.hook_pending) {
             s.hook_pending = false;
@@ -498,6 +528,7 @@
         HIPCHK(hipEventCreate(&s.ev2));
         HIPCHK(hipEventCreate(&s.ev3));
         if (hipEventCreateWithFlags(&s.ev_sync, hipEventBlockingSync | hipEventDisableTiming) != hipSuccess) { (void)hipGetLastError(); s.ev_sync = nullptr; }
+        if (hipEventCreateWithFlags(&s.ev_batch, hipEventDisableTiming) != hipSuccess) { (void)hipGetLastError(); s.ev_batch = nullptr; }
         HIPCHK(hipHostMalloc(&s.h_pinned, PIN_BYTES, hipHostMallocDefault));
         memset(s.h_pinned, 0, PIN_BYTES);
         static const int zero_copy = env_int("APK_ZERO_COPY", 1, 0, 1);
@@ -677,12 +708,16 @@
                 for (int k = 0; k < g.n; k++) member_of(reqs[g.req[k]]).pending_pts = rc == APK_OK ? msm_of(reqs[g.req[k]]).a.batch : 0;
             } else {
                 const Fr* ins[NTT_ARGS_MAX]; Fr* outs[NTT_ARGS_MAX]; uint32_t lens[NTT_ARGS_MAX];
+                NttTail tails[NTT_ARGS_MAX];
                 for (int k = 0; k < g.n; k++) {
                     const NttReq<Fr>& m = ntt_of(reqs[g.req[k]]);
-                    for (int t = 0; t < m.count; t++) { ins[g.first[k] + t] = m.ins[t]; outs[g.first[k] + t] = m.outs[t]; lens[g.first[k] + t] = m.in_lens[t]; }
+                    for (int t = 0; t < m.count; t++) {
+                        ins[g.first[k] + t] = m.ins[t]; outs[g.first[k] + t] = m.outs[t]; lens[g.first[k] + t] = m.in_lens[t];
+                        tails[g.first[k] + t] = m.tails[t];
+                    }
                 }
                 const NttReq<Fr>& f = ntt_of(reqs[g.req[0]]);
-                rc = run_ntt_batch_now(lead.own_stream, f.which, f.inverse, (int)g.total, ins, outs, lens, f.out_len, f.pre, f.post, f.scale, f.sub_log, f.semi);
+                rc = run_ntt_batch_now(lead.own_stream, f.which, f.inverse, (int)g.total, ins, outs, lens, f.out_len, f.pre, f.post, f.scale, f.sub_log, f.semi, tails);
                 if (g.n > 1) path(P_GANG_NTT);
             }
             for (int k = 0; k < g.n; k++) { reqs[g.req[k]]->rc = rc; if (rc != APK_OK) reqs[g.req[k]]->err = apk_last_error(); }
@@ -1741,8 +1776,9 @@
         a.plain = use_lag ? 1u : 0u;
         if (use_lag) path(P_LAGRANGE_WIRES);
         s.mark_acc = fill;
+        s.early_next = early_sums_ok(s, run.measuring, fill);
         const int rc = use_lag ? commit(s, tab_lag_, 1, a) : commit(s, tab_can_, 0, a);
-        s.mark_acc = 0;
+        s.mark_acc = 0; s.early_next = false;
         CHK(rc);
     }
     if (!qk_direct_) {
@@ -1772,7 +1808,7 @@
             CHK(coset_eval(st, 3, canon, lens, ev));
         }
     }
-    CHK(sync_results(s));
+    CHK(sync_results(s, true));
     if (run.measuring) wire_route_finish(run);
     for (int j = 0; j < 3; j++) { run.lro[j] = hp[j]; store_pt(run.out->lro[j], run.lro[j]); }
     return APK_OK;
@@ -1804,8 +1840,9 @@
         MsmBatchArgs a{};
         a.batch = 1; a.scalars[0] = s.cz.p; a.len[0] = n + 3; a.offset[0] = 0;
         s.mark_acc = fill;
+        s.early_next = early_sums_ok(s, false, fill);
         const int rc = commit(s, tab_can_, 0, a);
-        s.mark_acc = 0;
+        s.mark_acc = 0; s.early_next = false;
         CHK(rc);
     }
     if (fill) {
@@ -1821,7 +1858,7 @@
             CHK(coset_eval(st, 1, &cin, &zl, &e2, 1));
         }
     }
-    CHK(sync_results(s));
+    CHK(sync_results(s, true));
     run.zcom = pin_host<Aff>(s.h_pinned, PIN_AFF)[0];
     store_pt(run.out->z, run.zcom);
     return APK_OK;
@@ -1862,9 +1899,15 @@
     const uint32_t n = n_;
     {
         QuotientArgs<FRP> q = quotient_args(run);
+        s.epoch++;
+        uint32_t* const flag_pin = pin_dev<uint32_t>(s.d_pinned, PIN_TAIL);
+        uint32_t* const flag = flag_pin ? flag_pin : ptr<uint32_t>(s.tail_flag);
+        const bool tail_in_ntt = prover_knobs().tail_in_ntt && !sc_.on() && !hook_ && !wire_hook_;
         if (!sc_.on()) {
             CHK((klaunch<QuotientK<FRP>, POLY_THREADS>(st, cdiv(n4_, POLY_THREADS), POLY_THREADS, 0, q, ptr<Fr>(s.quot))));
-            CHK(run_ntt(st, 1, true, ptr<Fr>(s.quot), ptr<Fr>(s.hcan), n4_, n4_, nullptr, ptr<Fr>(coset_post_inv_), nullptr));
+            const NttTail tail{flag, 3 * (n + 2), s.epoch};
+            if (tail_in_ntt) path(P_TAIL_IN_NTT);
+            CHK(run_ntt(st, 1, true, ptr<Fr>(s.quot), ptr<Fr>(s.hcan), n4_, n4_, nullptr, ptr<Fr>(coset_post_inv_), nullptr, 0, false, tail_in_ntt ? &tail : nullptr));
         } else {
             const uint32_t m = n4_ >> sc_.glog;
             q.n4 = m; q.sub_k = (uint32_t)sc_.k; q.sub_glog = (uint32_t)sc_.glog; q.zs = ptr<Fr>(s.eqk);
@@ -1885,11 +1928,10 @@
         a.batch = 3;
         for (int j = 0; j < 3; j++) { a.scalars[j] = ptr<Fr>(s.hcan) + (size_t)j * (n + 2); a.len[j] = n + 2; a.offset[j] = 0; }
         CHK(commit(s, tab_can_, 0, a));
-        s.epoch++;
-        const uint32_t tail4 = (n4_ - 3 * (n + 2)) * (uint32_t)(sizeof(Fr) / 16);
-        uint32_t* const flag_pin = pin_dev<uint32_t>(s.d_pinned, PIN_TAIL);
-        CHK(poly_tail_nonzero(kl(), st, reinterpret_cast<const uint4*>(ptr<Fr>(s.hcan) + 3 * (size_t)(n + 2)), tail4, s.epoch,
-                              flag_pin ? flag_pin : ptr<uint32_t>(s.tail_flag)));
+        if (!tail_in_ntt) {
+            const uint32_t tail4 = (n4_ - 3 * (n + 2)) * (uint32_t)(sizeof(Fr) / 16);
+            CHK(poly_tail_nonzero(kl(), st, reinterpret_cast<const uint4*>(ptr<Fr>(s.hcan) + 3 * (size_t)(n + 2)), tail4, s.epoch, flag));
+        }
         if (!flag_pin) HIPCHK(hipMemcpyAsync(pin_host<uint32_t>(s.h_pinned, PIN_TAIL), s.tail_flag.p, 4, hipMemcpyDeviceToHost, st));
     }
     CHK(sync_results(s));
diff --git a/algoplonk_amd/csrc/gang_run.h b/algoplonk_amd/csrc/gang_run.h
--- a/algoplonk_amd/csrc/gang_run.h
+++ b/algoplonk_amd/csrc/gang_run.h
@@ -8,6 +8,7 @@
 #include "gang_plan.h"
 #include "msm_run.h"
 #include "ntt_plan.h"
+#include "kernels_ntt.h"
 
 namespace apk {
 
@@ -80,6 +81,7 @@
     int which; bool inverse; int count;
     const Fr* ins[NTT_MAX_BATCH]; Fr* outs[NTT_MAX_BATCH]; uint32_t in_lens[NTT_MAX_BATCH];
     uint32_t out_len; const Fr *pre, *post, *scale; int sub_log; bool semi;
+    NttTail tails[NTT_MAX_BATCH];
     GangPlanReq plan_req() const { return GangPlanReq{GANG_KIND_NTT, (uint32_t)count, nullptr, GangNttShape{which, inverse, out_len, pre, post, scale, sub_log, semi}}; }
 };
 
diff --git a/algoplonk_amd/csrc/kernels_msm.h b/algoplonk_amd/csrc/kernels_msm.h
--- a/algoplonk_amd/csrc/kernels_msm.h
+++ b/algoplonk_amd/csrc/kernels_msm.h
@@ -708,6 +708,9 @@
         offsets[total] = s_cnt[t]; unit_off[total] = s_unit[t]; full_off[total] = s_full[t];
         const uint32_t nonempty = total - L.s_bintot[MSM_UNIT_MAX];
         block_bins[nblocks * MSM_BINS] = nonempty ? s_unit[t] / nonempty : 0u;
+        uint32_t multi = 0;
+        for (uint32_t r = MSM_UNIT_MAX + 2; r < (uint32_t)MSM_BINS; r++) multi += L.s_bintot[r];
+        block_bins[nblocks * MSM_BINS + 1] = multi;
     }
     if (t < MSM_BINS) {
         uint32_t run = 0;
@@ -989,6 +992,57 @@
     }
 }
 
+template <class FP>
+__global__ void __launch_bounds__(256) msm_combine_thin_kernel(const XYZZ<FP, FeU<FP>>* __restrict__ partial, const uint32_t* __restrict__ unit_off,
+                                                               const uint32_t* __restrict__ merge_list, const uint32_t* __restrict__ merge_count,
+                                                               XYZZ<FP, FeU<FP>>* __restrict__ bucket_sum, uint32_t per_lane) {
+    wave_priority<APK_PRIO_TAIL>();
+    using PT = XYZZ<FP, FeU<FP>>;
+    const uint32_t count = *merge_count;
+    if (count == 0) return;
+    __shared__ PT sm[4];
+    __shared__ unsigned long long s_heavy[4];
+    const uint32_t heavy = msm_heavy_threshold(0, per_lane);
+    const uint32_t t = threadIdx.x, G = gridDim.x, lane = t & 63u, wave = t >> 6;
+    for (uint32_t base = 0; base < count; base += 256u * G) {
+        const uint32_t i = base + t * G + blockIdx.x;
+        uint32_t k = 0, beg = 0, end = 0;
+        if (i < count) { k = merge_list[i]; beg = unit_off[k]; end = unit_off[k + 1]; }
+        const bool is_heavy = end - beg > heavy;
+        if (i < count && !is_heavy) {
+            PT acc = PT::inf();
+            for (uint32_t u = beg; u < end; u++) acc.add_lazy(partial[u]);
+            bucket_sum[k] = acc;
+        }
+        const unsigned long long mine = __ballot(is_heavy);
+        if (!__syncthreads_or(is_heavy)) continue;
+        if (lane == 0) s_heavy[wave] = mine;
+        __syncthreads();
+        for (uint32_t w = 0; w < 4; w++) {
+            unsigned long long m = s_heavy[w];
+            while (m) {
+                const uint32_t l = (uint32_t)__ffsll(m) - 1u;
+                m &= m - 1;
+                const uint32_t kh = merge_list[base + (w * 64u + l) * G + blockIdx.x];
+                const uint32_t hbeg = unit_off[kh], hend = unit_off[kh + 1];
+                PT acc = PT::inf();
+                for (uint32_t u = hbeg + t; u < hend; u += 256) acc.add_lazy(partial[u]);
+                for (int d = 32; d >= 1; d >>= 1) {
+                    PT o = shfl_down_point<PT>(acc, d, 64);
+                    if (lane < (uint32_t)d) acc.add_lazy(o);
+                }
+                if (lane == 0) sm[wave] = acc;
+                __syncthreads();
+                if (t == 0) {
+                    for (uint32_t v = 1; v < 4; v++) { PT o = sm[v]; acc.add_lazy(o); }
+                    bucket_sum[kh] = acc;
+                }
+                __syncthreads();
+            }
+        }
+    }
+}
+
 
 template <class FP>
 __global__ void __launch_bounds__(256) msm_rowcol_kernel(const XYZZ<FP, FeU<FP>>* __restrict__ bucket_sum, uint32_t nb, uint32_t rows,
diff --git a/algoplonk_amd/csrc/kernels_ntt.h b/algoplonk_amd/csrc/kernels_ntt.h
--- a/algoplonk_amd/csrc/kernels_ntt.h
+++ b/algoplonk_amd/csrc/kernels_ntt.h
@@ -7,19 +7,24 @@
 
 __device__ __forceinline__ uint32_t bitrev32(uint32_t x, int bits) { return __brev(x) >> (32 - bits); }
 
+struct NttTail {
+    uint32_t* flag;
+    uint32_t first, epoch;
+};
 struct NttBatch {
     const void* in[NTT_ARGS_MAX];
     void* out[NTT_ARGS_MAX];
     uint32_t in_len[NTT_ARGS_MAX];
     void* wide[NTT_ARGS_MAX];
 };
-
-template <class FR, bool TWU = false>
-__global__ void __launch_bounds__(NTT_THREADS) ntt_pass_kernel(NttBatch nb, const Fe<FR>* __restrict__ tw,
-                                                               const Fe<FR>* __restrict__ pre,
-                                                               const Fe<FR>* __restrict__ post,
-                                                               const Fe<FR>* __restrict__ scale,
-                                                               NttPassArgs a) {
+struct NttTails {
+    NttTail t[NTT_ARGS_MAX];
+};
+
+template <class FR, bool TWU, bool TAIL>
+__device__ __forceinline__ void ntt_pass_body(const NttBatch& nb, const Fe<FR>* __restrict__ tw, const Fe<FR>* __restrict__ pre,
+                                              const Fe<FR>* __restrict__ post, const Fe<FR>* __restrict__ scale, const NttPassArgs& a,
+                                              const NttTail& tail) {
     wave_priority<APK_PRIO_FR>();
     using Fr = Fe<FR>;
     using Fu = FeU<FR>;
@@ -139,6 +144,8 @@
         }
         __syncthreads();
     }
+    const bool check_tail = TAIL && a.last && tail.flag && (post || scale || !a.semi);
+    uint32_t tail_bits = 0;
     for (uint32_t e = threadIdx.x; e < tile_elems; e += NT) {
         uint32_t c = e & (C - 1), mid = e >> clog;
         uint32_t g = g0 + c;
@@ -153,7 +160,30 @@
         Fr o;
         v.pack(o.l);
         out[idx] = o;
-    }
+        if constexpr (TAIL) {
+            if (check_tail && idx >= tail.first) {
+#pragma unroll
+                for (int w = 0; w < Fr::N; w++) tail_bits |= o.l[w];
+            }
+        }
+    }
+    if constexpr (TAIL) {
+        if (check_tail && __ballot(tail_bits != 0) != 0 && (threadIdx.x & 63) == 0) *reinterpret_cast<volatile uint32_t*>(tail.flag) = tail.epoch;
+    }
+}
+template <class FR, bool TWU = false>
+__global__ void __launch_bounds__(NTT_THREADS) ntt_pass_kernel(NttBatch nb, const Fe<FR>* __restrict__ tw,
+                                                               const Fe<FR>* __restrict__ pre,
+                                                               const Fe<FR>* __restrict__ post,
+                                                               const Fe<FR>* __restrict__ scale,
+                                                               NttPassArgs a) {
+    ntt_pass_body<FR, TWU, false>(nb, tw, pre, post, scale, a, NttTail{});
+}
+template <class FR, bool TWU = false>
+__global__ void __launch_bounds__(NTT_THREADS) ntt_pass_tail_kernel(NttBatch nb, const Fe<FR>* __restrict__ tw, const Fe<FR>* __restrict__ pre,
+                                                                    const Fe<FR>* __restrict__ post, const Fe<FR>* __restrict__ scale, NttPassArgs a,
+                                                                    NttTails tails) {
+    ntt_pass_body<FR, TWU, true>(nb, tw, pre, post, scale, a, tails.t[blockIdx.y]);
 }
 
 template <class FR>
diff --git a/algoplonk_amd/csrc/msm_plan.h b/algoplonk_amd/csrc/msm_plan.h
--- a/algoplonk_amd/csrc/msm_plan.h
+++ b/algoplonk_amd/csrc/msm_plan.h
@@ -73,7 +73,10 @@
     int rowcol_serial = -1;
     int rowcol_lanes = 16;
     int inplace = -1;
-};
+    int thin_merge = -1;
+    uint32_t thin_grid = 0;
+};
+inline uint32_t msm_thin_merge_grid(uint32_t simds) { return simds / 16u < 16u ? 16u : simds / 16u; }
 
 struct MsmCtxPlan {
     int rc = APK_OK;
@@ -200,7 +203,7 @@
 enum MsmPathBit : uint32_t {
     MSM_PATH_UNIT_LOADED = 1u << 0, MSM_PATH_SMALL_UNITS = 1u << 1, MSM_PATH_SORT2 = 1u << 2, MSM_PATH_SORT2_LOAD = 1u << 3, MSM_PATH_SORT_FUSED = 1u << 4,
     MSM_PATH_LEAN_TAIL = 1u << 5, MSM_PATH_COMBINE_QUAD = 1u << 6, MSM_PATH_ROWCOL_SERIAL = 1u << 7, MSM_PATH_DEVICE_LOAD = 1u << 8,
-    MSM_PATH_INPLACE = 1u << 9
+    MSM_PATH_INPLACE = 1u << 9, MSM_PATH_THIN_MERGE = 1u << 10
 };
 struct MsmBatchIn {
     uint32_t batch;
@@ -233,6 +236,8 @@
     int lanes_log = 0;
     bool dyn_lanes = false, cquad = false;
     bool inplace = false;
+    bool thin = false;
+    uint32_t merge_grid = 0;
     int quad = 0;
     bool serial = false;
     int rowcol_lanes = 16;
@@ -334,6 +339,8 @@
     if (p.cquad) p.paths |= MSM_PATH_COMBINE_QUAD;
     p.inplace = in.scan_runs && (k.inplace >= 0 ? k.inplace != 0 : (p.lanes_log == 0 && !p.cquad));
     if (p.inplace) p.paths |= MSM_PATH_INPLACE;
+    p.thin = p.inplace && !p.cquad && k.sorted_merge && (k.thin_merge >= 0 ? k.thin_merge != 0 : (p.lanes_log == 0 && !p.dyn_lanes));
+    if (p.thin) { p.merge_grid = k.thin_grid ? k.thin_grid : msm_thin_merge_grid(in.simds); p.paths |= MSM_PATH_THIN_MERGE; }
     const int m_bits = x.c - 1;
     p.cols_log = (uint32_t)(m_bits - m_bits / 2);
     p.rows = 1u << (m_bits / 2); p.cols = 1u << p.cols_log;
diff --git a/algoplonk_amd/csrc/msm_run.h b/algoplonk_amd/csrc/msm_run.h
--- a/algoplonk_amd/csrc/msm_run.h
+++ b/algoplonk_amd/csrc/msm_run.h
@@ -33,6 +33,8 @@
     k.rowcol_serial = env_int("APK_MSM_ROWCOL_SERIAL", -1, -1, 1);
     k.rowcol_lanes = env_int("APK_MSM_ROWCOL_LANES", 16, 8, 16);
     k.inplace = env_int("APK_MSM_INPLACE", -1, -1, 1);
+    k.thin_merge = env_int("APK_MSM_THIN_MERGE", -1, -1, 1);
+    k.thin_grid = (uint32_t)env_int("APK_MSM_THIN_GRID", 0, 0, 1024);
     return k;
 }
 inline const MsmKnobs& msm_knobs() { static const MsmKnobs k = msm_knobs_from_env(); return k; }
@@ -134,6 +136,7 @@
     hipEvent_t before = nullptr, scanned = nullptr, accumulated = nullptr, reduced = nullptr;
     hipEvent_t acc = nullptr;
     int mark_acc = 0;
+    hipEvent_t done = nullptr;
 };
 
 #ifdef APK_DEBUG_KNOCKOUT
@@ -258,7 +261,11 @@
     if (!APK_PHASE(4)) return APK_OK;
     const uint32_t* avg_partials = p.dyn_lanes ? ptr<uint32_t>(ws.scan_blk) + (size_t)(3 + MSM_BINS) * p.scan_nblk : nullptr;
     const uint32_t* merge_list = msm_knobs().sorted_merge ? ptr<uint32_t>(ws.merge_list) : nullptr;
-    if (p.cquad) {
+    if (p.thin) {
+        const uint32_t* merge_count = ptr<uint32_t>(ws.scan_blk) + (size_t)(3 + MSM_BINS) * p.scan_nblk + 1;
+        msm_combine_thin_kernel<FPP><<<p.merge_grid, 256, 0, st>>>(ptr<PtU>(ws.partial), ptr<uint32_t>(ws.unit_off), ptr<uint32_t>(ws.merge_list), merge_count,
+                                                                   ptr<PtU>(ws.bucket_sum), p.per_lane);
+    } else if (p.cquad) {
         const uint32_t qblocks = cdiv(((uint64_t)total_buckets << p.lanes_log) * 4, 256);
         msm_combine_quad_kernel<FPP><<<qblocks + MSM_HEAVY_BLOCKS, 256, 0, st>>>(
             ptr<PtU>(ws.partial), ptr<uint32_t>(ws.unit_off), merge_list, total_buckets, p.lanes_log,
@@ -326,7 +333,8 @@
     CHK(msm_launch_accumulate(st, ws, table, p, ev));
     CHK(msm_launch_reduce(st, x, ws, a, p, res_out));
     if (ev.reduced) HIPCHK(hipEventRecord(ev.reduced, st));
-    return APK_OK;
-}
-
-}
+    if (ev.done) HIPCHK(hipEventRecord(ev.done, st));
+    return APK_OK;
+}
+
+}
diff --git a/algoplonk_amd/csrc/ntt_run.h b/algoplonk_amd/csrc/ntt_run.h
--- a/algoplonk_amd/csrc/ntt_run.h
+++ b/algoplonk_amd/csrc/ntt_run.h
@@ -25,15 +25,21 @@
     const int lds = (int)(((size_t)1 << NTT_TILE_LOG) * sizeof(FeU<FRP>));
     HIPCHK(hipFuncSetAttribute(reinterpret_cast<const void*>(&ntt_pass_kernel<FRP, false>), hipFuncAttributeMaxDynamicSharedMemorySize, lds));
     HIPCHK(hipFuncSetAttribute(reinterpret_cast<const void*>(&ntt_pass_kernel<FRP, true>), hipFuncAttributeMaxDynamicSharedMemorySize, lds));
+    HIPCHK(hipFuncSetAttribute(reinterpret_cast<const void*>(&ntt_pass_tail_kernel<FRP, false>), hipFuncAttributeMaxDynamicSharedMemorySize, lds));
+    HIPCHK(hipFuncSetAttribute(reinterpret_cast<const void*>(&ntt_pass_tail_kernel<FRP, true>), hipFuncAttributeMaxDynamicSharedMemorySize, lds));
     return APK_OK;
 }
 
 template <class FRP>
 int ntt_launch(hipStream_t st, const NttPlan& plan, const NttBatch& nb, int count, const Fe<FRP>* tw, bool twu, const Fe<FRP>* pre,
-               const Fe<FRP>* post, const Fe<FRP>* scale) {
+               const Fe<FRP>* post, const Fe<FRP>* scale, const NttTails* tails = nullptr) {
     const dim3 grid(plan.grid_x, count);
     for (int p = 0; p < plan.passes; p++) {
-        if (twu) ntt_pass_kernel<FRP, true><<<grid, plan.threads, plan.lds_bytes, st>>>(nb, tw, pre, post, scale, plan.pass[p]);
+        if (tails && plan.pass[p].last) {
+            if (twu) ntt_pass_tail_kernel<FRP, true><<<grid, plan.threads, plan.lds_bytes, st>>>(nb, tw, pre, post, scale, plan.pass[p], *tails);
+            else ntt_pass_tail_kernel<FRP, false><<<grid, plan.threads, plan.lds_bytes, st>>>(nb, tw, pre, post, scale, plan.pass[p], *tails);
+        }
+        else if (twu) ntt_pass_kernel<FRP, true><<<grid, plan.threads, plan.lds_bytes, st>>>(nb, tw, pre, post, scale, plan.pass[p]);
         else ntt_pass_kernel<FRP, false><<<grid, plan.threads, plan.lds_bytes, st>>>(nb, tw, pre, post, scale, plan.pass[p]);
         KCHK();
     }
diff --git a/algoplonk_amd/csrc/poly_run.h b/algoplonk_amd/csrc/poly_run.h
--- a/algoplonk_amd/csrc/poly_run.h
+++ b/algoplonk_amd/csrc/poly_run.h
@@ -120,7 +120,7 @@
     auto pow2 = [](int64_t v) { return v >= 2 && v <= (int64_t)CAP && (v & (v - 1)) == 0; };
     auto flag = [&](int i) { return a->iv[i] == 0 || a->iv[i] == 1; };
     const int64_t* iv = a->iv;
-    static constexpr int places[] = {7, 1, 25, 2, 2 * EVAL_MAX + 1, LC_MAX, 3, 3, 1, 6, 1, 6};
+    static constexpr int places[] = {7, 1, 25, 2, 2 * EVAL_MAX + 1, LC_MAX, 3, 3, 1, 6, 1, 6, 4};
     if (op < 0 || op >= (int)(sizeof places / sizeof places[0])) return "unknown polynomial-stage op";
     for (int i = places[op]; i < APK_POLY_VECS; i++) if (a->vec[i]) return "a vector outside the op's layout must be null";
     switch (op) {
@@ -226,6 +226,15 @@
             if (iv[0] < 0 || iv[0] > 0xffffffffll || iv[1] < 0 || iv[1] > 0xffffffffll) return "tail: epoch and flag are 32-bit words";
             return nullptr;
         }
+        case APK_POLY_NTT_TAIL: {
+            if (iv[0] < 1 || iv[0] > 20) return "ntt tail: log2 N 1 .. 20";
+            const uint64_t N = 1ull << iv[0];
+            if (!in(0, N) || !in(2, N / 2) || !out(0, N) || !out(2, 1)) return "ntt tail: N evaluations, N / 2 twiddles, N outputs and one 32-byte record of flag words";
+            if (a->vec[1] ? (!in(1, N) || !out(1, N)) : a->out[1] != nullptr) return "ntt tail: the second transform takes N evaluations and N outputs, or neither";
+            if (a->vec[3] && !in(3, N)) return "ntt tail: the post table takes N elements";
+            for (int i = 1; i <= 6; i++) if (iv[i] < 0 || iv[i] > 0xffffffffll) return "ntt tail: first, epoch and flag are 32-bit words";
+            return nullptr;
+        }
         default: return "unknown polynomial-stage op";
     }
 }
diff --git a/algoplonk_amd/csrc/seam_run.h b/algoplonk_amd/csrc/seam_run.h
--- a/algoplonk_amd/csrc/seam_run.h
+++ b/algoplonk_amd/csrc/seam_run.h
@@ -5,6 +5,7 @@
 #include "backend.h"
 #include "dev_buf.h"
 #include "kernels_poly.h"
+#include "ntt_run.h"
 #include "poly_run.h"
 #include "selftest_ops.h"
 #include "setup_run.h"
@@ -227,6 +228,28 @@
                 CHK(poly_tail_nonzero(kl, st, reinterpret_cast<const uint4*>(in[0].p), (uint32_t)a.len[0], u(0), ptr<uint32_t>(scratch[0])));
                 return down(0, scratch[0].p, 4);
             }
+            case APK_POLY_NTT_TAIL: {
+                const int log_n = (int)u(0), count = v(1) ? 2 : 1;
+                const uint32_t N = 1u << log_n;
+                uint32_t flags[8] = {u(3), u(6), 0, 0, 0, 0, 0, 0};
+                CHK(scratch[0].alloc(sizeof flags));
+                HIPCHK(hipMemcpy(scratch[0].p, flags, sizeof flags, hipMemcpyHostToDevice));
+                CHK(scratch[1].alloc((size_t)count * N * sizeof(FeU<FRP>)));
+                CHK(ntt_allow_tile_lds<FRP>());
+                const NttPlan plan = ntt_plan(ntt_knobs(), NttPlanIn{log_n, count, N, 0, false, (uint32_t)sizeof(FeU<FRP>), true, false, false});
+                if (plan.rc != APK_OK) { set_error("%s", plan.message); return plan.rc; }
+                NttBatch nb{};
+                NttTails nt{};
+                for (int i = 0; i < count; i++) {
+                    CHK(mk(res[i], N));
+                    nb.in[i] = v(i); nb.out[i] = res[i].p; nb.in_len[i] = N;
+                    nb.wide[i] = ptr<FeU<FRP>>(scratch[1]) + (size_t)i * N;
+                    nt.t[i] = NttTail{ptr<uint32_t>(scratch[0]) + i, u(1 + 3 * i), u(2 + 3 * i)};
+                }
+                CHK(ntt_launch<FRP>(st, plan, nb, count, (const Fr*)v(2), false, nullptr, (const Fr*)v(3), nullptr, &nt));
+                for (int i = 0; i < count; i++) CHK(down(i, res[i].p));
+                return down(2, scratch[0].p);
+            }
         }
         set_error("unknown polynomial-stage op %d", op);
         return APK_ERR_ARG;
diff --git a/algoplonk_amd/plonk.py b/algoplonk_amd/plonk.py
--- a/algoplonk_amd/plonk.py
+++ b/algoplonk_amd/plonk.py
@@ -108,7 +108,12 @@
     def paths(self, reset: bool = False) -> dict:
         pc = _lib.PathCounts()
         check(lib.apk_paths_read(self.ctx, C.byref(pc), int(reset)))
-        return pc.as_dict()
+        out = pc.as_dict()
+        if hasattr(lib, "apk_paths_more_read"):
+            more = _lib.PathCountsMore()
+            check(lib.apk_paths_more_read(self.ctx, C.byref(more), int(reset)))
+            out.update(more.as_dict())
+        return out
 
 
 @dataclass
diff --git a/include/apk.h b/include/apk.h
--- a/include/apk.h
+++ b/include/apk.h
@@ -285,6 +285,7 @@
 #define APK_POLY_BLIND3 9
 #define APK_POLY_TAIL 10
 #define APK_POLY_KZG_QUOTIENT2 11
+#define APK_POLY_NTT_TAIL 12
 #define APK_POLY_VECS 32
 #define APK_POLY_FRS 24
 #define APK_POLY_INTS 8
@@ -356,6 +357,13 @@
     uint64_t msm_inplace;
 } apk_path_counts;
 int apk_paths_read(apk_ctx* ctx, apk_path_counts* out, int reset);
+typedef struct {
+    uint64_t msm_thin_merge;
+    uint64_t tail_in_ntt;
+    uint64_t early_sums;
+    uint64_t reserved[5];
+} apk_path_counts_more;
+int apk_paths_more_read(apk_ctx* ctx, apk_path_counts_more* out, int reset);
 
 typedef struct {
     uint32_t contexts;
```
